# gabegrand/VQA-Counterexamples

Hardware: AMD Instinct MI355X
Metric: VQA-CX triplets/sec (24 candidates each), NeuralCX training step (higher is better)
Workload: dtype f32; 1 GPU; configs[1]: NeuralCX MLP train step (fwd+listwise loss/recall+bwd+Adam), synthetic 2048-d feats, 24 candidates, batch 512 per GPU (weak scaling: global batch 512), H=256, L=1, dropout 0.25, fp32; global_batch=512, per_rank_batch=512, candidates=24, dim_h=256, n_layers=1, parallelism=dp1, feature_table_rows=82783

## Files before the change

### include/neuralcx.h

```cpp
#ifndef NEURALCX_H
#define NEURALCX_H

#include <stddef.h>
#include <stdint.h>

#ifdef __cplusplus
extern "C" {
#endif

#define NCX_OK            0
#define NCX_E_NULL       -1
#define NCX_E_DIMS       -2
#define NCX_E_WORKSPACE  -3
#define NCX_E_FLAGS      -4
#define NCX_E_UNSUPPORTED -5
#define NCX_E_COMM       -6

#define NCX_F_V_MULT   (1u << 0)
#define NCX_F_V_DIST   (1u << 1)
#define NCX_F_V_RANK   (1u << 2)
#define NCX_F_A_EMB    (1u << 3)
#define NCX_F_ALL      (NCX_F_V_MULT | NCX_F_V_DIST | NCX_F_V_RANK | NCX_F_A_EMB)
#define NCX_F_BF16     (1u << 4)
#define NCX_F_REUSE_GT (1u << 5)
#define NCX_F_FUSED_TAIL (1u << 6)
#define NCX_F_X6       (1u << 7)

typedef struct ncx_dims {
    int32_t B;
    int32_t K;
    int32_t dv;
    int32_t dq;
    int32_t dz;
    int32_t da;
    int32_t A;
    int32_t H;
    int32_t L;
    int32_t n_img;
    uint32_t flags;
    int32_t training;
    float   drop_p;
    float   loss_scale;
    uint64_t seed;
} ncx_dims;

typedef struct ncx_inputs {
    const float*   feats;
    const int32_t* img_idx;
    const float*   q_emb;
    const float*   z_orig;
    const float*   z_knns;
    const float*   a_knns;
    const int32_t* answer_aids;
    const float*   a_emb_gt;
    const float*   v_rank;
    const float*   keep_mask;
} ncx_inputs;

typedef struct ncx_params {
    const float* answer_embedding;
    const float* w1;  const float* b1;
    const float* w2;  const float* b2;
    const float* w3;  const float* b3;
    const float* w_out; const float* b_out;
} ncx_params;

typedef struct ncx_grads {
    float* answer_embedding;
    float* w1;  float* b1;
    float* w2;  float* b2;
    float* w3;  float* b3;
    float* w_out; float* b_out;
} ncx_grads;

int64_t ncx_input_size(const ncx_dims* d);

size_t ncx_workspace_bytes(const ncx_dims* d);

int ncx_forward(const ncx_dims* d, const ncx_inputs* in, const ncx_params* p,
                void* workspace, size_t workspace_bytes, float* scores, void* stream);

#define NCX_FWD_ALL     0
#define NCX_FWD_PRELUDE 1
#define NCX_FWD_REST    2
int ncx_forward_phase(const ncx_dims* d, const ncx_inputs* in, const ncx_params* p,
                      void* workspace, size_t workspace_bytes, float* scores, int32_t phase, void* stream);

int ncx_loss_rank(const float* scores, const int32_t* gt, int32_t B, int32_t K, float scale,
                  float* loss_rows, float* loss, float* dscores, int32_t* rank, int32_t* hits,
                  void* stream);

int ncx_backward(const ncx_dims* d, const ncx_inputs* in, const ncx_params* p,
                 void* workspace, size_t workspace_bytes, const float* dscores,
                 const ncx_grads* g, void* stream);

int ncx_backward_phase(const ncx_dims* d, const ncx_inputs* in, const ncx_params* p,
                       void* workspace, size_t workspace_bytes, const float* dscores,
                       const ncx_grads* g, int32_t phase, void* stream);

#define NCX_WS_DGT 1
#define NCX_WS_H1 2
#define NCX_WS_DPRE1 3
#define NCX_WS_DE_PERM 4
int ncx_ws_region(const ncx_dims* d, int32_t which, size_t* offset, size_t* bytes);

int ncx_train_tail(const ncx_dims* d, const ncx_params* p, void* workspace, size_t workspace_bytes, const int32_t* gt,
                   float* scores, float* loss_rows, float* loss, float* dscores, int32_t* rank, int32_t* hits,
                   const ncx_grads* g, void* stream);

#define NCX_COMM_ID_BYTES 128
typedef struct ncx_comm ncx_comm;
int ncx_comm_unique_id(void* id128);
int ncx_comm_create(const void* id128, int32_t nranks, int32_t rank, ncx_comm** out);
int ncx_comm_destroy(ncx_comm* comm);
int ncx_allreduce(ncx_comm* comm, float* buf, size_t n, void* stream);

int ncx_adam_step(float* param, const float* grad, float* exp_avg, float* exp_avg_sq, size_t n,
                  float lr, float beta1, float beta2, float eps, int32_t step, float grad_scale,
                  void* stream);

typedef struct ncx_mutan_params {
    const float* wv;  const float* bv;
    const float* wq;  const float* bq;
    const float* whv; const float* bhv;
    const float* whq; const float* bhq;
    const float* wc;  const float* bc;
    int32_t dhv, dhq, R;
    int32_t act_v, act_q;
} ncx_mutan_params;

size_t ncx_vqa_workspace_bytes(const ncx_dims* d, const ncx_mutan_params* m);

int ncx_vqa_forward(const ncx_dims* d, const float* feats, const int32_t* img_idx, const float* q_emb,
                    const ncx_mutan_params* m, void* workspace, size_t workspace_bytes,
                    float* z_orig, float* z_knns, float* a_knns, float* a_orig, void* stream);

typedef struct ncx_mlb_params {
    const float* wv;  const float* bv;
    const float* wq;  const float* bq;
    const float* wc;  const float* bc;
    int32_t dh;
    int32_t act_v, act_q, act_c;
} ncx_mlb_params;

size_t ncx_mlb_workspace_bytes(const ncx_dims* d, const ncx_mlb_params* m);

int ncx_mlb_forward(const ncx_dims* d, const float* feats, const int32_t* img_idx, const float* q_emb,
                    const ncx_mlb_params* m, void* workspace, size_t workspace_bytes,
                    float* z_orig, float* z_knns, float* a_knns, float* a_orig, void* stream);

typedef struct ncx_mlb_att_dims {
    int32_t B, P, dv, dq, dh_att, G, dh_f, A, n_img;
} ncx_mlb_att_dims;
typedef struct ncx_mlb_att_params {
    const float* wv_att; const float* bv_att;
    const float* wq_att; const float* bq_att;
    const float* wa;     const float* ba;
    const float* wg;     const float* bg;
    const float* wqf;    const float* bqf;
    const float* wc;     const float* bc;
    int32_t act_v_att, act_q_att, act_mm;
    int32_t act_v, act_q, act_c;
} ncx_mlb_att_params;

size_t ncx_mlb_att_workspace_bytes(const ncx_mlb_att_dims* d, const ncx_mlb_att_params* m);

int ncx_mlb_att_forward(const ncx_mlb_att_dims* d, const float* feats, const int32_t* img_idx, const float* q_emb,
                        const ncx_mlb_att_params* m, void* workspace, size_t workspace_bytes,
                        float* logits, float* att, void* stream);
int ncx_mlb_att_forward_flags(const ncx_mlb_att_dims* d, const float* feats, const int32_t* img_idx, const float* q_emb,
                              const ncx_mlb_att_params* m, uint32_t flags, void* workspace, size_t workspace_bytes,
                              float* logits, float* att, void* stream);
int ncx_mlb_att_logits_form(const ncx_mlb_att_dims* d, uint32_t flags);

size_t ncx_knn_status_offset(int32_t n);
size_t ncx_knn_workspace_bytes(int32_t n, int32_t block_rows);
int ncx_knn(const float* table, int32_t n, const float* queries, int32_t nq, int32_t dv, int32_t k,
            int32_t norms_ready, void* workspace, size_t workspace_bytes, int64_t* out_idx, float* out_dist,
            void* stream);

size_t ncx_cosine_gram_workspace_bytes(int32_t A, int32_t da);
int ncx_cosine_gram(const float* emb, int32_t A, int32_t da, void* ws, size_t ws_bytes, float* gram, void* stream);
int ncx_semantic_scores(const float* a_knns, const int32_t* aid, int32_t B, int32_t K, int32_t A, const float* gram,
                        float lam, float* scores, float* raw, int32_t* bad_id_flag, void* stream);

int ncx_similarity_scores(const float* feats, const int32_t* img_idx, int32_t n_img, int32_t dv,
                          const float* z_orig, const float* z_knns, int32_t dz,
                          const float* a_knns, const int32_t* aid, int32_t A,
                          int32_t B, int32_t K,
                          float* scores , float* parts ,
                          int32_t* bad_id_flag, void* stream);

size_t ncx_gru_packed_bytes(int32_t dim_emb, int32_t dim_q);
int ncx_gru_pack(const float* w_ih, const float* w_hh, const float* b_ih, const float* b_hh, int32_t dim_emb, int32_t dim_q,
                 float* packed, void* stream);
size_t ncx_gru_workspace_bytes(int32_t B, int32_t T, int32_t dim_emb, int32_t dim_q);
int ncx_gru_encode(const int32_t* wids, int32_t B, int32_t T, const float* E, int32_t V1, int32_t dim_emb, int32_t dim_q,
                   const float* packed, void* workspace, size_t workspace_bytes, float* q_out, int32_t* bad_id_flag, void* stream);
int ncx_gru_encode_flags(const int32_t* wids, int32_t B, int32_t T, const float* E, int32_t V1, int32_t dim_emb, int32_t dim_q,
                         const float* packed, uint32_t flags, void* workspace, size_t workspace_bytes, float* q_out, int32_t* bad_id_flag,
                         void* stream);
int ncx_gru_step_form(int32_t B, int32_t T, int32_t dim_emb, int32_t dim_q, uint32_t flags);

size_t ncx_gru_train_workspace_bytes(int32_t B, int32_t T, int32_t dim_emb, int32_t dim_q);
size_t ncx_gru_packed_t_bytes(int32_t dim_emb, int32_t dim_q);
int ncx_gru_pack_t(const float* w_ih, const float* w_hh, int32_t dim_emb, int32_t dim_q, float* packed_t, void* stream);
int ncx_gru_train_forward(const int32_t* wids, int32_t B, int32_t T, const float* E, int32_t V1, int32_t dim_emb, int32_t dim_q,
                          const float* packed, void* workspace, size_t workspace_bytes, float* q_out, int32_t* bad_id_flag, void* stream);
int ncx_gru_train_forward_flags(const int32_t* wids, int32_t B, int32_t T, const float* E, int32_t V1, int32_t dim_emb, int32_t dim_q,
                                const float* packed, uint32_t flags, void* workspace, size_t workspace_bytes, float* q_out,
                                int32_t* bad_id_flag, void* stream);
int ncx_gru_train_backward(const int32_t* wids, int32_t B, int32_t T, const float* E, int32_t V1, int32_t dim_emb, int32_t dim_q,
                           const float* packed_t, void* workspace, size_t workspace_bytes, const float* dq_out,
                           float* dW_ih, float* dW_hh, float* db_ih, float* db_hh, float* dE , void* stream);

size_t ncx_lstm2_packed_bytes(int32_t emb, int32_t H);
int ncx_lstm2_pack(const float* w_ih0, const float* w_hh0, const float* b_ih0, const float* b_hh0, const float* w_ih1, const float* w_hh1,
                   const float* b_ih1, const float* b_hh1, int32_t emb, int32_t H, float* packed, void* stream);
size_t ncx_lstm2_workspace_bytes(int32_t B, int32_t T, int32_t emb, int32_t H);
int ncx_lstm2_encode(const int32_t* wids, int32_t B, int32_t T, const float* E, int32_t V1, int32_t emb, int32_t H, const float* packed,
                     void* workspace, size_t workspace_bytes, float* q_out, int32_t* bad_id_flag, void* stream);

size_t ncx_lstm2_train_workspace_bytes(int32_t B, int32_t T, int32_t emb, int32_t H);
size_t ncx_lstm2_packed_t_bytes(int32_t emb, int32_t H);
int ncx_lstm2_pack_t(const float* w_ih0, const float* w_hh0, const float* w_ih1, const float* w_hh1, int32_t emb, int32_t H, float* packed_t,
                     void* stream);
int ncx_lstm2_train_forward(const int32_t* wids, int32_t B, int32_t T, const float* E, int32_t V1, int32_t emb, int32_t H, const float* packed,
                            void* workspace, size_t workspace_bytes, float* q_out, int32_t* bad_id_flag, void* stream);
int ncx_lstm2_train_backward(const int32_t* wids, int32_t B, int32_t T, const float* E, int32_t V1, int32_t emb, int32_t H, const float* packed_t,
                             void* workspace, size_t workspace_bytes, const float* dq_out, float* dW_ih0, float* dW_hh0, float* db_ih0,
                             float* db_hh0, float* dW_ih1, float* dW_hh1, float* db_ih1, float* db_hh1, float* dE , void* stream);

typedef struct ncx_scorer_dims {
    int32_t B, K, dv, dq, dz, A, n_img;
} ncx_scorer_dims;

typedef struct ncx_pairlin_params {
    const float* answer_embedding;
    const float* w;  const float* b;
    const float* w_out; const float* b_out;
} ncx_pairlin_params;
typedef struct ncx_pairlin_grads {
    float* answer_embedding; float* w; float* b; float* w_out; float* b_out;
} ncx_pairlin_grads;

size_t ncx_pairlin_workspace_bytes(const ncx_scorer_dims* d);
int ncx_pairlin_forward(const ncx_scorer_dims* d, const ncx_inputs* in, const ncx_pairlin_params* p, void* workspace,
                        size_t workspace_bytes, float* scores, int32_t* bad_id_flag, void* stream);
int ncx_pairlin_backward(const ncx_scorer_dims* d, const ncx_inputs* in, const ncx_pairlin_params* p, void* workspace,
                         size_t workspace_bytes, const float* dscores, const ncx_pairlin_grads* g, void* stream);
size_t ncx_linctx_workspace_bytes(const ncx_scorer_dims* d);
int ncx_linctx_forward(const ncx_scorer_dims* d, const float* z_knns, const float* w, const float* b, void* workspace,
                       size_t workspace_bytes, float* scores, void* stream);
int ncx_linctx_backward(const ncx_scorer_dims* d, const float* z_knns, const float* dscores, void* workspace,
                        size_t workspace_bytes, float* gw, float* gb, void* stream);

typedef struct ncx_contrastive_dims {
    int32_t B, P, dv, dz, n_img;
} ncx_contrastive_dims;
size_t ncx_contrastive_workspace_bytes(const ncx_contrastive_dims* d);
int ncx_contrastive_forward(const ncx_contrastive_dims* d, const ncx_inputs* in, const float* w, const float* b, void* workspace,
                            size_t workspace_bytes, float* h, int32_t* bad_id_flag, void* stream);
int ncx_contrastive_distances(const ncx_contrastive_dims* d, const float* h, void* workspace, size_t workspace_bytes, float* dist,
                              void* stream);
int ncx_contrastive_loss(const ncx_contrastive_dims* d, void* workspace, size_t workspace_bytes, float margin, float scale,
                         float* losses4, float* dist, void* stream);
int ncx_contrastive_backward(const ncx_contrastive_dims* d, const ncx_inputs* in, void* workspace, size_t workspace_bytes,
                             const float* dh, float* gw, float* gb, void* stream);

typedef struct ncx_vqa_train_dims {
    int32_t B, dv, dq, dz, A, n_img;
    float   p_v, p_q, p_c;
    int32_t dropout_mode;
    int32_t want_dq;
    int32_t pad_;
    uint64_t seed;
} ncx_vqa_train_dims;
typedef struct ncx_mutan_grads {
    float* wv;  float* bv;  float* wq;  float* bq;  float* whv; float* bhv; float* whq; float* bhq; float* wc;  float* bc;
} ncx_mutan_grads;
size_t ncx_vqa_train_workspace_bytes(const ncx_vqa_train_dims* d, const ncx_mutan_params* m);
int ncx_vqa_train_forward(const ncx_vqa_train_dims* d, const float* feats, const int32_t* img_idx, const float* q_emb,
                          const ncx_mutan_params* m, const float* masks, void* workspace, size_t workspace_bytes,
                          float* logits, float* z, void* stream);
int ncx_ce_loss(const float* logits, const int32_t* target, int32_t B, int32_t A, float scale, float* loss, float* dlogits,
                int32_t* hits_top1, int32_t* hits_top5, int32_t* bad_flag, float* rows, void* stream);
int ncx_vqa_train_backward(const ncx_vqa_train_dims* d, const ncx_mutan_params* m, const float* masks, void* workspace,
                           size_t workspace_bytes, const float* dlogits, const ncx_mutan_grads* g, float* dq_emb, void* stream);
#define NCX_VT_WS_VD 1
#define NCX_VT_WS_QD 2
#define NCX_VT_WS_ZC 3
int ncx_vqa_train_ws_region(const ncx_vqa_train_dims* d, const ncx_mutan_params* m, int32_t which, size_t* offset, size_t* bytes);

typedef struct ncx_mlb_grads {
    float* wv;  float* bv;  float* wq;  float* bq;  float* wc;  float* bc;
} ncx_mlb_grads;
size_t ncx_mlb_train_workspace_bytes(const ncx_vqa_train_dims* d, const ncx_mlb_params* m);
int ncx_mlb_train_forward(const ncx_vqa_train_dims* d, const float* feats, const int32_t* img_idx, const float* q_emb,
                          const ncx_mlb_params* m, const float* masks, void* workspace, size_t workspace_bytes,
                          float* logits, float* z, void* stream);
int ncx_mlb_train_backward(const ncx_vqa_train_dims* d, const ncx_mlb_params* m, const float* masks, void* workspace,
                           size_t workspace_bytes, const float* dlogits, const ncx_mlb_grads* g, float* dq_emb, void* stream);
int ncx_mlb_train_ws_region(const ncx_vqa_train_dims* d, const ncx_mlb_params* m, int32_t which, size_t* offset, size_t* bytes);

typedef struct ncx_mlb_att_train {
    float    p_att_v, p_att_q, p_att_mm, p_v, p_q, p_c;
    int32_t  dropout_mode;
    int32_t  want_dq;
    uint64_t seed;
} ncx_mlb_att_train;
typedef struct ncx_mlb_att_grads {
    float* wv_att; float* bv_att; float* wq_att; float* bq_att; float* wa; float* ba;
    float* wg;     float* bg;     float* wqf;    float* bqf;    float* wc; float* bc;
} ncx_mlb_att_grads;
size_t ncx_mlb_att_train_workspace_bytes(const ncx_mlb_att_dims* d, const ncx_mlb_att_train* t, const ncx_mlb_att_params* m);
int ncx_mlb_att_train_forward(const ncx_mlb_att_dims* d, const ncx_mlb_att_train* t, const float* feats, const int32_t* img_idx,
                              const float* q_emb, const ncx_mlb_att_params* m, const float* masks, void* workspace,
                              size_t workspace_bytes, float* logits, float* att, void* stream);
int ncx_mlb_att_train_forward_flags(const ncx_mlb_att_dims* d, const ncx_mlb_att_train* t, const float* feats, const int32_t* img_idx,
                                    const float* q_emb, const ncx_mlb_att_params* m, const float* masks, uint32_t flags, void* workspace,
                                    size_t workspace_bytes, float* logits, float* att, void* stream);
int ncx_mlb_att_train_backward(const ncx_mlb_att_dims* d, const ncx_mlb_att_train* t, const float* feats, const int32_t* img_idx,
                               const float* q_emb, const ncx_mlb_att_params* m, const float* masks, void* workspace,
                               size_t workspace_bytes, const float* att, const float* dlogits, const ncx_mlb_att_grads* g,
                               float* dq_emb, void* stream);
int ncx_mlb_att_train_backward_flags(const ncx_mlb_att_dims* d, const ncx_mlb_att_train* t, const float* feats, const int32_t* img_idx,
                                     const float* q_emb, const ncx_mlb_att_params* m, const float* masks, uint32_t flags, void* workspace,
                                     size_t workspace_bytes, const float* att, const float* dlogits, const ncx_mlb_att_grads* g,
                                     float* dq_emb, void* stream);
int ncx_mlb_att_dwv_form(const ncx_mlb_att_dims* d, uint32_t flags);
#define NCX_AT_WS_XV     1
#define NCX_AT_WS_VATT   2
#define NCX_AT_WS_T      3
#define NCX_AT_WS_VD     4
#define NCX_AT_WS_DWV    5
int ncx_mlb_att_train_ws_region(const ncx_mlb_att_dims* d, const ncx_mlb_att_train* t, const ncx_mlb_att_params* m, int32_t which,
                                size_t* offset, size_t* bytes);

#define NCX_GEMM_GT 0
#define NCX_GEMM_SH 1
#define NCX_GEMM_MAIN 2
#define NCX_GEMM_FWD_L 3
#define NCX_GEMM_DW1C 4
#define NCX_GEMM_DW1S 5
#define NCX_GEMM_DE 6
#define NCX_GEMM_DW1AK 7
#define NCX_GEMM_DAGT 8
#define NCX_GEMM_DWL 9
#define NCX_GEMM_DXL 10
#define NCX_QUERY_DW1_ROUTE 32
int ncx_profile_begin(uint32_t gemm_mask , int32_t max_launches);
int ncx_profile_end(float* ms, int32_t* ids, int32_t cap);
int ncx_profile_stamps(unsigned long long* stamps, int64_t words);
int ncx_plan_query(const ncx_dims* d, int32_t gemm_id, int32_t* out6);
int ncx_wgmap_check(int32_t tiles_m, int32_t tiles_n, int32_t S);

const char* ncx_version(void);

#ifdef __cplusplus
}
#endif
#endif
```

### vqa-counterexamples_amd/csrc/ncx_backward.hip

```cpp
#include "ncx_driver.h"
#include "ncx_wave.h"
#include "ncx_dwred.h"
#include "ncx_bf16.h"

namespace ncx {
__global__ __launch_bounds__(256) void k_dpre_last(const float* __restrict__ gs, const float* __restrict__ w_out,
                                                   const float* __restrict__ h, float* __restrict__ dpre,
                                                   long long total, int H, float scale) {
    long long i = ((long long)blockIdx.x * 256 + threadIdx.x) * 4;
    if (i >= total) return;
    const int r = (int)(i / H), n = (int)(i - (long long)r * H);
    if (n + 3 < H && i + 3 < total) {
        const f32x4 hv = *(const f32x4u*)(h + i);
        const f32x4 wv = *(const f32x4u*)(w_out + n);
        const float g = gs[r];
        f32x4 o;
#pragma unroll
        for (int j = 0; j < 4; ++j) o[j] = hv[j] > 0.f ? g * wv[j] * scale : 0.f;
        *(f32x4u*)(dpre + i) = o;
    } else {
        for (int j = 0; j < 4 && i + j < total; ++j) {
            const int rr = (int)((i + j) / H), nn = (int)((i + j) - (long long)rr * H);
            dpre[i + j] = h[i + j] > 0.f ? gs[rr] * w_out[nn] * scale : 0.f;
        }
// ... 230 lines not shown
                const float gk = __shfl(dsc, k, 64);
                f32x4 dp;
#pragma unroll
                for (int q = 0; q < 4; ++q) { dp[q] = hv[k][q] > 0.f ? gk * w[q] * gate_scale : 0.f; aw[q] = __builtin_fmaf(gk, hv[k][q], aw[q]); ds[q] += dp[q]; }
                put4(dpre + (r0 + k) * H, dp);
            }
        }
        if (dsh) { put4(dsh + (long long)b * H, ds); ab1 += ds; }
    }
    put4(partial_w + (long long)wv * H, aw);
    if (dsh) put4(partial_b1 + (long long)wv * H, ab1);
    sb = wave_sum(sb);
    if (lane == 0) partial_b[wv] = sb;
}

__global__ __launch_bounds__(256) void k_rowgroup_sum(const float* __restrict__ dpre, int B, int K, int H,
                                                      float* __restrict__ dsh) {
    const long long i = (long long)blockIdx.x * 256 + threadIdx.x;
    if (i >= (long long)B * H) return;
    const int b = (int)(i / H), n = (int)(i - (long long)b * H);
    const float* p = dpre + (long long)b * K * H + n;
    float s = 0.f;
    for (int k = 0; k < K; ++k) s += p[(long long)k * H];
    dsh[i] = s;
}

__global__ __launch_bounds__(256) void k_scatter_dsh_by_answer(const float* __restrict__ dsh, const int* __restrict__ aid,
                                                               int B, int H, int A, float* __restrict__ dggt) {
    __shared__ unsigned bits[NCX_SCATTER_MAX_B / 32];
    const int b = blockIdx.x;
    const int id = aid[b];
    int earlier = 0;
    for (int j = threadIdx.x; j < b; j += 256) earlier |= aid[j] == id;
    if (__syncthreads_or(earlier)) return;
    const int nw = (B + 31) / 32;
    for (int w = threadIdx.x; w < nw; w += 256) bits[w] = 0u;
    __syncthreads();
    for (int j = b + threadIdx.x; j < B; j += 256)
        if (aid[j] == id) atomicOr(&bits[j >> 5], 1u << (j & 31));
    __syncthreads();
    for (int n = threadIdx.x; n < H; n += 256) {
        float s = 0.f;
        for (int w = b >> 5; w < nw; ++w) {
            unsigned m = bits[w];
            while (m) {
                const int j = (w << 5) + __ffs(m) - 1;
                m &= m - 1;
                s += dsh[(long long)j * H + n];
            }
        }
        dggt[(long long)n * A + id] = s;
    }
}

struct EmbPrepArgs {
    const float* dsh; const int* aid; float* dggtT;
    const float* src[3]; float* dst[3]; long long lds_[3]; int cols[3], ldd[3], dcols[3], tile0[4];
    int B, H, A, Hp4;
    int* perm;
};
__global__ __launch_bounds__(256) void k_emb_prep(const EmbPrepArgs a, const FixupArgs fix, const Tn8ReduceArgs red) {
    __shared__ unsigned bits[NCX_SCATTER_MAX_B / 32 > 32 * 33 ? NCX_SCATTER_MAX_B / 32 : 32 * 33];
    const int bx = (int)blockIdx.x - (a.perm ? 1 : 0);
    if (bx < 0) {
        __shared__ int scan[256];
        static_assert(NCX_PERM_MAX_A / 32 <= (int)(sizeof(bits) / sizeof(bits[0])), "one bit per answer");
        const int A = a.A, nw = (A + 31) / 32, per = (nw + 255) / 256, tid = threadIdx.x;
        for (int w = tid; w < nw; w += 256) bits[w] = 0u;
        __syncthreads();
        for (int j = tid; j < a.B; j += 256) {
            const int id = a.aid[j];
            if ((unsigned)id < (unsigned)A) atomicOr(&bits[id >> 5], 1u << (id & 31));
        }
        __syncthreads();
        const int w0 = min(tid * per, nw), w1 = min(w0 + per, nw);
        int cnt = 0;
        for (int w = w0; w < w1; ++w) cnt += __popc(bits[w]);
        scan[tid] = cnt;
        __syncthreads();
        for (int off = 1; off < 256; off <<= 1) {
            const int v = tid >= off ? scan[tid - off] : 0;
            __syncthreads();
            scan[tid] += v;
            __syncthreads();
        }
        const int n_present = scan[255];
        int pos = scan[tid] - cnt;
        for (int w = w0; w < w1; ++w) {
            const unsigned m = bits[w];
            for (int bit = 0; bit < 32; ++bit) {
                const int id = 32 * w + bit;
                if (id >= A) break;
                if ((m >> bit) & 1u) a.perm[pos++] = id;
                else a.perm[n_present + (id - pos)] = id;
            }
        }
        if (tid == 0) a.perm[A] = n_present;
        return;
    }
    if (bx >= a.B + a.tile0[3]) {
        const int id = bx - (a.B + a.tile0[3]);
        const int nfix = fix.valid ? fix.grid_x * 4 : 0;
        if (id < nfix) split_fixup_body<64, 64>(fix, id / 4, id % 4);
        else tn8_reduce_body(red, id - nfix);
        return;
    }
    if (bx < a.B) {
        const int b = bx, B = a.B;
        const int id = a.aid[b];
        int earlier = 0;
        for (int j = threadIdx.x; j < b; j += 256) earlier |= a.aid[j] == id;
        if (__syncthreads_or(earlier)) return;
        const int nw = (B + 31) / 32;
        for (int w = threadIdx.x; w < nw; w += 256) bits[w] = 0u;
        __syncthreads();
        for (int j = b + threadIdx.x; j < B; j += 256)
            if (a.aid[j] == id) atomicOr(&bits[j >> 5], 1u << (j & 31));
        __syncthreads();
        for (int n = threadIdx.x; n < a.H; n += 256) {
            float s = 0.f;
            for (int w = b >> 5; w < nw; ++w) {
                unsigned m = bits[w];
                while (m) { const int j = (w << 5) + __ffs(m) - 1; m &= m - 1; s += a.dsh[(long long)j * a.H + n]; }
            }
            a.dggtT[(long long)id * a.Hp4 + n] = s;
        }
        return;
    }
    float* tile = (float*)bits;
    int t = bx - a.B, e = 0;
    while (e < 2 && t >= a.tile0[e + 1]) ++e;
    t -= a.tile0[e];
    const int tiles_h = (a.dcols[e] + 31) / 32;
    const int th = t % tiles_h, tc = t / tiles_h;
    const int x = threadIdx.x & 31, y = threadIdx.x >> 5;
#pragma unroll
    for (int i = 0; i < 4; ++i) {
        const int h = th * 32 + y + 8 * i, c = tc * 32 + x;
        tile[(y + 8 * i) * 33 + x] = (h < a.H && c < a.cols[e]) ? a.src[e][(long long)h * a.lds_[e] + c] : 0.f;
    }
    __syncthreads();
#pragma unroll
    for (int i = 0; i < 4; ++i) {
        const int c = tc * 32 + y + 8 * i, h = th * 32 + x;
        if (c < a.cols[e] && h < a.dcols[e]) a.dst[e][(long long)c * a.ldd[e] + h] = tile[x * 33 + y + 8 * i];
    }
}

__global__ __launch_bounds__(256) void k_zero_cols(float* __restrict__ p, int rows, long long ld, int cols) {
    const long long i = (long long)blockIdx.x * 256 + threadIdx.x;
    if (i >= (long long)rows * cols) return;
    const int r = (int)(i / cols), c = (int)(i - (long long)r * cols);
    p[(long long)r * ld + c] = 0.f;
}
}

using namespace ncx;
extern "C" {
int ncx_train_tail(const ncx_dims* dp, const ncx_params* p, void* workspace, size_t workspace_bytes, const int32_t* gt,
                   float* scores, float* loss_rows, float* loss, float* dscores, int32_t* rank, int32_t* hits,
                   const ncx_grads* g, void* stream_) {
    int rc = check_dims(dp);
    if (rc != NCX_OK) return rc;
    if (!p || !workspace || !gt || !scores || !loss_rows || !rank || !g) return NCX_E_NULL;
    if (!p->w_out || !p->b_out || !g->w_out || !g->b_out || !g->b1) return NCX_E_NULL;
    const ncx_dims& d = *dp;
    if (!(d.flags & NCX_F_FUSED_TAIL)) return NCX_E_FLAGS;
    if (d.K > 32 || d.H > 256) return NCX_E_DIMS;
    const StepRoutes r = routes(d);
    const WsLayout w = ws_layout(d, r);
    if (workspace_bytes < w.total || ((uintptr_t)workspace & 255)) return NCX_E_WORKSPACE;
    hipStream_t s = (hipStream_t)stream_;
    char* ws = (char*)workspace;
    const int H = d.H;
    const bool aemb = d.flags & NCX_F_A_EMB;
    const bool emb_nt = r.emb_nt;
    const int Hp4 = pad_to(H, 4);
    float* dagtT = (float*)(ws + w.dgtT) + (size_t)d.A * Hp4;
    float* dagt = (float*)(ws + w.dagt);
    float* partial = (float*)(ws + w.partial);
    float* part_w = partial;
    float* part_b1 = partial + (size_t)NCX_PRELUDE_WAVES * H;
    float* part_b = partial + (size_t)NCX_PRELUDE_WAVES * H * 2;
    const float dscale = (d.training && d.drop_p > 0.f) ? 1.f / (1.f - d.drop_p) : 1.f;
    const float scale = d.loss_scale > 0.f ? d.loss_scale : 1.f / (float)d.B;
    const int nblk = (int)cdiv(d.B < NCX_PRELUDE_WAVES ? d.B : NCX_PRELUDE_WAVES, 4);
    const bool fuse_l1 = d.L == 1;
    const float* hL = (const float*)(ws + w.h[d.L - 1]);
    float* dpre = (float*)(ws + w.dpre[0]);
    float* dsh = fuse_l1 ? (float*)(ws + w.dsh) : (float*)nullptr;
    float* zb = emb_nt ? dagtT : aemb ? dagt : (float*)nullptr;
    const long long zn = emb_nt ? (long long)d.A * Hp4 : (long long)H * d.A;
#define NCX_TAIL_LAUNCH(KB, FULL) hipLaunchKernelGGL((k_train_tail<KB, FULL>), dim3(nblk * 4), dim3(64), 0, s, hL, p->w_out, p->b_out, gt, d.B, d.K, H, scale, dscale, \
                                               scores, loss_rows, dscores, rank, dpre, dsh, part_w, part_b1, part_b, zb, zn, zchunk)
    const int zchunk = (int)((cdiv(zn, (long long)nblk * 4) + 3) / 4 * 4);
    if (H == 256 && d.K == 24) NCX_TAIL_LAUNCH(24, true);
    else if (d.K <= 8) NCX_TAIL_LAUNCH(8, false); else if (d.K <= 16) NCX_TAIL_LAUNCH(16, false); else if (d.K <= 24) NCX_TAIL_LAUNCH(24, false); else NCX_TAIL_LAUNCH(32, false);
#undef NCX_TAIL_LAUNCH
    NCX_HIP_TRY(hipGetLastError());
    hipLaunchKernelGGL(k_bwd_prelude_finish, dim3((unsigned)cdiv(H, 8), 3), dim3(256), 0, s, (const float*)part_w, (const float*)part_b1,
                       (const float*)part_b, nblk * 4, H, g->w_out, fuse_l1 ? g->b1 : (float*)nullptr, g->b_out,
                       (const float*)loss_rows, (const int*)rank, d.B, loss, hits);
    NCX_HIP_TRY(hipGetLastError());
    return NCX_OK;
}

static int backward_impl(const ncx_dims* dp, const ncx_inputs* in, const ncx_params* p, void* workspace,
                         size_t workspace_bytes, const float* dscores, const ncx_grads* g, void* stream_, int phase) {
    int rc = check_dims(dp);
    if (rc != NCX_OK) return rc;
    if (!in || !p || !workspace || !g || (!dscores && !(dp->flags & NCX_F_FUSED_TAIL))) return NCX_E_NULL;
    const ncx_dims& d = *dp;
    const bool aemb = d.flags & NCX_F_A_EMB;
    if (!g->answer_embedding || !g->w1 || !g->b1 || !g->w_out || !g->b_out) return NCX_E_NULL;
    if (d.L >= 2 && (!g->w2 || !g->b2)) return NCX_E_NULL;
    if (d.L >= 3 && (!g->w3 || !g->b3)) return NCX_E_NULL;
    const StepRoutes r = routes(d);
    const WsLayout w = ws_layout(d, r);
    if (workspace_bytes < w.total || ((uintptr_t)workspace & 255)) return NCX_E_WORKSPACE;
    hipStream_t s = (hipStream_t)stream_;
    char* ws = (char*)workspace;
    const int M = d.B * d.K, H = d.H;
    const SegOffsets o = seg_offsets(d);
    const long long din = o.din;
    const int* idx_k = (const int*)(ws + w.idx_k); const int* idx_o = (const int*)(ws + w.idx_o);
    const int* idx_ob = (const int*)(ws + w.idx_ob);
    const float* mx = (const float*)(ws + w.mx); const float* inv = (const float*)(ws + w.inv);
    const float* misc = (const float*)(ws + w.misc);
    float* dsh = (float*)(ws + w.dsh); float* dgt = (float*)(ws + w.dgt); float* dagt = (float*)(ws + w.dagt);
    const bool emb_nt = r.emb_nt;
    const int Hp4 = pad_to(H, 4), Hp32 = pad_to(H, 32);
    float* dgtT = (float*)(ws + w.dgtT); float* dagtT = dgtT + (size_t)d.A * Hp4;
    float* w1akT = (float*)(ws + w.w1aT); float* w1agtT = w1akT + (size_t)d.da * Hp32;
    float* partial = (float*)(ws + w.partial); float* slab = (float*)(ws + w.slab);
    GemmUse u[U_COUNT];
    list_uses(d, r, u);
    const float dscale = (d.training && d.drop_p > 0.f) ? 1.f / (1.f - d.drop_p) : 1.f;

    auto colsum = [&](const float* x, const float* wgt, int rows, int cols, float* out) -> int {
        const int ch = rows < NCX_COLSUM_CHUNKS * 8 ? (int)cdiv(rows, 8) : NCX_COLSUM_CHUNKS;
        hipLaunchKernelGGL(k_colsum_partial, dim3((unsigned)cdiv(cols, 256), ch), dim3(256), 0, s, x, wgt, rows, cols, partial);
        hipLaunchKernelGGL(k_colsum_finish, dim3((unsigned)cdiv(cols, 8)), dim3(256), 0, s, (const float*)partial, ch, cols, out);
        return (int)hipGetLastError();
    };

    const float* hL = (const float*)(ws + w.h[d.L - 1]);
    float* dpre = (float*)(ws + w.dpre[0]);
    const bool only_de = phase == 4;
    const bool skip_de = phase == 3 || phase == 5;
    const bool do1 = phase != 2 && !only_de, do2 = phase != 1 && phase != 5 && !only_de;
    const bool de_skip = r.de_skip && (phase == 0 || phase == 1);
    int* const de_perm = (int*)(ws + w.de_perm);
    if (!do1) {
        dpre = (float*)(ws + w.dpre[(d.L - 1) & 1]);
    } else if (d.flags & NCX_F_FUSED_TAIL) {
    } else {
        const int nblk = (int)cdiv(d.B < NCX_PRELUDE_WAVES ? d.B : NCX_PRELUDE_WAVES, 4);
        float* part_w = partial;
        float* part_b1 = partial + (size_t)NCX_PRELUDE_WAVES * H;
        float* part_b = partial + (size_t)NCX_PRELUDE_WAVES * H * 2;
        const bool fuse_l1 = d.L == 1;
        hipLaunchKernelGGL(k_bwd_prelude, dim3(nblk), dim3(256), 0, s, dscores, p->w_out, hL, dpre, fuse_l1 ? dsh : (float*)nullptr,
                           d.B, d.K, H, dscale, part_w, part_b1, part_b,
                           emb_nt ? dagtT : aemb ? dagt : (float*)nullptr, emb_nt ? (long long)d.A * Hp4 : (long long)H * d.A);
        NCX_HIP_TRY(hipGetLastError());
        hipLaunchKernelGGL(k_bwd_prelude_finish, dim3((unsigned)cdiv(H, 8), fuse_l1 ? 2 : 1), dim3(256), 0, s, (const float*)part_w,
                           (const float*)part_b1, (const float*)part_b, nblk * 4, H, g->w_out, fuse_l1 ? g->b1 : (float*)nullptr, g->b_out);
        NCX_HIP_TRY(hipGetLastError());
    }
    int cur = 0;
    for (int l = d.L; l >= 2 && do1; --l) {
        const float* wl = l == 2 ? p->w2 : p->w3;
        float* gw = l == 2 ? g->w2 : g->w3;
        float* gb = l == 2 ? g->b2 : g->b3;
        const float* hprev = (const float*)(ws + w.h[l - 2]);
        rc = colsum(dpre, nullptr, M, H, gb); if (rc) return rc;
        {
            GemmArgs a{}; a.mode = MODE_GROUP; a.nseg = 1; a.M = H;
            a.a[0] = x_plain(dpre, H, M, H); a.b[0] = x_plain(hprev, H, M, H); a.klen[0] = M;
            a.out[0] = gw; a.ldo[0] = H; a.n_cols[0] = H;
            rc = run_gemm(U_DWL, a, FORM_TN, u[U_DWL].plan, slab, w.slab_bytes, nullptr, s); if (rc) return rc;
        }
        {
            float* dnext = (float*)(ws + w.dpre[cur ^ 1]);
            GemmArgs a{}; a.mode = MODE_CHAIN; a.nseg = 1; a.M = M;
            a.a[0] = x_plain(dpre, H, M, H); a.b[0] = x_plain(wl, H, H, H); a.klen[0] = H;
            a.out[0] = dnext; a.ldo[0] = H; a.n_cols[0] = H;
            a.epi.gate = hprev; a.epi.ld_gate = H; a.epi.gate_scale = dscale;
            rc = run_gemm(U_DXL, a, FORM_NN, u[U_DXL].plan, slab, w.slab_bytes, nullptr, s); if (rc) return rc;
            dpre = dnext; cur ^= 1;
        }
    }
    if (do1 && d.L >= 2) {
        hipLaunchKernelGGL(k_rowgroup_sum, dim3((unsigned)cdiv((long long)d.B * H, 256)), dim3(256), 0, s, (const float*)dpre, d.B, d.K, H, dsh);
        NCX_HIP_TRY(hipGetLastError());
        rc = colsum(dsh, nullptr, d.B, H, g->b1); if (rc) return rc;
    }
    bool km_deferred = false, km_reduced = false;
    auto run_km = [&](bool finish = true) -> int {
        return profiled(U_DW1C, s, [&] { return dw_km(d, dpre, in->feats, idx_k, idx_o, (float*)(ws + w.km_slab), g->w1 + o.v_other, g->w1 + o.v_mult, din, s, finish); });
    };
    {
        GemmArgs a{}; a.mode = MODE_GROUP; a.M = H;
        int n = 0;
        auto add_c = [&](const XDesc& x, float* out, long long ldo) {
            a.a[n] = x_plain(dpre, H, M, H); a.b[n] = x; a.klen[n] = M; a.out[n] = out; a.ldo[n] = ldo; a.n_cols[n] = x.cols;
            a.split[n] = dw1c_seg_split(x.cols, u[U_DW1C].plan.split, u[U_DW1C].ksteps); ++n; };
        auto add_s = [&](const XDesc& x, float* out) {
            a.a[n] = x_plain(dsh, H, d.B, H); a.b[n] = x; a.klen[n] = d.B; a.out[n] = out; a.ldo[n] = din; a.n_cols[n] = x.cols;
            a.split[n] = u[U_DW1S].plan.split; ++n; };
        const bool bf16 = d.flags & NCX_F_BF16;
        const bool want_dgt = aemb && do1 && !bf16, want_rest = do2;
        if (bf16 && do1) {
            rc = profiled(U_DW1C, s, [&] { return bf16_dw1c(d, dpre, (u16*)(ws + w.dpre_bf), (const u16*)(ws + w.xc), (float*)(ws + w.bf_slab), g->w1, dgt, s); }); if (rc) return rc;
        }
        const bool km = r.km;
        const bool tn8 = r.tn8;
        km_deferred = want_rest && do1 && do2 && km_defers_to_side_stream(d, r);
        const bool km_merge = want_rest && km && !km_deferred && !hook_env("NCX_NO_MERGE_FIX");
        if (want_rest && km && !km_deferred) {
            rc = run_km(!km_merge); if (rc) return rc;
        }
        if (want_rest && !bf16 && !km) {
            add_c(x_gather(in->feats, d.dv, idx_k, M, d.dv), g->w1 + o.v_other, din);
            if (d.flags & NCX_F_V_MULT) add_c(x_gather_mul(in->feats, d.dv, idx_k, idx_o, M, d.dv), g->w1 + o.v_mult, din);
        }
        if (tn8 && (want_dgt || want_rest)) {
            Tn8Prob tp[TN8_MAX_PROB]; int np = 0, n_al = 0;
            auto prob = [&](const float* A_, int rows, const float* X, long long ldx, const float* lse, int gsel, int N, float* out, long long ldo, int n_valid) {
                tp[np] = Tn8Prob{};
                Tn8Prob& q = tp[np++]; q.A = A_; q.rows = rows; q.X = X; q.ldx = ldx; q.lse = lse; q.gsel = gsel; q.N = N; q.out = out; q.ldo = ldo; q.n_valid = n_valid; };
            if (aemb) {
                prob(dpre, M, in->a_knns, d.A, mx, 0, d.A, dgt, d.A, d.A); n_al = 1;
                if (emb_nt) {
                    tp[0].outT = dgtT; tp[0].outT2 = (float*)(ws + w.dgtT2); tp[0].ldT = Hp4; tp[0].padT2 = pad_to(d.A, 32) - d.A;
                }
            }
            else prob(dpre, M, in->a_knns, d.da, nullptr, 0, d.da, g->w1 + o.a_other, din, d.da);
            prob(dpre, M, in->z_knns, d.dz, nullptr, 0, d.dz, g->w1 + o.z_other, din, d.dz);
            prob(dpre, M, misc, w.ldm, nullptr, 0, w.ldm, g->w1 + o.v_dist, din, d.K + 1);
            prob(dsh, d.B, in->feats, d.dv, nullptr, 1, d.dv, g->w1 + o.v_orig, din, d.dv);
            prob(dsh, d.B, in->q_emb, d.dq, nullptr, 0, d.dq, g->w1 + o.q_emb, din, d.dq);
            prob(dsh, d.B, in->z_orig, d.dz, nullptr, 0, d.dz, g->w1 + o.z_orig, din, d.dz);
            if (aemb) prob(dsh, d.B, p->answer_embedding, d.da, nullptr, 2, d.da, g->w1 + o.a_gt, din, d.da);
            else      prob(dsh, d.B, in->a_emb_gt, d.da, nullptr, 0, d.da, g->w1 + o.a_gt, din, d.da);
            const bool with_km = want_rest && km && !km_deferred && km_merge;
            Tn8ReduceArgs red{};
            rc = prof_open(U_DW1C, s); if (rc) return rc;
            rc = dw_tn8_products(d, tp, np, n_al, want_dgt, want_rest, idx_ob, aemb ? in->answer_aids : nullptr, slab, w.slab_bytes, &red, s); if (rc) return rc;
            bool kvec = true;
            KmReduceArgs kr{};
            if (with_km) { kr = dw_km_reduce_args(d, (const float*)(ws + w.km_slab), g->w1 + o.v_other, g->w1 + o.v_mult, din, &kvec); km_reduced = true; }
            rc = dw_reduce_km_tn8(with_km ? &kr : nullptr, kvec, &red, s); if (rc) return rc;
            rc = prof_close(U_DW1C, s); if (rc) return rc;
        }
        if (want_rest && !bf16 && !tn8) {
            if (!aemb) add_c(x_plain(in->a_knns, d.da, M, d.da), g->w1 + o.a_other, din);
        }
        if (want_dgt && !tn8) add_c(x_softmax(in->a_knns, d.A, mx, inv, M, d.A), dgt, d.A);
        if (want_rest && !bf16 && !tn8) {
            add_c(x_plain(in->z_knns, d.dz, M, d.dz), g->w1 + o.z_other, din);
            add_c(x_plain(misc, w.ldm, M, d.K + 1), g->w1 + o.v_dist, din);
        }
        if (want_rest && bf16 && r.tn8_shared) {
            Tn8Prob tp[4]; int np = 0;
            auto prob = [&](const float* X, long long ldx, int gsel, int N, float* out) {
                tp[np] = Tn8Prob{};
                Tn8Prob& q = tp[np++]; q.A = dsh; q.rows = d.B; q.X = X; q.ldx = ldx; q.gsel = gsel; q.N = N; q.out = out; q.ldo = din; q.n_valid = N; };
            prob(in->feats, d.dv, 1, d.dv, g->w1 + o.v_orig);
            prob(in->q_emb, d.dq, 0, d.dq, g->w1 + o.q_emb);
            prob(in->z_orig, d.dz, 0, d.dz, g->w1 + o.z_orig);
            if (aemb) prob(p->answer_embedding, d.da, 2, d.da, g->w1 + o.a_gt);
            else      prob(in->a_emb_gt, d.da, 0, d.da, g->w1 + o.a_gt);
            rc = dw_tn8(d, tp, np, 0, false, true, idx_ob, aemb ? in->answer_aids : nullptr, slab, w.slab_bytes, s); if (rc) return rc;
        } else
        if (want_rest && !tn8) {
            add_s(x_gather(in->feats, d.dv, idx_ob, d.B, d.dv), g->w1 + o.v_orig);
            add_s(x_plain(in->q_emb, d.dq, d.B, d.dq), g->w1 + o.q_emb);
            add_s(x_plain(in->z_orig, d.dz, d.B, d.dz), g->w1 + o.z_orig);
            add_s(aemb ? x_gather(p->answer_embedding, d.da, in->answer_aids, d.B, d.da) : x_plain(in->a_emb_gt, d.da, d.B, d.da),
                  g->w1 + o.a_gt);
        }
        a.nseg = n;
        FixupArgs fix_tn{};
        if (km_merge) a.defer_fix = &fix_tn;
        if (n > 0) { rc = run_gemm(U_DW1C, a, FORM_TN, u[U_DW1C].plan, slab, w.slab_bytes, nullptr, s); if (rc) return rc; }
        if (km_merge && !km_reduced) {
            rc = profiled(U_DW1C, s, [&] { return dw_km_finish(d, (const float*)(ws + w.km_slab), g->w1 + o.v_other, g->w1 + o.v_mult, din, &fix_tn, u[U_DW1C].plan.cfg, s); }); if (rc) return rc;
        }
        if (!(d.flags & NCX_F_V_MULT) && do2) {
            hipLaunchKernelGGL(k_zero_cols, dim3((unsigned)cdiv((long long)H * d.dv, 256)), dim3(256), 0, s, g->w1 + o.v_mult, H, din, d.dv);
            NCX_HIP_TRY(hipGetLastError());
        }
    }
    if (aemb) {
        SideStream* ss = km_deferred ? side_stream() : nullptr;
        hipStream_t se = ss ? ss->s : s;
        FixupArgs fix_ak{};
        Tn8ReduceArgs red_ak{};
        const bool tn8_ak = r.dw1ak_on_tn8(ss != nullptr);
        if (ss) { rc = side_fork(ss, s); if (rc) return rc; }
        const bool bf16e = d.flags & NCX_F_BF16;
        const Bf16Emb bm = bf16e ? bf16_emb_layout(d, ws + w.bf_emb) : Bf16Emb{};
        if (do2 && bf16e) {
            rc = profiled(U_DW1AK, se, [&] { return bf16_dw1ak(d, bm, dgt, g->w1, se); }); if (rc) return rc;
        } else if (do2 && tn8_ak) {
            Tn8Prob q{};
            q.A = (const float*)(ws + w.dgtT2); q.rows = pad_to(d.A, 32); q.rows_valid = d.A; q.X = p->answer_embedding; q.ldx = d.da; q.N = d.da;
            q.out = g->w1 + o.a_other; q.ldo = din; q.n_valid = d.da;
            rc = prof_open(U_DW1AK, se); if (rc) return rc;
            rc = dw_tn8_products(d, &q, 1, 0, false, true, nullptr, nullptr, slab, w.slab_bytes, &red_ak, se); if (rc) return rc;
            if (!(do1 && emb_nt)) { rc = dw_reduce_km_tn8(nullptr, true, &red_ak, se); if (rc) return rc; red_ak.n_tiles_total = 0; }
            rc = prof_close(U_DW1AK, se); if (rc) return rc;
        } else if (do2) {
            GemmArgs a{}; a.mode = MODE_CHAIN; a.nseg = 1; a.M = H;
            a.a[0] = x_plain(dgt, d.A, H, d.A); a.b[0] = x_plain(p->answer_embedding, d.da, d.A, d.da); a.klen[0] = d.A;
            a.out[0] = g->w1 + o.a_other; a.ldo[0] = din; a.n_cols[0] = d.da;
            if (do1 && emb_nt && u[U_DW1AK].plan.cfg == CFG_64x64 && !hook_env("NCX_NO_MERGE_FIX")) a.defer_fix = &fix_ak;
            rc = run_gemm(U_DW1AK, a, FORM_NN, u[U_DW1AK].plan, ss ? (float*)(ws + w.slab2) : slab,
                          ss ? w.slab2_bytes : w.slab_bytes, nullptr, se); if (rc) return rc;
        }
        if (do1 && emb_nt) {
            EmbPrepArgs ea{};
            ea.dsh = dsh; ea.aid = in->answer_aids; ea.dggtT = dagtT; ea.B = d.B; ea.H = H; ea.A = d.A; ea.Hp4 = Hp4;
            const float* srcs[3] = {dgt, p->w1 + o.a_other, p->w1 + o.a_gt};
            float* dsts[3] = {dgtT, w1akT, w1agtT};
            const long long ldss[3] = {d.A, din, din};
            const int colss[3] = {tn8_ak ? 0 : d.A, d.da, d.da}, ldds[3] = {Hp4, Hp32, Hp32};
            int tiles = 0;
            for (int e = 0; e < 3; ++e) {
                ea.src[e] = srcs[e]; ea.dst[e] = dsts[e]; ea.lds_[e] = ldss[e]; ea.cols[e] = colss[e]; ea.ldd[e] = ldds[e]; ea.dcols[e] = ldds[e];
                ea.tile0[e] = tiles; tiles += ((ldds[e] + 31) / 32) * ((colss[e] + 31) / 32);
            }
            ea.tile0[3] = tiles;
            ea.perm = de_skip ? de_perm : (int*)nullptr;
            hipLaunchKernelGGL(k_emb_prep, dim3((de_skip ? 1 : 0) + d.B + tiles + (fix_ak.valid ? fix_ak.grid_x * 4 : 0) + red_ak.n_tiles_total * 8), dim3(256), 0, se, ea, fix_ak, red_ak);
            fix_ak.valid = 0; red_ak.n_tiles_total = 0;
            NCX_HIP_TRY(hipGetLastError());
        } else if (do1) {
            hipLaunchKernelGGL(k_scatter_dsh_by_answer, dim3(d.B), dim3(256), 0, se, (const float*)dsh, in->answer_aids, d.B, H, d.A, dagt);
            NCX_HIP_TRY(hipGetLastError());
        }
        if (fix_ak.valid) { rc = run_fixup2(fix_ak, FixupArgs{}, CFG_64x64, se); if (rc) return rc; }
        if (((do1 && !skip_de) || only_de) && bf16e) {
            rc = profiled(U_DE, se, [&] { return bf16_de(d, bm, dgt, g->answer_embedding, se); }); if (rc) return rc;
        } else if (((do1 && !skip_de) || only_de) && emb_nt) {
            MainArgs a{}; a.M = d.A; a.N = d.da; a.nseg = 2;
            a.seg[0].kind = MK_PLAIN; a.seg[0].a = dgtT;  a.seg[0].lda = Hp4; a.seg[0].klen = Hp4; a.seg[0].b = w1akT;  a.seg[0].ldb = Hp32;
            a.seg[1].kind = MK_PLAIN; a.seg[1].a = dagtT; a.seg[1].lda = Hp4; a.seg[1].klen = Hp4; a.seg[1].b = w1agtT; a.seg[1].ldb = Hp32;
            a.out = g->answer_embedding; a.ldo = d.da;
            a.split = 1;
            if (de_skip) {
                a.seg[0].kind = MK_GATHER; a.seg[0].idx = de_perm;
                a.seg[1].kind = MK_GATHER; a.seg[1].idx = de_perm;
            }
            rc = profiled(U_DE, se, [&] { return de_skip ? main_forward_rowmap(a, se) : main_forward(a, se); }); if (rc) return rc;
        } else if ((do1 && !skip_de) || only_de) {
            GemmArgs a{}; a.mode = MODE_CHAIN; a.nseg = 2; a.M = d.A;
            a.a[0] = x_plain(dgt, d.A, H, d.A);  a.b[0] = x_plain(p->w1 + o.a_other, din, H, d.da); a.klen[0] = H;
            a.a[1] = x_plain(dagt, d.A, H, d.A); a.b[1] = x_plain(p->w1 + o.a_gt, din, H, d.da);    a.klen[1] = H;
            a.out[0] = g->answer_embedding; a.ldo[0] = d.da; a.n_cols[0] = d.da;
            rc = run_gemm(U_DE, a, FORM_TN, u[U_DE].plan, ss ? (float*)(ws + w.slab2) : slab, ss ? w.slab2_bytes : w.slab_bytes, nullptr, se); if (rc) return rc;
        }
        if (km_deferred) { rc = run_km(); if (rc) return rc; }
        if (ss) { rc = side_join(ss, s); if (rc) return rc; }
    } else if (do1) {
        NCX_HIP_TRY(hipMemsetAsync(g->answer_embedding, 0, (size_t)d.A * d.da * 4, s));
    }
    return NCX_OK;
}

int ncx_backward(const ncx_dims* dp, const ncx_inputs* in, const ncx_params* p, void* workspace,
                 size_t workspace_bytes, const float* dscores, const ncx_grads* g, void* stream_) {
    return backward_impl(dp, in, p, workspace, workspace_bytes, dscores, g, stream_, 0);
}

int ncx_backward_phase(const ncx_dims* dp, const ncx_inputs* in, const ncx_params* p, void* workspace,
                       size_t workspace_bytes, const float* dscores, const ncx_grads* g, int32_t phase, void* stream_) {
    if (phase < 0 || phase > 5) return NCX_E_FLAGS;
    return backward_impl(dp, in, p, workspace, workspace_bytes, dscores, g, stream_, phase);
}

int ncx_ws_region(const ncx_dims* dp, int32_t which, size_t* offset, size_t* bytes) {
    if (check_dims(dp) != NCX_OK) return NCX_E_DIMS;
    if (!offset || !bytes) return NCX_E_NULL;
    if (which != NCX_WS_DGT && which != NCX_WS_H1 && which != NCX_WS_DPRE1 && which != NCX_WS_DE_PERM) return NCX_E_FLAGS;
    const StepRoutes r = routes(*dp);
    const WsLayout w = ws_layout(*dp, r);
    if (which == NCX_WS_DE_PERM) {
        *offset = w.de_perm; *bytes = r.de_skip ? ((size_t)dp->A + 1) * 4 : 0;
        return NCX_OK;
    }
    if (which == NCX_WS_H1 || which == NCX_WS_DPRE1) {
        *offset = which == NCX_WS_H1 ? w.h[0] : w.dpre[(dp->L - 1) & 1];
        *bytes = (size_t)dp->B * dp->K * dp->H * 4;
        return NCX_OK;
    }
    if (!r.emb_nt) { *offset = w.dgt; *bytes = (dp->flags & NCX_F_A_EMB) ? (size_t)2 * dp->H * dp->A * 4 : 0; }
    else { *offset = w.dgtT; *bytes = (size_t)2 * dp->A * pad_to(dp->H, 4) * 4; }
    return NCX_OK;
}
}
```

### vqa-counterexamples_amd/csrc/ncx_diag.hip

```cpp
#include "ncx_driver.h"
#include <stdlib.h>

using namespace ncx;
extern "C" {
int ncx_profile_begin(uint32_t gemm_mask, int32_t max_launches) {
    if (g_prof.on || gemm_mask == 0 || (gemm_mask >> U_COUNT) != 0 || max_launches < 1 || max_launches > 65536) return NCX_E_DIMS;
    g_prof.ev = (hipEvent_t*)malloc(sizeof(hipEvent_t) * 2 * (size_t)max_launches);
    g_prof.ids = (int*)malloc(sizeof(int) * (size_t)max_launches);
    if (!g_prof.ev || !g_prof.ids) return NCX_E_NULL;
    for (int i = 0; i < 2 * max_launches; ++i) NCX_HIP_TRY(hipEventCreate(&g_prof.ev[i]));
    g_prof.mask = gemm_mask; g_prof.n = 0; g_prof.cap = max_launches; g_prof.on = true;
    return NCX_OK;
}

int ncx_profile_end(float* ms, int32_t* ids, int32_t cap) {
    if (!g_prof.on) return NCX_E_FLAGS;
    int n = 0;
    for (int i = 0; i < g_prof.n; ++i) {
        if (hipEventSynchronize(g_prof.ev[2 * i + 1]) != hipSuccess) break;
        float t = 0.f;
        if (hipEventElapsedTime(&t, g_prof.ev[2 * i], g_prof.ev[2 * i + 1]) != hipSuccess) break;
        if (n < cap) { if (ms) ms[n] = t; if (ids) ids[n] = g_prof.ids[i]; }
        ++n;
    }
    for (int i = 0; i < 2 * g_prof.cap; ++i) (void)hipEventDestroy(g_prof.ev[i]);
    free(g_prof.ev); free(g_prof.ids);
    g_prof.ev = nullptr; g_prof.ids = nullptr; g_prof.on = false; g_prof.mask = 0; g_prof.n = 0; g_prof.cap = 0;
    return n < cap ? n : cap;
}

int ncx_profile_stamps(unsigned long long* stamps, int64_t words) {
    if ((stamps == nullptr) != (words == 0) || words < 0) return NCX_E_DIMS;
    int dev = 0;
    NCX_HIP_TRY(hipGetDevice(&dev));
    if (dev < 0 || dev >= 16) return NCX_E_DIMS;
    if (!stamps) { g_stamps[dev].ptr.store(nullptr, std::memory_order_release); g_stamps[dev].words.store(0, std::memory_order_release); }
    else { g_stamps[dev].ptr.store(nullptr, std::memory_order_release); g_stamps[dev].words.store(words, std::memory_order_release);
           g_stamps[dev].ptr.store(stamps, std::memory_order_release); }
    return NCX_OK;
}

int ncx_wgmap_check(int32_t tiles_m, int32_t tiles_n, int32_t S) {
    if (tiles_m < 1 || tiles_n < 1 || S < 1 || (long long)tiles_m * tiles_n * S > (1 << 24)) return NCX_E_DIMS;
    const WgMap w{tiles_m, tiles_n, S};
    const int total = tiles_m * tiles_n * S, count = w.count();
    if (count < total) return 1;
    unsigned char* seen = (unsigned char*)calloc((size_t)total, 1);
    if (!seen) return NCX_E_NULL;
    int bad = 0, nvalid = 0;
    for (int lw = 0; lw < count && !bad; ++lw) {
        int tm = -1, tn = -1, z = -1;
        if (!w.decode(lw, tm, tn, z)) continue;
        ++nvalid;
        if (tm < 0 || tm >= tiles_m || tn < 0 || tn >= tiles_n || z < 0 || z >= S) { bad = 2; break; }
        if (w.encode(tm, tn, z) != lw) { bad = 3; break; }
        unsigned char& f = seen[((size_t)z * tiles_m + tm) * tiles_n + tn];
        if (f) { bad = 4; break; }
        f = 1;
    }
    if (!bad && nvalid != total) bad = 5;
    free(seen);
    return bad;
}

int ncx_plan_query(const ncx_dims* d, int32_t gemm_id, int32_t* out6) {
    if (check_dims(d) != NCX_OK || !out6) return NCX_E_DIMS;
    if (gemm_id == NCX_QUERY_DW1_ROUTE) {
        const bool bf16 = d->flags & NCX_F_BF16;
        const StepRoutes r = routes(*d);
        out6[0] = r.km_form;
        out6[1] = (bf16 ? r.tn8_shared : r.tn8) ? (r.tn8_x6 ? 2 : 1) : 0;
        int grid = 0;
        out6[2] = dw_tn8_pieces(*d, bf16 ? TN8_LIST_SHARED : TN8_LIST_MAIN, &grid);
        out6[3] = grid;
        out6[4] = r.dw1ak_on_tn8(km_defers_to_side_stream(*d, r)) ? 1 : 0;
        out6[5] = TN8_MAX_SEG;
        return NCX_OK;
    }
    if (gemm_id < 0 || gemm_id >= U_COUNT) return NCX_E_DIMS;
    GemmUse u[U_COUNT];
    list_uses(*d, routes(*d), u);
    out6[0] = u[gemm_id].form; out6[1] = (int32_t)u[gemm_id].M; out6[2] = (int32_t)u[gemm_id].N;
    out6[3] = (int32_t)u[gemm_id].ksteps; out6[4] = u[gemm_id].plan.cfg; out6[5] = u[gemm_id].plan.split;
    const bool fast = (gemm_id == U_MAIN && main_fwd_dims_ok(*d)) || (gemm_id == U_FWD_L && hidden_fwd_dims_ok(*d) && !(d->flags & NCX_F_BF16));
    if (fast) {
        const long long M = (long long)d->B * d->K, T = u[gemm_id].ksteps;
        const int sp = main_split(M, d->H, T);
        const bool vfold = gemm_id == U_MAIN && (d->flags & NCX_F_V_MULT) && (d->K == 24 || (d->K == 48 && main_fold_rows(M, d->H) >= 96)) && d->dv % 32 == 0 && d->dv >= 64 && sp == 1;
        const long long tiles96 = ((M + 95) / 96) * ((d->H + 127) / 128);
        out6[4] = vfold ? (main_fold_rows(M, d->H) == 192 ? 8 : (main_fold_rows(M, d->H) == 96 || d->K == 48) ? 7 : 6) : (sp == 1 && tiles96 * 10 >= (long long)num_cus() * 9) ? CFG_96x128 : 5;
        out6[5] = sp;
    }
    return NCX_OK;
}
}
```

### vqa-counterexamples_amd/csrc/ncx_driver.h

```cpp
#pragma once
#include "ncx_plan.h"
#include <atomic>

#pragma GCC visibility push(hidden)
namespace ncx {
struct SideStream { hipStream_t s; hipEvent_t fork, join; int state, mode; };
SideStream* side_stream();
int side_fork(SideStream* ss, hipStream_t main);
int side_join(SideStream* ss, hipStream_t main);
bool km_defers_to_side_stream(const ncx_dims& d, const StepRoutes& r);

struct ProfState { bool on; unsigned mask; int n, cap; hipEvent_t* ev; int* ids; };
extern ProfState g_prof;
struct StampSlot { std::atomic<unsigned long long*> ptr; std::atomic<long long> words; };
extern StampSlot g_stamps[16];
unsigned long long* stamps_for_current_device(long long need_words);
int prof_open(int use_id, hipStream_t s);
int prof_close(int use_id, hipStream_t s);
template <class F> static inline int profiled(int use_id, hipStream_t s, F&& launch) {
    int rc = prof_open(use_id, s); if (rc) return rc;
    rc = launch(); if (rc) return rc;
    return prof_close(use_id, s);
}
int run_gemm(int use_id, GemmArgs& a, int form, const GemmPlan& pl, float* slab, size_t slab_bytes, const float* reduce_bias, hipStream_t s);
void set_dropout(EpiArgs& e, const ncx_dims& d, const ncx_inputs& in, int layer, long long M);
}
#pragma GCC visibility pop
```

### vqa-counterexamples_amd/csrc/ncx_internal.h

```cpp
#pragma once
#include "ncx_common.h"
#include "ncx_gemm.h"

namespace ncx {

enum TileCfg : int { CFG_64x64 = 0, CFG_128x128 = 1, CFG_96x128 = 2, CFG_96x64 = 3, CFG_128x64 = 4 };
enum GemmForm : int { FORM_NT = 0, FORM_TN = 1, FORM_NN = 2 };

int run_gemm_nt(GemmArgs& a, int cfg, hipStream_t s);
int run_fixup2(const FixupArgs& a, const FixupArgs& b, int cfg, hipStream_t s);
int run_gemm_nt_fold(GemmArgs& a, hipStream_t s);
int run_gemm_tn(GemmArgs& a, int cfg, hipStream_t s);
int run_gemm_nn(GemmArgs& a, int cfg, hipStream_t s);
int occupancy_nt(int cfg);
int occupancy_tn(int cfg);
int occupancy_nn(int cfg);

struct SegOffsets {
    int v_orig, v_other, v_mult, v_dist, v_rank, q_emb, z_orig, z_other, a_gt, a_other, din;
};
static inline SegOffsets seg_offsets(const ncx_dims& d) {
    SegOffsets o; int c = 0;
    o.v_orig = c;  c += d.dv;
    o.v_other = c; c += d.dv;
    o.v_mult = c;  c += d.dv;
    o.v_dist = c;  c += 1;
    o.v_rank = c;  c += d.K;
    o.q_emb = c;   c += d.dq;
    o.z_orig = c;  c += d.dz;
    o.z_other = c; c += d.dz;
    o.a_gt = c;    c += d.da;
    o.a_other = c; c += d.da;
    o.din = c;
    return o;
}

struct GemmPlan { int cfg; int split; };
GemmPlan plan_gemm(int form, long long M, long long N, long long ksteps, bool allow_96);
int num_cus();
static inline long long cdiv(long long a, long long b) { return (a + b - 1) / b; }
static inline long long ksteps(long long k) { return cdiv(k, GEMM_BK); }
__attribute__((visibility("hidden"))) size_t gemm_slab_bytes(GemmArgs a, const GemmPlan& pl);
__attribute__((visibility("hidden"))) int run_gemm_planned(GemmArgs& a, int form, const GemmPlan& pl, float* slab, size_t slab_bytes,
                                                           const float* reduce_bias, hipStream_t s);
__attribute__((visibility("hidden"))) hipError_t colsum_rows(const float* in, long long ld, int R, int cols, float* out, hipStream_t s);

struct WsLayout {
    size_t idx_k, idx_o, idx_ob;
    size_t mx, inv;
    size_t misc;
    size_t gt;
    size_t sh;
    size_t h[3];
    size_t dpre[2];
    size_t dsh;
    size_t dgt;
    size_t dagt;
    size_t dgtT;
    size_t dgtT2;
    size_t de_perm;
    size_t w1aT;
    size_t partial;
    size_t slab;
    size_t slab_bytes;
    size_t slab2, slab2_bytes;
    size_t xc, wc, dpre_bf, bf_slab;
    size_t bf_emb;
    size_t km_slab;
    size_t mslab, mslab_bytes;
    size_t wpad;
    int ldm;
    int ldgt;
    size_t total;
};
constexpr int NCX_COLSUM_CHUNKS = 256;
constexpr int NCX_PRELUDE_WAVES = 1024;

enum MainKind : int { MK_PLAIN = 0, MK_GATHER = 1, MK_GATHER_MUL = 2, MK_SOFTMAX = 3,
                      MK_VFOLD = 4 };
constexpr int MAIN_MAX_SEG = 5;
struct MainSeg {
    const float* a;
    const int*   idx;
    const int*   idx2;
    const float* lse;
    const float* b;
    const float* b2;
    long long lda, ldb;
    int kind, klen;
};
struct MainArgs {
    MainSeg seg[MAIN_MAX_SEG]; int nseg, M, N, split; float* out; long long ldo; EpiArgs epi;
    float* slab;
    float* dist_out; long long ld_dist;
    unsigned long long* stamps;
    int x6;
    float* t_out; float* t_out0;
};
int main_forward(MainArgs& a, hipStream_t s);
int main_forward_rowmap(MainArgs& a, hipStream_t s);
int main_forward_mlb(MainArgs& a, hipStream_t s);
int main_split(long long M, long long N, long long T);
int main_fold_rows_eff(long long M, long long N, int rowdiv);
int main_fold_rows(long long M, long long N);

constexpr int DW_KM_SPLIT = 8;
bool dw_km_supported(const ncx_dims& d);
enum DwKmForm : int { KM_FORM_NONE = 0, KM_FORM_8 = 1, KM_FORM_X6 = 2, KM_FORM_GENERIC = 3, KM_FORM_GROUPED = 4 };
int dw_km_form(const ncx_dims& d);
size_t dw_km_slab_bytes(const ncx_dims& d);
int dw_km(const ncx_dims& d, const float* dpre, const float* feats, const int* idx_k, const int* idx_o, float* slab,
          float* g_vother, float* g_vmult, long long din, hipStream_t s, bool finish = true);
int dw_km_finish(const ncx_dims& d, const float* slab, float* g_vother, float* g_vmult, long long din, const FixupArgs* fix, int fix_cfg,
                 hipStream_t s);
constexpr int TN8_MAX_PROB = 8;
constexpr int TN8_MAX_SEG = 16;
struct Tn8Prob {
    const float* A;
    const float* X; long long ldx;
    const float* lse;
    int gsel;
    int rows, N;
    float* out; long long ldo; int n_valid;
    int rows_valid;
    float* outT; float* outT2; long long ldT; int padT2;
};
bool dw_tn8_supported(const ncx_dims& d);
bool dw_tn8_shapes_ok(const ncx_dims& d);
bool dw_tn8_shared_ok(const ncx_dims& d);
enum Tn8List : int { TN8_LIST_MAIN = 0, TN8_LIST_SHARED = 1, TN8_LIST_AK = 2 };
int dw_tn8_pieces(const ncx_dims& d, int list, int* grid);
bool dw_tn8_x6(const ncx_dims& d);
size_t dw_tn8_slab_bytes(const ncx_dims& d);
int dw_tn8(const ncx_dims& d, const Tn8Prob* probs, int np, int n_al, bool do_al, bool do_rest, const int* idx_ob, const int* aid,
           float* slab, size_t slab_bytes, hipStream_t s);
bool mutan_fold_supported(const ncx_dims& d, const ncx_mutan_params& m);
int mutan_fold(const ncx_dims& d, const ncx_mutan_params& m, const float* xv, const float* hq, float* z_orig, float* z_knns, hipStream_t s);
__attribute__((visibility("hidden"))) hipError_t pad_rows(const float* src, long long ld_src, int cols, float* dst, int ldd, int rows, hipStream_t s);
WsLayout ws_layout(const ncx_dims& d);
__host__ __device__ static inline int pad_to(int x, int m) { return (x + m - 1) / m * m; }
static inline bool main_fwd_extents_ok(const ncx_dims& d) {
    const long long lim = (1ll << 32) - 65536, M = (long long)d.B * d.K, wa = d.A > d.da ? d.A : d.da;
    return (long long)d.n_img * d.dv * 4 < lim && M * wa * 4 < lim && M * (long long)d.H * 4 < lim && M * (long long)d.dz * 4 < lim && (long long)d.A * wa * 4 < lim &&
           (long long)d.H * (2ll * d.dv + d.dq + 2ll * d.dz + 2ll * d.da + d.K + 2) * 4 < lim;
}
static inline bool main_fwd_dims_ok(const ncx_dims& d) {
    return d.dv % 4 == 0 && d.dz % 4 == 0 && ((d.flags & NCX_F_A_EMB) ? d.A : d.da) % 4 == 0 && !(d.flags & NCX_F_BF16) && main_fwd_extents_ok(d);
}
static inline bool hidden_fwd_dims_ok(const ncx_dims& d) { return d.H % 4 == 0 && main_fwd_extents_ok(d); }
constexpr uint32_t NCX_F_PRIV_DIST_IN_MAIN = 1u << 30;


}
```

### vqa-counterexamples_amd/csrc/ncx_loss_adam.hip

```cpp
#include "ncx_wave.h"

namespace ncx {
__global__ __launch_bounds__(256) void k_loss_rank(const float* __restrict__ scores, const int* __restrict__ gt,
                                                   int B, int K, float scale, float* __restrict__ loss_rows,
                                                   float* __restrict__ dscores, int* __restrict__ rank) {
    const int lane = threadIdx.x & 63;
    const int b = blockIdx.x * 4 + (threadIdx.x >> 6);
    if (b >= B) return;
    const float s = lane < K ? scores[(long long)b * K + lane] : -INFINITY;
    const int g = gt[b];
    const float m = wave_max(s);
    const float e = lane < K ? __expf(s - m) : 0.f;
    const float sum = wave_sum(e);
    const float sg = __shfl(s, g, 64);
    if (dscores && lane < K) dscores[(long long)b * K + lane] = (e / sum - (lane == g ? 1.f : 0.f)) * scale;
    const bool ahead = lane < K && (s > sg || (s == sg && lane < g));
    const unsigned long long bal = __ballot(ahead);
    if (lane == 0) {
        if (loss_rows) loss_rows[b] = (logf(sum) - (sg - m)) * scale;
        if (rank) rank[b] = __popcll(bal);
    }
}

__global__ __launch_bounds__(256) void k_loss_finish(const float* __restrict__ loss_rows, const int* __restrict__ rank,
                                                     int B, float* __restrict__ loss, int* __restrict__ hits) {
    __shared__ float sl[4];
    __shared__ int s1[4], s5[4];
    float acc = 0.f; int h1 = 0, h5 = 0;
    for (int i = threadIdx.x; i < B; i += 256) {
        if (loss_rows) acc += loss_rows[i];
        if (rank) { const int rk = rank[i]; h1 += rk < 1; h5 += rk < 5; }
    }
    acc = wave_sum(acc);
    h1 = (int)wave_sum((float)h1); h5 = (int)wave_sum((float)h5);
    const int w = threadIdx.x >> 6;
    if ((threadIdx.x & 63) == 0) { sl[w] = acc; s1[w] = h1; s5[w] = h5; }
    __syncthreads();
    if (threadIdx.x == 0) {
        if (loss) loss[0] = sl[0] + sl[1] + sl[2] + sl[3];
        if (hits) { hits[0] = s1[0] + s1[1] + s1[2] + s1[3]; hits[1] = s5[0] + s5[1] + s5[2] + s5[3]; }
    }
}

__global__ __launch_bounds__(256) void k_adam(float* __restrict__ p, const float* __restrict__ g, float* __restrict__ m,
                                              float* __restrict__ v, size_t n, float step_size, float b1, float b2,
                                              float eps, float inv_bc2_sqrt, float gscale) {
    size_t i = ((size_t)blockIdx.x * 256 + threadIdx.x) * 4;
    const size_t stride = (size_t)gridDim.x * 256 * 4;
    for (; i < n; i += stride) {
        if (i + 3 < n) {
            f32x4 pv = *(f32x4*)(p + i), gv = *(const f32x4*)(g + i), mv = *(f32x4*)(m + i), vv = *(f32x4*)(v + i);
#pragma unroll
            for (int j = 0; j < 4; ++j) {
                const float gj = gv[j] * gscale;
                mv[j] = mv[j] + (gj - mv[j]) * (1.f - b1);
                vv[j] = vv[j] * b2 + (1.f - b2) * gj * gj;
                const float den = sqrtf(vv[j]) * inv_bc2_sqrt + eps;
                pv[j] = pv[j] - step_size * (mv[j] / den);
            }
            *(f32x4*)(p + i) = pv; *(f32x4*)(m + i) = mv; *(f32x4*)(v + i) = vv;
        } else {
            for (size_t j = i; j < n; ++j) {
                const float gj = g[j] * gscale;
                const float mj = m[j] + (gj - m[j]) * (1.f - b1);
                const float vj = v[j] * b2 + (1.f - b2) * gj * gj;
                m[j] = mj; v[j] = vj;
                p[j] = p[j] - step_size * (mj / (sqrtf(vj) * inv_bc2_sqrt + eps));
            }
        }
    }
}
}

using namespace ncx;
extern "C" {
int ncx_loss_rank(const float* scores, const int32_t* gt, int32_t B, int32_t K, float scale, float* loss_rows,
                  float* loss, float* dscores, int32_t* rank, int32_t* hits, void* stream_) {
    if (!scores || !gt) return NCX_E_NULL;
    if (B < 1 || K < 1 || K > 64) return NCX_E_DIMS;
    if ((loss && !loss_rows) || (hits && !rank)) return NCX_E_NULL;
    hipStream_t s = (hipStream_t)stream_;
    if (scale <= 0.f) scale = 1.f / (float)B;
    hipLaunchKernelGGL(k_loss_rank, dim3((unsigned)cdiv(B, 4)), dim3(256), 0, s, scores, gt, B, K, scale, loss_rows, dscores, rank);
    NCX_HIP_TRY(hipGetLastError());
    if (loss || hits) {
        hipLaunchKernelGGL(k_loss_finish, dim3(1), dim3(256), 0, s, (const float*)loss_rows, (const int*)rank, B, loss, hits);
        NCX_HIP_TRY(hipGetLastError());
    }
    return NCX_OK;
}

int ncx_adam_step(float* param, const float* grad, float* exp_avg, float* exp_avg_sq, size_t n, float lr,
                  float beta1, float beta2, float eps, int32_t step, float grad_scale, void* stream_) {
    if (!param || !grad || !exp_avg || !exp_avg_sq) return NCX_E_NULL;
    if (step < 1 || n == 0) return NCX_E_DIMS;
    if (((uintptr_t)param | (uintptr_t)grad | (uintptr_t)exp_avg | (uintptr_t)exp_avg_sq) & 15) return NCX_E_WORKSPACE;
    const double bc1 = 1.0 - pow((double)beta1, (double)step);
    const double bc2 = 1.0 - pow((double)beta2, (double)step);
    const float step_size = (float)((double)lr / bc1);
    const float inv_bc2_sqrt = (float)(1.0 / sqrt(bc2));
    size_t blocks = (n + 1023) / 1024;
    if (blocks > 4096) blocks = 4096;
    hipLaunchKernelGGL(k_adam, dim3((unsigned)blocks), dim3(256), 0, (hipStream_t)stream_, param, grad, exp_avg, exp_avg_sq, n,
                       step_size, beta1, beta2, eps, inv_bc2_sqrt, grad_scale);
    NCX_HIP_TRY(hipGetLastError());
    return NCX_OK;
}
}
```

### vqa-counterexamples_amd/csrc/ncx_main.h

```cpp
#pragma once
#include "ncx_internal.h"
#include <type_traits>

namespace ncx {

constexpr int MF_BK = 32, MF_P = MF_BK + 4, MF_T = 256;

enum { LK_PLAIN = 0, LK_MUL = 1, LK_SOFTMAX = 2 };
template <int V> struct IntC { static constexpr int value = V; };

constexpr int MF6_P = 80;
template <int BM_, int BN_, int WGM_, int WGN_, int DEPTH_, int OCC_, int T_ = MF_T, bool X6_ = false>
struct MainCfg {
    static constexpr int BM = BM_, BN = BN_, WGM = WGM_, WGN = WGN_, DEPTH = DEPTH_, OCC = OCC_, T = T_;
    static constexpr bool X6 = X6_;
    static constexpr int EPI = 0;
    static constexpr int RP = T / 8;
    static constexpr int BM_LDS = (BM + RP - 1) / RP * RP;
    static constexpr int LDS6 = 2 * 3 * (BM_LDS + BN) * MF6_P;
    static constexpr int LDS_FOLD6 = 2 * (3 * 208 * MF6_P + 8 * 32 * 4 + 128 * MF_P * 4);
    static constexpr int LDS32 = 2 * (BM_LDS + BN) * MF_P * 4;
    static constexpr int LDS = !X6_ ? LDS32 : (LDS_FOLD6 > LDS6 ? (LDS_FOLD6 > LDS32 ? LDS_FOLD6 : LDS32) : (LDS6 > LDS32 ? LDS6 : LDS32));
    static constexpr int LDS_FOLD = BM % 96 == 0 ? 2 * (32 * (T / 64) + 128) * MF_P * 4
                                                 : 2 * (80 + 2 * 64) * MF_P * 4;
};

enum { EPI_STD = 0, EPI_MLB = 1, EPI_ROWMAP = 2 };
template <class CFG> struct WithMlbEpi : CFG { static constexpr int EPI = EPI_MLB; };
template <class CFG> struct WithRowMap : CFG { static constexpr int EPI = EPI_ROWMAP; };

typedef const __attribute__((address_space(1))) float* gfptr;
typedef const __attribute__((address_space(1))) int* giptr;
typedef const __attribute__((address_space(1))) f32x4u* gf4ptr;

template <class CFG, bool DIST, int K0, int K1 = -1, int K2 = -1, int K3 = -1, int K4 = -1>
__global__ __launch_bounds__(CFG::T, CFG::OCC) void k_main_fwd(const MainArgs args) {
    constexpr bool VFOLD = K0 == MK_VFOLD;
    constexpr int DIST_SEG = VFOLD ? 1 : 2;
    static_assert(!DIST || (VFOLD ? K1 == MK_PLAIN : (K1 == MK_GATHER_MUL && K2 == MK_PLAIN)), "DIST: v_o, v_k segment followed by the dist | rank segment");
    static_assert(!VFOLD || (CFG::BM == 48 && CFG::BN == 64 && CFG::WGM == 1 && CFG::WGN == 4 && CFG::DEPTH == 2) ||
                            (CFG::BM == 96 && CFG::BN == 64 && CFG::WGM == 2 && CFG::WGN == 2 && CFG::DEPTH == 2) ||
                            (CFG::BM == 192 && CFG::BN == 64 && CFG::T == 512 && CFG::WGM == 4 && CFG::WGN == 2 && CFG::DEPTH == 2), "fold: 48 x 64, 96 x 64 or (8 waves) 192 x 64 tiles");
    static_assert(!(DIST && CFG::X6), "the X6 form leaves the distance to k_prep");
    constexpr int KS[6] = {K0, K1, K2, K3, K4, -1};
    constexpr int NSEG = K1 < 0 ? 1 : K2 < 0 ? 2 : K3 < 0 ? 3 : K4 < 0 ? 4 : 5;
    constexpr int BM = CFG::BM, BN = CFG::BN, BK = MF_BK, P = MF_P, DEPTH = CFG::DEPTH, BML = CFG::BM_LDS;
    constexpr int WTM = BM / CFG::WGM, WTN = BN / CFG::WGN, WM = WTM / 16, WN = WTN / 16, NSUB = BK / 8, NMF = 2 * WM * WN;
    constexpr int MT = CFG::T, RP = CFG::RP;
    static_assert(CFG::WGM * CFG::WGN == MT / 64 && WTM % 16 == 0 && WTN % 16 == 0 && BN % RP == 0 && NSUB == 4, "tile");
    static_assert(MT == 256 || !VFOLD || BM % 96 == 0, "the 48-row fold is a 256-thread form");
    constexpr int NA = BML / RP, NB = BN / RP;
    extern __shared__ __attribute__((aligned(16))) float mf_smem[];
    float* const lds_a = mf_smem;
    float* const lds_b = mf_smem + 2 * BML * P;
    const int tid = threadIdx.x, lane = tid & 63, wave = tid >> 6, li = lane & 15, lk = lane >> 4;
    const int wm0 = (wave / CFG::WGN) * WTM, wn0 = (wave % CFG::WGN) * WTN;
    const int M = args.M, N = args.N;
    const int tiles_m = (M + BM - 1) / BM, tiles_n = (N + BN - 1) / BN;
    const int S = args.split > 1 ? args.split : 1;
    const int id = blockIdx.x, xcd = id & 7, local = id >> 3;
    const int tn = local % tiles_n, unit = (local / tiles_n) * 8 + xcd;
    if (unit >= tiles_m * S) return;
    const int tm = unit / S, z = unit - tm * S;
    const int m0 = tm * BM, n0 = tn * BN;
    const int quad = tid & 7, trow = tid >> 3;
    unsigned long long* const stamps = args.stamps ? args.stamps + (size_t)blockIdx.x * 16 : nullptr;
    auto stamp = [&](int slot) __attribute__((always_inline)) {
        if (stamps && tid == 0) stamps[slot] = __builtin_readcyclecounter();
    };
    if (stamps && tid == 0) { stamps[14] = __builtin_amdgcn_s_memrealtime(); stamps[13] = __builtin_amdgcn_s_getreg((3 << 11) | (0 << 6) | 20); }
    stamp(0);

    f32x4 acc[WM][WN];
#pragma unroll
    for (int i = 0; i < WM; ++i)
#pragma unroll
        for (int j = 0; j < WN; ++j) acc[i][j] = f32x4{0.f, 0.f, 0.f, 0.f};
    f32x2 afA[WM], bfA[WN], afB[WM], bfB[WN];
#pragma unroll
    for (int i = 0; i < WM; ++i) afB[i] = f32x2{0.f, 0.f};
#pragma unroll
    for (int j = 0; j < WN; ++j) bfB[j] = f32x2{0.f, 0.f};

    auto read_frags = [&](int buf, int s, f32x2 (&af)[WM], f32x2 (&bf)[WN]) __attribute__((always_inline)) {
        const float* a = lds_a + buf * BML * P + (wm0 + li) * P + 8 * s + 2 * lk;
        const float* b = lds_b + buf * BN * P + (wn0 + li) * P + 8 * s + 2 * lk;
#pragma unroll
        for (int i = 0; i < WM; ++i) af[i] = *(const f32x2*)(a + i * 16 * P);
#pragma unroll
        for (int j = 0; j < WN; ++j) bf[j] = *(const f32x2*)(b + j * 16 * P);
    };
    auto mfma = [&](const f32x2 (&af)[WM], const f32x2 (&bf)[WN]) __attribute__((always_inline)) {
#pragma unroll
        for (int e = 0; e < 2; ++e)
#pragma unroll
            for (int i = 0; i < WM; ++i)
#pragma unroll
                for (int j = 0; j < WN; ++j) acc[i][j] = __builtin_amdgcn_mfma_f32_16x16x4f32(af[i][e], bf[j][e], acc[i][j], 0, 0, 0);
    };

    constexpr bool X6 = CFG::X6;
    static_assert(!X6 || (VFOLD && BM == 192 && WM == 3 && WN == 2 && DEPTH == 2), "X6: the 8-wave 192 x 64 fold form only");
    typedef __bf16 mbf16x8 __attribute__((ext_vector_type(8)));
    typedef unsigned int mu32x2 __attribute__((ext_vector_type(2)));
    constexpr int P6 = MF6_P, A6_PL = BML * P6, PL6 = (BML + BN) * P6, BUF6 = 3 * PL6;
    unsigned char* const lds6 = (unsigned char*)mf_smem;
    mbf16x8 xa[2][3], xb[2][X6 ? WN : 1][3];
    auto split_store6 = [&](f32x4 v, unsigned char* base) __attribute__((always_inline)) {
        unsigned p1[4], p2[4], p3[4];
#pragma unroll
        for (int j = 0; j < 4; ++j) {
            const float xj = v[j];
            p1[j] = __builtin_bit_cast(unsigned, xj) & 0xFFFF0000u;
            const float r1 = xj - __builtin_bit_cast(float, p1[j]);
            p2[j] = __builtin_bit_cast(unsigned, r1) & 0xFFFF0000u;
            const float r2 = r1 - __builtin_bit_cast(float, p2[j]);
            p3[j] = __builtin_bit_cast(unsigned, r2);
        }
        const mu32x2 w1 = {__builtin_amdgcn_perm(p1[1], p1[0], 0x07060302u), __builtin_amdgcn_perm(p1[3], p1[2], 0x07060302u)};
        const mu32x2 w2 = {__builtin_amdgcn_perm(p2[1], p2[0], 0x07060302u), __builtin_amdgcn_perm(p2[3], p2[2], 0x07060302u)};
        const mu32x2 w3 = {__builtin_amdgcn_perm(p3[1], p3[0], 0x07060302u), __builtin_amdgcn_perm(p3[3], p3[2], 0x07060302u)};
        *(mu32x2*)(base) = w1; *(mu32x2*)(base + PL6) = w2; *(mu32x2*)(base + 2 * PL6) = w3;
    };
    auto read_a6 = [&](int buf, int i, mbf16x8 (&f)[3]) __attribute__((always_inline)) {
        const unsigned char* a = lds6 + buf * BUF6 + (wm0 + 16 * i + li) * P6 + 16 * lk;
#pragma unroll
        for (int p = 0; p < 3; ++p) f[p] = *(const mbf16x8*)(a + p * PL6);
    };
    auto read_b6 = [&](int buf, mbf16x8 (&f)[X6 ? WN : 1][3]) __attribute__((always_inline)) {
        const unsigned char* b = lds6 + buf * BUF6 + A6_PL + (wn0 + li) * P6 + 16 * lk;
#pragma unroll
        for (int j = 0; j < (X6 ? WN : 1); ++j)
#pragma unroll
            for (int p = 0; p < 3; ++p) f[j][p] = *(const mbf16x8*)(b + j * 16 * P6 + p * PL6);
    };
    auto mfma6 = [&](const mbf16x8 (&a)[3], const mbf16x8 (&b)[X6 ? WN : 1][3], f32x4 (&c)[WN]) __attribute__((always_inline)) {
        if constexpr (X6) {
#pragma unroll
            for (int j = 0; j < WN; ++j) c[j] = __builtin_amdgcn_mfma_f32_16x16x32_bf16(a[0], b[j][2], c[j], 0, 0, 0);
#pragma unroll
            for (int j = 0; j < WN; ++j) c[j] = __builtin_amdgcn_mfma_f32_16x16x32_bf16(a[1], b[j][1], c[j], 0, 0, 0);
#pragma unroll
            for (int j = 0; j < WN; ++j) c[j] = __builtin_amdgcn_mfma_f32_16x16x32_bf16(a[2], b[j][0], c[j], 0, 0, 0);
#pragma unroll
            for (int j = 0; j < WN; ++j) c[j] = __builtin_amdgcn_mfma_f32_16x16x32_bf16(a[0], b[j][1], c[j], 0, 0, 0);
#pragma unroll
            for (int j = 0; j < WN; ++j) c[j] = __builtin_amdgcn_mfma_f32_16x16x32_bf16(a[1], b[j][0], c[j], 0, 0, 0);
#pragma unroll
            for (int j = 0; j < WN; ++j) c[j] = __builtin_amdgcn_mfma_f32_16x16x32_bf16(a[0], b[j][0], c[j], 0, 0, 0);
        }
    };

    int nsteps[MAIN_MAX_SEG], total_steps = 0;
#pragma unroll
    for (int i = 0; i < MAIN_MAX_SEG; ++i) { nsteps[i] = i < NSEG ? (args.seg[i].klen + BK - 1) / BK : 0; total_steps += nsteps[i]; }
    constexpr bool ROWMAP = CFG::EPI == EPI_ROWMAP;
    static_assert(!ROWMAP || (K0 == MK_GATHER && K1 == MK_GATHER && NSEG == 2 && !DIST && !X6), "row map: two gathered segments");
    const int g0 = (int)((long long)total_steps * z / S), g1_all = (int)((long long)total_steps * (z + 1) / S);
    const int g1 = [&]() __attribute__((always_inline)) {
        if constexpr (ROWMAP) return m0 >= ((giptr)args.seg[0].idx)[M] ? min(g1_all, nsteps[0]) : g1_all;
        else return g1_all;
    }();

    f32x4 va[DEPTH][NA], vm[DEPTH][NA], vb[DEPTH][NB];
    typedef unsigned int bu32x4 __attribute__((ext_vector_type(4)));
    __amdgpu_buffer_rsrc_t rsPA = __builtin_amdgcn_make_buffer_rsrc((void*)nullptr, 0, 0, 0x00020000), rsPB = rsPA;
    unsigned roA[NA], roM[NA], roB[NB]; float lse[NA];
    float dacc[NA];
    constexpr int FOLD_DIST_OFF = 2 * (BML + BN) * P > 32 * (MT / 64) * 68 ? 2 * (BML + BN) * P : 32 * (MT / 64) * 68;
#pragma unroll
    for (int i = 0; i < NA; ++i) dacc[i] = 0.f;
    auto setup = [&](auto kind_c, const MainSeg& g) __attribute__((always_inline)) {
        constexpr int KIND = decltype(kind_c)::value;
#pragma unroll
        for (int i = 0; i < NA; ++i) {
            const int r = min(m0 + min(trow + RP * i, BM - 1), M - 1);
            constexpr bool GAT = KIND == MK_GATHER || KIND == MK_GATHER_MUL;
            const unsigned row = GAT ? (unsigned)((giptr)g.idx)[r] : (unsigned)r;
            roA[i] = row * (unsigned)(g.lda * 4);
            roM[i] = KIND == MK_GATHER_MUL ? (unsigned)((giptr)g.idx2)[r] * (unsigned)(g.lda * 4) : roA[i];
            lse[i] = KIND == MK_SOFTMAX ? ((gfptr)g.lse)[r] : 0.f;
        }
#pragma unroll
        for (int i = 0; i < NB; ++i) roB[i] = (unsigned)min(n0 + trow + RP * i, N - 1) * (unsigned)(g.ldb * 4) + 16u * quad;
        rsPA = __builtin_amdgcn_make_buffer_rsrc(const_cast<float*>(g.a), 0, 0xFFFFFFF0u, 0x00020000);
        rsPB = __builtin_amdgcn_make_buffer_rsrc(const_cast<float*>(g.b), 0, 0xFFFFFFF0u, 0x00020000);
    };
    auto issue = [&](auto set_c, auto mul_c, int klen, int nst, int t) __attribute__((always_inline)) {
        constexpr int S = decltype(set_c)::value;
        const int tk4 = min(t, nst - 1) * (BK * 4);
        const unsigned ca4 = (unsigned)min(tk4 + 16 * quad, (klen - 4) * 4);
#pragma unroll
        for (int i = 0; i < NA; ++i) va[S][i] = __builtin_bit_cast(f32x4, (bu32x4)__builtin_amdgcn_raw_buffer_load_b128(rsPA, roA[i] + ca4, 0, 0));
        if (decltype(mul_c)::value) {
#pragma unroll
            for (int i = 0; i < NA; ++i) vm[S][i] = __builtin_bit_cast(f32x4, (bu32x4)__builtin_amdgcn_raw_buffer_load_b128(rsPA, roM[i] + ca4, 0, 0));
        }
#pragma unroll
        for (int i = 0; i < NB; ++i) vb[S][i] = __builtin_bit_cast(f32x4, (bu32x4)__builtin_amdgcn_raw_buffer_load_b128(rsPB, roB[i], tk4, 0));
    };
    typedef IntC<0> S0; typedef IntC<DEPTH - 1> S1;
    typedef std::true_type Tt; typedef std::false_type Ff;

    auto run_seg = [&](auto idx_c, const int t0, const int t1, const bool pf_next) __attribute__((always_inline)) {
        constexpr int I = decltype(idx_c)::value;
        constexpr int KIND = KS[I], NKIND = KS[I + 1];
        constexpr int LKIND = KIND == MK_GATHER_MUL ? LK_MUL : KIND == MK_SOFTMAX ? LK_SOFTMAX : LK_PLAIN;
        typedef std::integral_constant<bool, LKIND == LK_MUL> MULC;
        const MainSeg& sg = args.seg[I];
        const int klen = sg.klen;
        const int nst = (klen + BK - 1) / BK;
        float lse_c[NA];
#pragma unroll
// ... 647 lines not shown
#pragma unroll
        for (int i = 0; i < WM; ++i)
#pragma unroll
            for (int j = 0; j < WN; ++j)
#pragma unroll
                for (int q = 0; q < 4; ++q) {
                    const int rho = wm0 + 16 * i + 4 * lk + q;
                    acc[i][j][q] = fc[(32 * (rho / 24) + rho % 24) * CP + wn0 + 16 * j + li];
                }
        __syncthreads();
      }
    };

    bool started = false;
    int base = 0;
    auto seg_pass = [&](auto idx_c) __attribute__((always_inline)) {
        constexpr int I = decltype(idx_c)::value;
        const int nst = nsteps[I];
        const int lo = min(max(g0 - base, 0), nst), hi = min(max(g1 - base, 0), nst);
        base += nst;
        if (lo < hi) {
            if (!started) {
                const MainSeg& g = args.seg[I];
                setup(IntC<KS[I]>{}, g);
                typedef std::integral_constant<bool, KS[I] == MK_GATHER_MUL> MI;
                issue(S0{}, MI{}, g.klen, nst, lo);
                if (DEPTH == 2) issue(S1{}, MI{}, g.klen, nst, lo + 1);
                started = true;
            }
            run_seg(idx_c, lo, hi, g1 > base);
        }
        stamp(1 + I);
    };
    if constexpr (VFOLD) {
        if constexpr (X6) {
            run_vfold6(args.seg[0], NSEG > 1);
            const mbf16x8 z8 = {0, 0, 0, 0, 0, 0, 0, 0};
#pragma unroll
            for (int q = 0; q < 2; ++q)
#pragma unroll
                for (int p = 0; p < 3; ++p) {
                    xa[q][p] = z8;
#pragma unroll
                    for (int j = 0; j < WN; ++j) xb[q][j][p] = z8;
                }
        }
        else if constexpr (BM % 96 == 0) run_vfold4(args.seg[0], NSEG > 1);
        else run_vfold(args.seg[0], NSEG > 1);
        base = nsteps[0]; started = true;
        stamp(1);
    } else {
        seg_pass(IntC<0>{});
    }
    if constexpr (NSEG > 1) seg_pass(IntC<1>{});
    if constexpr (NSEG > 2) seg_pass(IntC<2>{});
    if constexpr (NSEG > 3) seg_pass(IntC<3>{});
    if constexpr (NSEG > 4) seg_pass(IntC<4>{});
    if constexpr (!X6) mfma(afB, bfB);

    constexpr int SP = BN + 4;
    float* const stage = mf_smem;
    constexpr int QR = BN / 4;
    const EpiArgs& e = args.epi;
    float* const dst = S > 1 ? args.slab + (long long)z * M * N : args.out;
    const long long ldd = S > 1 ? (long long)N : args.ldo;
    const bool plain = S > 1 || !(e.rowadd || e.bias || e.relu || e.dropout || e.gate);
    auto item = [&](int f, int& r, int& n, int& nl) __attribute__((always_inline)) {
        const int rr = f / QR, cq = f - rr * QR;
        r = m0 + rr; n = n0 + 4 * cq;
        nl = min(n, N - 4 >= 0 ? N - 4 : 0);
        return rr * SP + 4 * cq;
    };
    auto win = [&](const float* p, int nl, int sh) __attribute__((always_inline)) {
        const f32x4 w = *(const f32x4u*)(p + nl);
        f32x4 o;
#pragma unroll
        for (int jj = 0; jj < 4; ++jj) { const int sj = jj + sh; o[jj] = sj == 0 ? w[0] : sj == 1 ? w[1] : sj == 2 ? w[2] : sj == 3 ? w[3] : 0.f; }
        return o;
    };
    const bool use_add = !plain && e.rowadd;
    const int rdiv = use_add ? e.rowdiv : 1;
    auto fetch_add = [&](int f) __attribute__((always_inline)) -> f32x4 {
        int r2, n2, nl2; item(f, r2, n2, nl2);
        const int n2c = min(n2, N - 1), nl2c = min(nl2, n2c);
        return win(e.rowadd + (long long)(min(r2, M - 1) / rdiv) * e.ld_rowadd, nl2c, n2c - nl2c);
    };
    constexpr int LAST_F = BM * QR - 1;
    f32x4 add0 = {0.f, 0.f, 0.f, 0.f}, add1 = add0, add2 = add0;
    if (use_add) { add0 = fetch_add(min(tid, LAST_F)); add1 = fetch_add(min(tid + MT, LAST_F)); add2 = fetch_add(min(tid + 2 * MT, LAST_F)); }
    int orow_v = 0;
    if constexpr (ROWMAP) orow_v = ((giptr)args.seg[0].idx)[min(m0 + min(tid, BM - 1), M - 1)];
#pragma unroll
    for (int i = 0; i < WM; ++i)
#pragma unroll
        for (int j = 0; j < WN; ++j)
#pragma unroll
            for (int q = 0; q < 4; ++q) stage[(wm0 + 16 * i + 4 * lk + q) * SP + wn0 + 16 * j + li] = acc[i][j][q];
    int* const orow = (int*)(stage + BM * SP);
    if constexpr (ROWMAP) {
        static_assert(!ROWMAP || (BM <= MT && (BM * SP + BM) * 4 <= CFG::LDS), "row map: one thread per tile row, table behind the staged tile");
        if (tid < BM) orow[tid] = orow_v;
    }
    __syncthreads();
#pragma unroll 1
    for (int f = tid; f < BM * QR; f += MT) {
        int r, n, nl;
        const int so = item(f, r, n, nl);
        const f32x4 addv = add0;
        add0 = add1; add1 = add2;
        if (use_add) add2 = fetch_add(min(f + 3 * MT, LAST_F));
        if (r >= M || n >= N) continue;
        f32x4 v = *(const f32x4*)(stage + so);
        const int sh = n - nl;
        if (!plain) {
            f32x4 add = addv, msk = {1.f, 1.f, 1.f, 1.f}, gte = {1.f, 1.f, 1.f, 1.f};
            if (e.bias) add += win(e.bias, nl, sh);
            if (e.dropout == 2) msk = win(e.keep_mask + (long long)r * e.ld_mask, nl, sh);
            if (e.gate) gte = win(e.gate + (long long)r * e.ld_gate, nl, sh);
#pragma unroll
            for (int jj = 0; jj < 4; ++jj) {
                float x = v[jj] + add[jj];
                if (e.relu == 1) x = x > 0.f ? x : 0.f;
                else if (e.relu == 2) x = tanhf(x);
                if (e.dropout == 1)
                    x = dropout_keep(e.seed_lo, e.seed_hi, e.layer, (unsigned long long)r * (unsigned)N + (unsigned)(n + jj), e.drop_p) ? x * e.drop_scale : 0.f;
                else if (e.dropout == 2)
                    x = msk[jj] != 0.f ? x * e.drop_scale : 0.f;
                if (e.gate) x = gte[jj] > 0.f ? x * e.gate_scale : 0.f;
                v[jj] = x;
            }
        }
        if constexpr (CFG::EPI == EPI_MLB) {
            const int g = e.rowsplit_g, b = r / g, jr = r - b * g;
            const f32x4 xq = win(e.fold_mul + (long long)b * e.ld_fold, nl, sh);
            v *= xq;
            const long long ro = jr == 0 ? (long long)b : (long long)b * (g - 1) + jr - 1;
            float* oz = (jr == 0 ? e.out0 + ro * e.ldo0 : args.out + ro * args.ldo) + n;
            if (n + 3 < N) *(f32x4u*)oz = v;
            else { oz[0] = v[0]; if (n + 1 < N) oz[1] = v[1]; if (n + 2 < N) oz[2] = v[2]; }
            if (args.t_out) {
                float* ot = (jr == 0 ? args.t_out0 : args.t_out) + ro * N + n;
                f32x4 t;
#pragma unroll
                for (int jj = 0; jj < 4; ++jj) t[jj] = tanhf(v[jj]);
                if (n + 3 < N) *(f32x4u*)ot = t;
                else { ot[0] = t[0]; if (n + 1 < N) ot[1] = t[1]; if (n + 2 < N) ot[2] = t[2]; }
            }
            continue;
        }
        float* o = dst + (long long)r * ldd + n;
        if constexpr (ROWMAP) o = dst + (long long)orow[f / QR] * ldd + n;
        if (n + 3 < N) *(f32x4u*)o = v;
        else { o[0] = v[0]; if (n + 1 < N) o[1] = v[1]; if (n + 2 < N) o[2] = v[2]; }
    }
    stamp(8);
    if (stamps && tid == 0) stamps[15] = __builtin_amdgcn_s_memrealtime();
}

__global__ __launch_bounds__(256) void k_main_fixup(const MainArgs a) {
    const int M = a.M, N = a.N, S = a.split;
    const int nq = (N + 3) / 4;
    const long long i = (long long)blockIdx.x * 256 + threadIdx.x;
    if (i >= (long long)M * nq) return;
    const int r = (int)(i / nq), n0 = (int)(i - (long long)r * nq) * 4;
    float v[4] = {0.f, 0.f, 0.f, 0.f};
    const long long mn = (long long)M * N, off = (long long)r * N + n0;
    for (int z = 0; z < S; ++z)
#pragma unroll
        for (int j = 0; j < 4; ++j) if (n0 + j < N) v[j] += a.slab[z * mn + off + j];
    const EpiArgs& e = a.epi;
#pragma unroll
    for (int j = 0; j < 4; ++j) {
        const int n = n0 + j;
        if (n >= N) break;
        a.out[(long long)r * a.ldo + n] = apply_epilogue(e, v[j], r, n, N);
    }
}

static inline bool main_fwd_operand_ok(int klen) { return klen >= 4 && klen % 4 == 0; }

template <int K0, int... REST> struct FirstKind { static constexpr int value = K0; };

template <class CFG, bool DIST, int... KINDS>
static inline int launch_main_fwd_seq(MainArgs& a, hipStream_t s) {
    constexpr int lds = FirstKind<KINDS...>::value == MK_VFOLD ? (CFG::LDS_FOLD > CFG::LDS ? CFG::LDS_FOLD : CFG::LDS) : CFG::LDS;
    static DevMask attr{0};
    NCX_HIP_TRY(set_max_lds_once(attr, (const void*)k_main_fwd<CFG, DIST, KINDS...>, lds));
    const int tiles_m = (a.M + CFG::BM - 1) / CFG::BM, tiles_n = (a.N + CFG::BN - 1) / CFG::BN;
    const int S = a.split > 1 ? a.split : 1;
    const int grid = ((tiles_m * S + 7) / 8) * 8 * tiles_n;
    hipLaunchKernelGGL((k_main_fwd<CFG, DIST, KINDS...>), dim3(grid), dim3(CFG::T), lds, s, a);
    NCX_HIP_TRY(hipGetLastError());
    if (S > 1) {
        const long long nthreads = (long long)a.M * ((a.N + 3) / 4);
        hipLaunchKernelGGL(k_main_fixup, dim3((unsigned)((nthreads + 255) / 256)), dim3(256), 0, s, a);
        NCX_HIP_TRY(hipGetLastError());
    }
    return NCX_OK;
}

template <class CFG>
static inline int launch_main_fwd(MainArgs& a, hipStream_t s) {
    if (a.nseg < 1 || a.nseg > MAIN_MAX_SEG || a.M < 1 || a.N < 1) return NCX_E_DIMS;
    for (int i = 0; i < a.nseg; ++i) if (!main_fwd_operand_ok(a.seg[i].klen)) return NCX_E_DIMS;
    if (a.epi.rowadd && a.epi.rowdiv < 3) return NCX_E_DIMS;
    if (a.split > 1 && !a.slab) return NCX_E_WORKSPACE;
    auto is = [&](std::initializer_list<int> ks) { if ((int)ks.size() != a.nseg) return false; int i = 0; for (int k : ks) if (a.seg[i++].kind != k) return false; return true; };
    constexpr int G = MK_GATHER, X = MK_GATHER_MUL, P = MK_PLAIN, S = MK_SOFTMAX;
    constexpr int V = MK_VFOLD;
    if constexpr (CFG::EPI == EPI_ROWMAP) {
        const EpiArgs& e = a.epi;
        if (!is({G, G}) || a.split > 1 || a.dist_out || !a.out || !a.seg[0].idx || a.seg[0].idx != a.seg[1].idx ||
            e.rowadd || e.bias || e.relu || e.dropout || e.gate)
            return NCX_E_FLAGS;
        return launch_main_fwd_seq<CFG, false, G, G>(a, s);
    } else
    if constexpr (CFG::EPI == EPI_MLB) {
        if (!is({G}) || a.split > 1 || a.dist_out || a.N < 4 || !a.epi.bias || !a.epi.fold_mul || a.epi.rowsplit_g < 2 || !a.epi.out0 ||
            !a.out || (a.t_out && !a.t_out0))
            return NCX_E_FLAGS;
        return launch_main_fwd_seq<CFG, false, G>(a, s);
    } else {
    if (a.seg[0].kind == V) {
        if constexpr (CFG::BM == 48 && CFG::BN == 64 && CFG::WGM == 1 && CFG::DEPTH == 2) {
            if (a.split > 1 || a.seg[0].klen % MF_BK || a.seg[0].klen < 2 * MF_BK || !a.epi.rowadd || a.epi.rowdiv != 24) return NCX_E_FLAGS;
            if (a.dist_out) {
                if (is({V, P, P, S})) return launch_main_fwd_seq<CFG, true, V, P, P, S>(a, s);
                if (is({V, P, P, P})) return launch_main_fwd_seq<CFG, true, V, P, P, P>(a, s);
            } else {
                if (is({V, P, P, S})) return launch_main_fwd_seq<CFG, false, V, P, P, S>(a, s);
                if (is({V, P, P, P})) return launch_main_fwd_seq<CFG, false, V, P, P, P>(a, s);
            }
        }
        if constexpr (CFG::BM % 96 == 0 && CFG::BN == 64 && CFG::WGM * CFG::WGN == CFG::T / 64 && CFG::DEPTH == 2) {
            if (a.split > 1 || a.seg[0].klen % MF_BK || a.seg[0].klen < 2 * MF_BK || !a.epi.rowadd || (a.epi.rowdiv != 24 && a.epi.rowdiv != 48))
                return NCX_E_FLAGS;
            if (a.dist_out) {
                if constexpr (CFG::X6) return NCX_E_FLAGS;
                else {
                    if (a.epi.rowdiv != 24) return NCX_E_FLAGS;
                    if (is({V, P, P, S})) return launch_main_fwd_seq<CFG, true, V, P, P, S>(a, s);
                    if (is({V, P, P, P})) return launch_main_fwd_seq<CFG, true, V, P, P, P>(a, s);
                    return NCX_E_FLAGS;
                }
            }
            if (is({V, P, P, S})) return launch_main_fwd_seq<CFG, false, V, P, P, S>(a, s);
            if (is({V, P, P, P})) return launch_main_fwd_seq<CFG, false, V, P, P, P>(a, s);
        }
        return NCX_E_FLAGS;
    }
    if constexpr (CFG::X6) return NCX_E_FLAGS;
    else {
    if (a.dist_out) {
        if (a.split > 1 || a.nseg < 3 || a.seg[1].klen % MF_BK) return NCX_E_FLAGS;
        if (is({G, X, P, P, S})) return launch_main_fwd_seq<CFG, true, G, X, P, P, S>(a, s);
        if (is({G, X, P, P, P})) return launch_main_fwd_seq<CFG, true, G, X, P, P, P>(a, s);
        return NCX_E_FLAGS;
    }
    if (is({G, X, P, P, S})) return launch_main_fwd_seq<CFG, false, G, X, P, P, S>(a, s);
    if (is({P}))             return launch_main_fwd_seq<CFG, false, P>(a, s);
    if (is({G}))             return launch_main_fwd_seq<CFG, false, G>(a, s);
    if (is({G, P, P, S}))    return launch_main_fwd_seq<CFG, false, G, P, P, S>(a, s);
    if (is({G, X, P, P, P})) return launch_main_fwd_seq<CFG, false, G, X, P, P, P>(a, s);
    if (is({G, P, P, P}))    return launch_main_fwd_seq<CFG, false, G, P, P, P>(a, s);
    if (is({P, P}))          return launch_main_fwd_seq<CFG, false, P, P>(a, s);
    return NCX_E_FLAGS;
    }
    }
}

}
```

### vqa-counterexamples_amd/csrc/ncx_main.hip

```cpp
#include "ncx_main.h"

namespace ncx {

typedef MainCfg<48, 128, 1, 4, 2, 2> MainCfg0;
typedef MainCfg<96, 64, 2, 2, 1, 2> MainCfg1;
typedef MainCfg<96, 128, 2, 2, 2, 1> MainCfg2;
typedef MainCfg<160, 128, 2, 2, 2, 1> MainCfgW;
typedef MainCfg<64, 64, 2, 2, 2, 3> MainCfg3;
typedef MainCfg<48, 64, 1, 4, 2, 2> MainCfgFold;
typedef MainCfg<96, 64, 2, 2, 2, 2> MainCfgFold4;
typedef MainCfg<192, 64, 4, 2, 2, 2, 512, true> MainCfgFold8X6;
typedef MainCfg<192, 64, 4, 2, 2, 2, 512> MainCfgFold8;

template <class C> using AsIs = C;
template <template <class> class W>
static int main_forward_chain(MainArgs& a, hipStream_t s) {
    long long T = 0;
    for (int i = 0; i < a.nseg; ++i) T += (a.seg[i].klen + MF_BK - 1) / MF_BK;
    if (a.split <= 1 && T <= 32 && (long long)((a.M + 63) / 64) * ((a.N + 63) / 64) >= 2 * num_cus() && !hook_env("NCX_MAIN_CFG"))
        return launch_main_fwd<W<MainCfg3>>(a, s);
    const long long tiles96 = (long long)((a.M + 95) / 96) * ((a.N + 127) / 128);
    constexpr bool wide_ok = W<MainCfgW>::EPI != EPI_ROWMAP;
    if constexpr (wide_ok)
    if (a.split <= 1 && a.nseg == 1 && a.seg[0].kind == MK_GATHER && !hook_env("NCX_MAIN_CFG")) {
        const long long cus = num_cus(), tiles160 = (long long)((a.M + 159) / 160) * ((a.N + 127) / 128);
        const double e96 = (double)tiles96 / (double)(((tiles96 + cus - 1) / cus) * cus), e160 = (double)tiles160 / (double)(((tiles160 + cus - 1) / cus) * cus);
        if (tiles160 * 10 >= cus * 7 && e160 > e96 + 0.1) return launch_main_fwd<W<MainCfgW>>(a, s);
    }
    int cfg = (a.split <= 1 && tiles96 * 10 >= (long long)num_cus() * 9) ? 2 : 0;
    if (const char* e = hook_env("NCX_MAIN_CFG")) cfg = atoi(e);
    if (cfg == 3) {
        if constexpr (wide_ok) return launch_main_fwd<W<MainCfgW>>(a, s);
        else return NCX_E_FLAGS;
    }
    if (cfg == 1) return launch_main_fwd<W<MainCfg1>>(a, s);
    if (cfg == 2) return launch_main_fwd<W<MainCfg2>>(a, s);
    return launch_main_fwd<W<MainCfg0>>(a, s);
}

int main_forward(MainArgs& a, hipStream_t s) {
    if (a.nseg > 0 && a.seg[0].kind == MK_VFOLD) {
        const int rows = main_fold_rows_eff(a.M, a.N, a.epi.rowdiv);
        if (rows == 192 && a.x6 && a.epi.rowdiv == 24) return launch_main_fwd<MainCfgFold8X6>(a, s);
        return rows == 192 ? launch_main_fwd<MainCfgFold8>(a, s) : rows == 96 ? launch_main_fwd<MainCfgFold4>(a, s) : launch_main_fwd<MainCfgFold>(a, s);
    }
    return main_forward_chain<AsIs>(a, s);
}

int main_forward_rowmap(MainArgs& a, hipStream_t s) {
    if (a.nseg != 2 || a.seg[0].kind != MK_GATHER) return NCX_E_FLAGS;
    return main_forward_chain<WithRowMap>(a, s);
}

int main_forward_mlb(MainArgs& a, hipStream_t s) {
    const long long tiles96 = (long long)((a.M + 95) / 96) * ((a.N + 127) / 128);
    if (tiles96 * 10 >= (long long)num_cus() * 9) return launch_main_fwd<WithMlbEpi<MainCfg2>>(a, s);
    return launch_main_fwd<WithMlbEpi<MainCfg0>>(a, s);
}

int main_fold_rows_eff(long long M, long long N, int rowdiv) {
    int rows = main_fold_rows(M, N);
    if (rowdiv == 48 && rows == 48) rows = 96;
    if (const char* f4 = hook_env("NCX_FOLD4")) rows = atoi(f4) != 0 ? 96 : (rowdiv == 48 ? 96 : 48);
    if (const char* f8 = hook_env("NCX_FOLD8")) rows = atoi(f8) != 0 ? 192 : (rows == 192 ? 96 : rows);
    return rows;
}

int main_fold_rows(long long M, long long N) {
    const long long cus = num_cus();
    const long long wg96 = ((M + 95) / 96) * ((N + 63) / 64), wg192 = ((M + 191) / 192) * ((N + 63) / 64);
    if (wg96 * 4 < cus * 2 * 3) return 48;
    const double e8 = (double)wg192 / (double)(((wg192 + cus - 1) / cus) * cus), e4 = (double)wg96 / (double)(((wg96 + 2 * cus - 1) / (2 * cus)) * 2 * cus);
    return e8 + 0.03 >= e4 ? 192 : 96;
}

int main_split(long long M, long long N, long long T) {
    const long long tiles = ((M + 47) / 48) * ((N + 127) / 128), cus = num_cus();
    if (tiles >= cus) return 1;
    long long S = 2 * cus / tiles;
    if (S > T / 8) S = T / 8;
    if (const char* e = hook_env("NCX_MAIN_SPLIT")) S = atoll(e);
    return (int)(S < 1 ? 1 : S);
}

}
```

### vqa-counterexamples_amd/neuralcx/_lib.py

```python
import ctypes as C
import os

_HERE = os.path.dirname(os.path.abspath(__file__))
LIB_PATH = os.environ.get("NCX_LIB") or os.path.join(os.path.dirname(_HERE), "lib", "libneuralcx_hip.so")

NCX_F_V_MULT, NCX_F_V_DIST, NCX_F_V_RANK, NCX_F_A_EMB = 1, 2, 4, 8
NCX_F_ALL = 15
NCX_F_REUSE_GT = 32
NCX_F_FUSED_TAIL = 64
NCX_F_X6 = 128
NCX_F_BF16 = 16

EXPORTS = ("ncx_input_size", "ncx_workspace_bytes", "ncx_forward", "ncx_forward_phase", "ncx_loss_rank", "ncx_backward", "ncx_backward_phase",
           "ncx_adam_step", "ncx_version", "ncx_profile_begin", "ncx_profile_end", "ncx_plan_query",
           "ncx_vqa_workspace_bytes", "ncx_vqa_forward", "ncx_mlb_workspace_bytes", "ncx_mlb_forward", "ncx_mlb_att_workspace_bytes", "ncx_mlb_att_forward", "ncx_mlb_att_forward_flags", "ncx_mlb_att_logits_form", "ncx_knn_workspace_bytes", "ncx_knn_status_offset", "ncx_knn", "ncx_cosine_gram_workspace_bytes", "ncx_cosine_gram", "ncx_semantic_scores",
           "ncx_similarity_scores",
           "ncx_gru_packed_bytes", "ncx_gru_pack", "ncx_gru_workspace_bytes", "ncx_gru_encode", "ncx_gru_encode_flags", "ncx_gru_step_form",
           "ncx_gru_train_workspace_bytes", "ncx_gru_packed_t_bytes", "ncx_gru_pack_t", "ncx_gru_train_forward", "ncx_gru_train_forward_flags", "ncx_gru_train_backward",
           "ncx_lstm2_packed_bytes", "ncx_lstm2_pack", "ncx_lstm2_workspace_bytes", "ncx_lstm2_encode",
           "ncx_lstm2_train_workspace_bytes", "ncx_lstm2_packed_t_bytes", "ncx_lstm2_pack_t", "ncx_lstm2_train_forward", "ncx_lstm2_train_backward",
           "ncx_ws_region", "ncx_wgmap_check",
           "ncx_comm_unique_id", "ncx_comm_create", "ncx_comm_destroy", "ncx_allreduce", "ncx_train_tail", "ncx_profile_stamps",
           "ncx_pairlin_workspace_bytes", "ncx_pairlin_forward", "ncx_pairlin_backward",
           "ncx_linctx_workspace_bytes", "ncx_linctx_forward", "ncx_linctx_backward",
           "ncx_contrastive_workspace_bytes", "ncx_contrastive_forward", "ncx_contrastive_distances", "ncx_contrastive_loss",
           "ncx_contrastive_backward",
           "ncx_vqa_train_workspace_bytes", "ncx_vqa_train_forward", "ncx_ce_loss", "ncx_vqa_train_backward", "ncx_vqa_train_ws_region",
           "ncx_mlb_train_workspace_bytes", "ncx_mlb_train_forward", "ncx_mlb_train_backward", "ncx_mlb_train_ws_region",
           "ncx_mlb_att_train_workspace_bytes", "ncx_mlb_att_train_forward", "ncx_mlb_att_train_forward_flags", "ncx_mlb_att_train_backward", "ncx_mlb_att_train_ws_region",
           "ncx_mlb_att_train_backward_flags", "ncx_mlb_att_dwv_form")


class NcxDims(C.Structure):
    _fields_ = [("B", C.c_int32), ("K", C.c_int32), ("dv", C.c_int32), ("dq", C.c_int32),
                ("dz", C.c_int32), ("da", C.c_int32), ("A", C.c_int32), ("H", C.c_int32),
                ("L", C.c_int32), ("n_img", C.c_int32), ("flags", C.c_uint32),
                ("training", C.c_int32), ("drop_p", C.c_float), ("loss_scale", C.c_float),
                ("seed", C.c_uint64)]


class NcxInputs(C.Structure):
    _fields_ = [(n, C.c_void_p) for n in ("feats", "img_idx", "q_emb", "z_orig", "z_knns", "a_knns",
                                           "answer_aids", "a_emb_gt", "v_rank", "keep_mask")]


_PNAMES = ("answer_embedding", "w1", "b1", "w2", "b2", "w3", "b3", "w_out", "b_out")


class NcxParams(C.Structure):
    _fields_ = [(n, C.c_void_p) for n in _PNAMES]


class NcxGrads(C.Structure):
    _fields_ = [(n, C.c_void_p) for n in _PNAMES]


class NcxMutanParams(C.Structure):
    _fields_ = [(n, C.c_void_p) for n in ("wv", "bv", "wq", "bq", "whv", "bhv", "whq", "bhq", "wc", "bc")] + \
               [(n, C.c_int32) for n in ("dhv", "dhq", "R", "act_v", "act_q")]


class NcxMutanGrads(C.Structure):
    _fields_ = [(n, C.c_void_p) for n in ("wv", "bv", "wq", "bq", "whv", "bhv", "whq", "bhq", "wc", "bc")]


class NcxVqaTrainDims(C.Structure):
    _fields_ = [(n, C.c_int32) for n in ("B", "dv", "dq", "dz", "A", "n_img")] + [(n, C.c_float) for n in ("p_v", "p_q", "p_c")] + \
               [("dropout_mode", C.c_int32), ("want_dq", C.c_int32), ("pad_", C.c_int32), ("seed", C.c_uint64)]


class NcxMlbParams(C.Structure):
    _fields_ = [(n, C.c_void_p) for n in ("wv", "bv", "wq", "bq", "wc", "bc")] + \
               [(n, C.c_int32) for n in ("dh", "act_v", "act_q", "act_c")]


class NcxMlbAttDims(C.Structure):
    _fields_ = [(n, C.c_int32) for n in ("B", "P", "dv", "dq", "dh_att", "G", "dh_f", "A", "n_img")]


class NcxMlbAttParams(C.Structure):
    _fields_ = [(n, C.c_void_p) for n in ("wv_att", "bv_att", "wq_att", "bq_att", "wa", "ba", "wg", "bg", "wqf", "bqf", "wc", "bc")] + \
               [(n, C.c_int32) for n in ("act_v_att", "act_q_att", "act_mm", "act_v", "act_q", "act_c")]


class NcxMlbAttTrain(C.Structure):
    _fields_ = [(n, C.c_float) for n in ("p_att_v", "p_att_q", "p_att_mm", "p_v", "p_q", "p_c")] + \
               [("dropout_mode", C.c_int32), ("want_dq", C.c_int32), ("seed", C.c_uint64)]


class NcxMlbAttGrads(C.Structure):
    _fields_ = [(n, C.c_void_p) for n in ("wv_att", "bv_att", "wq_att", "bq_att", "wa", "ba", "wg", "bg", "wqf", "bqf", "wc", "bc")]


class NcxMlbGrads(C.Structure):
    _fields_ = [(n, C.c_void_p) for n in ("wv", "bv", "wq", "bq", "wc", "bc")]


class NcxScorerDims(C.Structure):
    _fields_ = [(n, C.c_int32) for n in ("B", "K", "dv", "dq", "dz", "A", "n_img")]


class NcxContrastiveDims(C.Structure):
    _fields_ = [(n, C.c_int32) for n in ("B", "P", "dv", "dz", "n_img")]


_PL_NAMES = ("answer_embedding", "w", "b", "w_out", "b_out")


class NcxPairlinParams(C.Structure):
    _fields_ = [(n, C.c_void_p) for n in _PL_NAMES]


class NcxPairlinGrads(C.Structure):
    _fields_ = [(n, C.c_void_p) for n in _PL_NAMES]


class NcxError(RuntimeError):
    pass


_ERR = {-1: "NCX_E_NULL (required pointer is NULL)", -2: "NCX_E_DIMS (dimension out of range)",
        -3: "NCX_E_WORKSPACE (workspace too small or misaligned)", -4: "NCX_E_FLAGS (inconsistent lesion inputs)",
        -5: "NCX_E_UNSUPPORTED (RCCL could not be loaded)", -6: "NCX_E_COMM (RCCL reported an error)"}

_lib = None


def lib():
    global _lib
    if _lib is not None:
        return _lib
    if not os.path.exists(LIB_PATH):
        raise NcxError("HIP library not built: %s is missing. Run `python -c 'import __graft_entry__ as g; "
                       "g.build()'` or `make -C vqa-counterexamples_amd`." % LIB_PATH)
    import torch
    L = C.CDLL(LIB_PATH)
    L.ncx_version.restype = C.c_char_p
    L.ncx_input_size.restype = C.c_int64
    L.ncx_input_size.argtypes = [C.POINTER(NcxDims)]
    L.ncx_workspace_bytes.restype = C.c_size_t
    L.ncx_workspace_bytes.argtypes = [C.POINTER(NcxDims)]
    L.ncx_forward.restype = C.c_int
    L.ncx_forward.argtypes = [C.POINTER(NcxDims), C.POINTER(NcxInputs), C.POINTER(NcxParams), C.c_void_p,
                              C.c_size_t, C.c_void_p, C.c_void_p]
    L.ncx_forward_phase.restype = C.c_int
    L.ncx_forward_phase.argtypes = [C.POINTER(NcxDims), C.POINTER(NcxInputs), C.POINTER(NcxParams), C.c_void_p,
                                    C.c_size_t, C.c_void_p, C.c_int32, C.c_void_p]
    L.ncx_loss_rank.restype = C.c_int
    L.ncx_loss_rank.argtypes = [C.c_void_p, C.c_void_p, C.c_int32, C.c_int32, C.c_float, C.c_void_p,
                                C.c_void_p, C.c_void_p, C.c_void_p, C.c_void_p, C.c_void_p]
    L.ncx_backward.restype = C.c_int
    L.ncx_backward.argtypes = [C.POINTER(NcxDims), C.POINTER(NcxInputs), C.POINTER(NcxParams), C.c_void_p,
                               C.c_size_t, C.c_void_p, C.POINTER(NcxGrads), C.c_void_p]
    L.ncx_backward_phase.restype = C.c_int
    L.ncx_backward_phase.argtypes = [C.POINTER(NcxDims), C.POINTER(NcxInputs), C.POINTER(NcxParams), C.c_void_p,
                                     C.c_size_t, C.c_void_p, C.POINTER(NcxGrads), C.c_int32, C.c_void_p]
    L.ncx_adam_step.restype = C.c_int
    L.ncx_adam_step.argtypes = [C.c_void_p, C.c_void_p, C.c_void_p, C.c_void_p, C.c_size_t, C.c_float,
                                C.c_float, C.c_float, C.c_float, C.c_int32, C.c_float, C.c_void_p]
    L.ncx_vqa_workspace_bytes.restype = C.c_size_t
    L.ncx_vqa_workspace_bytes.argtypes = [C.POINTER(NcxDims), C.POINTER(NcxMutanParams)]
    L.ncx_vqa_forward.restype = C.c_int
    L.ncx_vqa_forward.argtypes = [C.POINTER(NcxDims), C.c_void_p, C.c_void_p, C.c_void_p, C.POINTER(NcxMutanParams), C.c_void_p,
                                  C.c_size_t, C.c_void_p, C.c_void_p, C.c_void_p, C.c_void_p, C.c_void_p]
    L.ncx_mlb_workspace_bytes.restype = C.c_size_t
    L.ncx_mlb_workspace_bytes.argtypes = [C.POINTER(NcxDims), C.POINTER(NcxMlbParams)]
    L.ncx_mlb_forward.restype = C.c_int
    L.ncx_mlb_forward.argtypes = [C.POINTER(NcxDims), C.c_void_p, C.c_void_p, C.c_void_p, C.POINTER(NcxMlbParams), C.c_void_p,
                                  C.c_size_t, C.c_void_p, C.c_void_p, C.c_void_p, C.c_void_p, C.c_void_p]
    L.ncx_mlb_att_workspace_bytes.restype = C.c_size_t
    L.ncx_mlb_att_workspace_bytes.argtypes = [C.POINTER(NcxMlbAttDims), C.POINTER(NcxMlbAttParams)]
    L.ncx_mlb_att_forward.restype = C.c_int
    L.ncx_mlb_att_forward.argtypes = [C.POINTER(NcxMlbAttDims), C.c_void_p, C.c_void_p, C.c_void_p, C.POINTER(NcxMlbAttParams), C.c_void_p,
                                      C.c_size_t, C.c_void_p, C.c_void_p, C.c_void_p]
    L.ncx_mlb_att_forward_flags.restype = C.c_int
    L.ncx_mlb_att_forward_flags.argtypes = [C.POINTER(NcxMlbAttDims), C.c_void_p, C.c_void_p, C.c_void_p, C.POINTER(NcxMlbAttParams), C.c_uint32,
                                            C.c_void_p, C.c_size_t, C.c_void_p, C.c_void_p, C.c_void_p]
    L.ncx_mlb_att_logits_form.restype = C.c_int
    L.ncx_mlb_att_logits_form.argtypes = [C.POINTER(NcxMlbAttDims), C.c_uint32]
    L.ncx_knn_workspace_bytes.restype = C.c_size_t
    L.ncx_knn_workspace_bytes.argtypes = [C.c_int32, C.c_int32]
    L.ncx_knn_status_offset.restype = C.c_size_t
    L.ncx_knn_status_offset.argtypes = [C.c_int32]
    L.ncx_knn.restype = C.c_int
    L.ncx_knn.argtypes = [C.c_void_p, C.c_int32, C.c_void_p, C.c_int32, C.c_int32, C.c_int32, C.c_int32, C.c_void_p,
                          C.c_size_t, C.c_void_p, C.c_void_p, C.c_void_p]
    L.ncx_cosine_gram_workspace_bytes.restype = C.c_size_t
    L.ncx_cosine_gram_workspace_bytes.argtypes = [C.c_int32, C.c_int32]
    L.ncx_cosine_gram.restype = C.c_int
    L.ncx_cosine_gram.argtypes = [C.c_void_p, C.c_int32, C.c_int32, C.c_void_p, C.c_size_t, C.c_void_p, C.c_void_p]
    L.ncx_semantic_scores.restype = C.c_int
    L.ncx_semantic_scores.argtypes = [C.c_void_p, C.c_void_p, C.c_int32, C.c_int32, C.c_int32, C.c_void_p, C.c_float,
                                      C.c_void_p, C.c_void_p, C.c_void_p, C.c_void_p]
    L.ncx_similarity_scores.restype = C.c_int
    L.ncx_similarity_scores.argtypes = [C.c_void_p, C.c_void_p, C.c_int32, C.c_int32, C.c_void_p, C.c_void_p, C.c_int32, C.c_void_p,
                                        C.c_void_p, C.c_int32, C.c_int32, C.c_int32, C.c_void_p, C.c_void_p, C.c_void_p, C.c_void_p]
    L.ncx_gru_packed_bytes.restype = C.c_size_t
    L.ncx_gru_packed_bytes.argtypes = [C.c_int32, C.c_int32]
    L.ncx_gru_pack.restype = C.c_int
    L.ncx_gru_pack.argtypes = [C.c_void_p, C.c_void_p, C.c_void_p, C.c_void_p, C.c_int32, C.c_int32, C.c_void_p, C.c_void_p]
    L.ncx_gru_workspace_bytes.restype = C.c_size_t
    L.ncx_gru_workspace_bytes.argtypes = [C.c_int32, C.c_int32, C.c_int32, C.c_int32]
    L.ncx_gru_encode.restype = C.c_int
    L.ncx_gru_encode.argtypes = [C.c_void_p, C.c_int32, C.c_int32, C.c_void_p, C.c_int32, C.c_int32, C.c_int32, C.c_void_p, C.c_void_p,
                                 C.c_size_t, C.c_void_p, C.c_void_p, C.c_void_p]
    L.ncx_gru_encode_flags.restype = C.c_int
    L.ncx_gru_encode_flags.argtypes = L.ncx_gru_encode.argtypes[:8] + [C.c_uint32] + L.ncx_gru_encode.argtypes[8:]
    L.ncx_gru_step_form.restype = C.c_int
    L.ncx_gru_step_form.argtypes = [C.c_int32, C.c_int32, C.c_int32, C.c_int32, C.c_uint32]
    L.ncx_gru_train_workspace_bytes.restype = C.c_size_t
    L.ncx_gru_train_workspace_bytes.argtypes = [C.c_int32, C.c_int32, C.c_int32, C.c_int32]
    L.ncx_gru_packed_t_bytes.restype = C.c_size_t
    L.ncx_gru_packed_t_bytes.argtypes = [C.c_int32, C.c_int32]
    L.ncx_gru_pack_t.restype = C.c_int
    L.ncx_gru_pack_t.argtypes = [C.c_void_p, C.c_void_p, C.c_int32, C.c_int32, C.c_void_p, C.c_void_p]
    L.ncx_gru_train_forward.restype = C.c_int
    L.ncx_gru_train_forward.argtypes = L.ncx_gru_encode.argtypes
    L.ncx_gru_train_forward_flags.restype = C.c_int
    L.ncx_gru_train_forward_flags.argtypes = L.ncx_gru_encode_flags.argtypes
    L.ncx_gru_train_backward.restype = C.c_int
    L.ncx_gru_train_backward.argtypes = [C.c_void_p, C.c_int32, C.c_int32, C.c_void_p, C.c_int32, C.c_int32, C.c_int32, C.c_void_p, C.c_void_p,
                                         C.c_size_t] + [C.c_void_p] * 7
    L.ncx_lstm2_packed_bytes.restype = C.c_size_t
    L.ncx_lstm2_packed_bytes.argtypes = [C.c_int32, C.c_int32]
    L.ncx_lstm2_pack.restype = C.c_int
    L.ncx_lstm2_pack.argtypes = [C.c_void_p] * 8 + [C.c_int32, C.c_int32, C.c_void_p, C.c_void_p]
    L.ncx_lstm2_workspace_bytes.restype = C.c_size_t
    L.ncx_lstm2_workspace_bytes.argtypes = [C.c_int32, C.c_int32, C.c_int32, C.c_int32]
    L.ncx_lstm2_encode.restype = C.c_int
    L.ncx_lstm2_encode.argtypes = L.ncx_gru_encode.argtypes
    L.ncx_lstm2_train_workspace_bytes.restype = C.c_size_t
    L.ncx_lstm2_train_workspace_bytes.argtypes = [C.c_int32, C.c_int32, C.c_int32, C.c_int32]
    L.ncx_lstm2_packed_t_bytes.restype = C.c_size_t
    L.ncx_lstm2_packed_t_bytes.argtypes = [C.c_int32, C.c_int32]
    L.ncx_lstm2_pack_t.restype = C.c_int
    L.ncx_lstm2_pack_t.argtypes = [C.c_void_p] * 4 + [C.c_int32, C.c_int32, C.c_void_p, C.c_void_p]
    L.ncx_lstm2_train_forward.restype = C.c_int
    L.ncx_lstm2_train_forward.argtypes = L.ncx_gru_encode.argtypes
    L.ncx_lstm2_train_backward.restype = C.c_int
    L.ncx_lstm2_train_backward.argtypes = [C.c_void_p, C.c_int32, C.c_int32, C.c_void_p, C.c_int32, C.c_int32, C.c_int32, C.c_void_p, C.c_void_p,
                                           C.c_size_t] + [C.c_void_p] * 11
    L.ncx_ws_region.restype = C.c_int
    L.ncx_ws_region.argtypes = [C.POINTER(NcxDims), C.c_int32, C.POINTER(C.c_size_t), C.POINTER(C.c_size_t)]
    L.ncx_profile_begin.restype = C.c_int
    L.ncx_profile_begin.argtypes = [C.c_uint32, C.c_int32]
    L.ncx_profile_end.restype = C.c_int
    L.ncx_profile_end.argtypes = [C.POINTER(C.c_float), C.POINTER(C.c_int32), C.c_int32]
    L.ncx_profile_stamps.restype = C.c_int
    L.ncx_profile_stamps.argtypes = [C.c_void_p, C.c_int64]
    L.ncx_train_tail.restype = C.c_int
    L.ncx_train_tail.argtypes = [C.POINTER(NcxDims), C.POINTER(NcxParams), C.c_void_p, C.c_size_t] + [C.c_void_p] * 7 + [C.POINTER(NcxGrads), C.c_void_p]
    L.ncx_comm_unique_id.restype = C.c_int; L.ncx_comm_unique_id.argtypes = [C.c_void_p]
    L.ncx_comm_create.restype = C.c_int; L.ncx_comm_create.argtypes = [C.c_void_p, C.c_int32, C.c_int32, C.POINTER(C.c_void_p)]
    L.ncx_comm_destroy.restype = C.c_int; L.ncx_comm_destroy.argtypes = [C.c_void_p]
    L.ncx_allreduce.restype = C.c_int; L.ncx_allreduce.argtypes = [C.c_void_p, C.c_void_p, C.c_size_t, C.c_void_p]
    L.ncx_plan_query.restype = C.c_int
    L.ncx_plan_query.argtypes = [C.POINTER(NcxDims), C.c_int32, C.POINTER(C.c_int32)]
    P_SD = C.POINTER(NcxScorerDims)
    L.ncx_pairlin_workspace_bytes.restype = C.c_size_t
    L.ncx_pairlin_workspace_bytes.argtypes = [P_SD]
    L.ncx_pairlin_forward.restype = C.c_int
    L.ncx_pairlin_forward.argtypes = [P_SD, C.POINTER(NcxInputs), C.POINTER(NcxPairlinParams), C.c_void_p, C.c_size_t,
                                      C.c_void_p, C.c_void_p, C.c_void_p]
    L.ncx_pairlin_backward.restype = C.c_int
    L.ncx_pairlin_backward.argtypes = [P_SD, C.POINTER(NcxInputs), C.POINTER(NcxPairlinParams), C.c_void_p, C.c_size_t,
                                       C.c_void_p, C.POINTER(NcxPairlinGrads), C.c_void_p]
    L.ncx_linctx_workspace_bytes.restype = C.c_size_t
    L.ncx_linctx_workspace_bytes.argtypes = [P_SD]
    L.ncx_linctx_forward.restype = C.c_int
    L.ncx_linctx_forward.argtypes = [P_SD, C.c_void_p, C.c_void_p, C.c_void_p, C.c_void_p, C.c_size_t, C.c_void_p, C.c_void_p]
    L.ncx_linctx_backward.restype = C.c_int
    L.ncx_linctx_backward.argtypes = [P_SD, C.c_void_p, C.c_void_p, C.c_void_p, C.c_size_t, C.c_void_p, C.c_void_p, C.c_void_p]
    P_CD = C.POINTER(NcxContrastiveDims)
    L.ncx_contrastive_workspace_bytes.restype = C.c_size_t
    L.ncx_contrastive_workspace_bytes.argtypes = [P_CD]
    L.ncx_contrastive_forward.restype = C.c_int
    L.ncx_contrastive_forward.argtypes = [P_CD, C.POINTER(NcxInputs), C.c_void_p, C.c_void_p, C.c_void_p, C.c_size_t, C.c_void_p,
                                          C.c_void_p, C.c_void_p]
    L.ncx_contrastive_distances.restype = C.c_int
    L.ncx_contrastive_distances.argtypes = [P_CD, C.c_void_p, C.c_void_p, C.c_size_t, C.c_void_p, C.c_void_p]
    L.ncx_contrastive_loss.restype = C.c_int
    L.ncx_contrastive_loss.argtypes = [P_CD, C.c_void_p, C.c_size_t, C.c_float, C.c_float, C.c_void_p, C.c_void_p, C.c_void_p]
    L.ncx_contrastive_backward.restype = C.c_int
    L.ncx_contrastive_backward.argtypes = [P_CD, C.POINTER(NcxInputs), C.c_void_p, C.c_size_t, C.c_void_p, C.c_void_p, C.c_void_p,
                                           C.c_void_p]
    P_VT, P_MP = C.POINTER(NcxVqaTrainDims), C.POINTER(NcxMutanParams)
    L.ncx_vqa_train_workspace_bytes.restype = C.c_size_t
    L.ncx_vqa_train_workspace_bytes.argtypes = [P_VT, P_MP]
    L.ncx_vqa_train_forward.restype = C.c_int
    L.ncx_vqa_train_forward.argtypes = [P_VT, C.c_void_p, C.c_void_p, C.c_void_p, P_MP, C.c_void_p, C.c_void_p, C.c_size_t, C.c_void_p,
                                        C.c_void_p, C.c_void_p]
    L.ncx_ce_loss.restype = C.c_int
    L.ncx_ce_loss.argtypes = [C.c_void_p, C.c_void_p, C.c_int32, C.c_int32, C.c_float] + [C.c_void_p] * 7
    L.ncx_vqa_train_backward.restype = C.c_int
    L.ncx_vqa_train_backward.argtypes = [P_VT, P_MP, C.c_void_p, C.c_void_p, C.c_size_t, C.c_void_p, C.POINTER(NcxMutanGrads), C.c_void_p,
                                         C.c_void_p]
    L.ncx_vqa_train_ws_region.restype = C.c_int
    L.ncx_vqa_train_ws_region.argtypes = [P_VT, P_MP, C.c_int32, C.POINTER(C.c_size_t), C.POINTER(C.c_size_t)]
    P_LP = C.POINTER(NcxMlbParams)
    L.ncx_mlb_train_workspace_bytes.restype = C.c_size_t
    L.ncx_mlb_train_workspace_bytes.argtypes = [P_VT, P_LP]
    L.ncx_mlb_train_forward.restype = C.c_int
    L.ncx_mlb_train_forward.argtypes = [P_VT, C.c_void_p, C.c_void_p, C.c_void_p, P_LP, C.c_void_p, C.c_void_p, C.c_size_t, C.c_void_p,
                                        C.c_void_p, C.c_void_p]
    L.ncx_mlb_train_backward.restype = C.c_int
    L.ncx_mlb_train_backward.argtypes = [P_VT, P_LP, C.c_void_p, C.c_void_p, C.c_size_t, C.c_void_p, C.POINTER(NcxMlbGrads), C.c_void_p,
                                         C.c_void_p]
    L.ncx_mlb_train_ws_region.restype = C.c_int
    L.ncx_mlb_train_ws_region.argtypes = [P_VT, P_LP, C.c_int32, C.POINTER(C.c_size_t), C.POINTER(C.c_size_t)]
    P_AD, P_AT, P_AP = C.POINTER(NcxMlbAttDims), C.POINTER(NcxMlbAttTrain), C.POINTER(NcxMlbAttParams)
    L.ncx_mlb_att_train_workspace_bytes.restype = C.c_size_t
    L.ncx_mlb_att_train_workspace_bytes.argtypes = [P_AD, P_AT, P_AP]
    L.ncx_mlb_att_train_forward.restype = C.c_int
    L.ncx_mlb_att_train_forward.argtypes = [P_AD, P_AT, C.c_void_p, C.c_void_p, C.c_void_p, P_AP, C.c_void_p, C.c_void_p, C.c_size_t,
                                            C.c_void_p, C.c_void_p, C.c_void_p]
    L.ncx_mlb_att_train_forward_flags.restype = C.c_int
    L.ncx_mlb_att_train_forward_flags.argtypes = [P_AD, P_AT, C.c_void_p, C.c_void_p, C.c_void_p, P_AP, C.c_void_p, C.c_uint32, C.c_void_p,
                                                  C.c_size_t, C.c_void_p, C.c_void_p, C.c_void_p]
    L.ncx_mlb_att_train_backward.restype = C.c_int
    L.ncx_mlb_att_train_backward.argtypes = [P_AD, P_AT, C.c_void_p, C.c_void_p, C.c_void_p, P_AP, C.c_void_p, C.c_void_p, C.c_size_t,
                                             C.c_void_p, C.c_void_p, C.POINTER(NcxMlbAttGrads), C.c_void_p, C.c_void_p]
    L.ncx_mlb_att_train_backward_flags.restype = C.c_int
    L.ncx_mlb_att_train_backward_flags.argtypes = [P_AD, P_AT, C.c_void_p, C.c_void_p, C.c_void_p, P_AP, C.c_void_p, C.c_uint32, C.c_void_p,
                                                   C.c_size_t, C.c_void_p, C.c_void_p, C.POINTER(NcxMlbAttGrads), C.c_void_p, C.c_void_p]
    L.ncx_mlb_att_dwv_form.restype = C.c_int
    L.ncx_mlb_att_dwv_form.argtypes = [P_AD, C.c_uint32]
    L.ncx_mlb_att_train_ws_region.restype = C.c_int
    L.ncx_mlb_att_train_ws_region.argtypes = [P_AD, P_AT, P_AP, C.c_int32, C.POINTER(C.c_size_t), C.POINTER(C.c_size_t)]
    _lib = L
    return L


def check(rc, what):
    if rc == 0:
        return
    if rc < 0:
        raise NcxError("%s failed: %s" % (what, _ERR.get(rc, rc)))
    raise NcxError("%s failed: hipError_t %d" % (what, rc))


def version():
    return lib().ncx_version().decode()


GEMM_IDS = dict(GT=0, SH=1, MAIN=2, FWD_L=3, DW1C=4, DW1S=5, DE=6, DW1AK=7, DAGT=8, DWL=9, DXL=10)


def profile_begin(names, max_launches=4096):
    mask = 0
    for n in names:
        mask |= 1 << GEMM_IDS[n]
    check(lib().ncx_profile_begin(mask, max_launches), "ncx_profile_begin")


def profile_end(cap=4096):
    ms = (C.c_float * cap)()
    ids = (C.c_int32 * cap)()
    n = lib().ncx_profile_end(ms, ids, cap)
    if n < 0:
        check(n, "ncx_profile_end")
    inv = {v: k for k, v in GEMM_IDS.items()}
    out = {}
    for i in range(n):
        out.setdefault(inv[ids[i]], []).append(float(ms[i]))
    return out


def profile_stamps(buf=None):
    if buf is None:
        check(lib().ncx_profile_stamps(None, 0), "ncx_profile_stamps")
    else:
        check(lib().ncx_profile_stamps(C.c_void_p(buf.data_ptr()), buf.numel()), "ncx_profile_stamps")


NCX_QUERY_DW1_ROUTE = 32
DW1_FOLD_FORMS = ("none", "k_dw_km8", "k_dw_km_x6", "k_dw_km", "grouped")
DW1_TN_FORMS = ("grouped", "k_dw_tn8", "k_dw_tn8_x6")


def plan_query(d, name):
    out = (C.c_int32 * 6)()
    if name == "DW1_ROUTE":
        check(lib().ncx_plan_query(C.byref(d), NCX_QUERY_DW1_ROUTE, out), "ncx_plan_query")
        return dict(fold=DW1_FOLD_FORMS[out[0]], tn=DW1_TN_FORMS[out[1]], tn_pieces=out[2], tn_grid=out[3],
                    a_other_on_tn=bool(out[4]), tn_max_pieces=out[5])
    check(lib().ncx_plan_query(C.byref(d), GEMM_IDS[name], out), "ncx_plan_query")
    return dict(form=("NT", "TN", "NN")[out[0]], M=out[1], N=out[2], ksteps=out[3],
                tile=("64x64", "128x128", "96x128", "96x64", "128x64", "48x128", "48x64 (per-triplet fold of the two v segments)",
                      "96x64 (per-triplet fold of the two v segments, four triplets per workgroup)",
                      "192x64 (per-triplet fold of the two v segments, eight triplets per 8-wave workgroup, one workgroup per CU)")[out[4]], ksplit=out[5])


def comm_unique_id() -> bytes:
    buf = C.create_string_buffer(128)
    check(lib().ncx_comm_unique_id(buf), "ncx_comm_unique_id")
    return buf.raw


def comm_create(unique_id: bytes, nranks: int, rank: int) -> C.c_void_p:
    if len(unique_id) != 128:
        raise ValueError("unique id must be the 128 bytes ncx_comm_unique_id produced on rank 0")
    comm = C.c_void_p()
    check(lib().ncx_comm_create(C.create_string_buffer(unique_id, 128), int(nranks), int(rank), C.byref(comm)), "ncx_comm_create")
    return comm


def allreduce(comm: C.c_void_p, t, stream_ptr=None) -> None:
    import torch
    if t.dtype != torch.float32 or not t.is_contiguous() or not t.is_cuda:
        raise TypeError("ncx_allreduce takes a contiguous fp32 device tensor")
    sp = torch.cuda.current_stream(t.device).cuda_stream if stream_ptr is None else stream_ptr
    check(lib().ncx_allreduce(comm, C.c_void_p(t.data_ptr()), t.numel(), C.c_void_p(sp)), "ncx_allreduce")


def comm_destroy(comm: C.c_void_p) -> None:
    check(lib().ncx_comm_destroy(comm), "ncx_comm_destroy")
```

### vqa-counterexamples_amd/neuralcx/engine.py

```python
import math
from typing import Dict, Optional

import torch

from . import dp, ops
from ._lib import NCX_F_ALL, NCX_F_A_EMB, NCX_F_BF16, NCX_F_FUSED_TAIL, NCX_F_REUSE_GT, NCX_F_X6

STATE_NAMES = ("answer_embedding.weight", "linear_1.weight", "linear_1.bias", "linear_2.weight", "linear_2.bias",
               "linear_3.weight", "linear_3.bias", "out.weight", "out.bias")


def param_shapes(K, dv, dq, dz, da, A, H, L):
    din = 3 * dv + 2 * da + 2 * dz + dq + K + 1
    s = {"answer_embedding.weight": (A, da), "linear_1.weight": (H, din), "linear_1.bias": (H,)}
    if L >= 2: s["linear_2.weight"] = (H, H); s["linear_2.bias"] = (H,)
    if L >= 3: s["linear_3.weight"] = (H, H); s["linear_3.bias"] = (H,)
    s["out.weight"] = (1, H); s["out.bias"] = (1,)
    return s


class FlatParams:

    def __init__(self, shapes: Dict[str, tuple], device):
        self.shapes = shapes
# ... 15 lines not shown
    def fields(self):
        return {ops.STATE_TO_FIELD[n]: v for n, v in self.views.items()}


class NeuralCXEngine:
    def __init__(self, K=24, dv=2048, dq=2400, dz=360, da=2400, A=2000, H=256, L=1, drop_p=0.25, lr=1e-4,
                 device="cuda:0", spec: Optional[dict] = None, world_size=1, process_group=None, bf16: bool = False, x6: bool = False):
        self.cfg = dict(K=K, dv=dv, dq=dq, dz=dz, da=da, A=A, H=H, L=L)
        self.drop_p, self.lr = drop_p, lr
        self.device = torch.device(device)
        self.flags = ops.flags_from_spec(spec) if spec is not None else NCX_F_ALL
        if bf16:
            if self.flags != NCX_F_ALL:
                raise ValueError("the bf16 variant supports the full model_spec only (no lesions)")
            self.flags |= NCX_F_BF16
        if x6:
            self.flags |= NCX_F_X6
        self.params = FlatParams(param_shapes(**self.cfg), self.device)
        self.grads = self.params.like()
        self.exp_avg = torch.zeros_like(self.params.flat)
        self.exp_avg_sq = torch.zeros_like(self.params.flat)
        self.step_count = 0
        self.world_size, self.pg = world_size, process_group
        self.fused_tail = True
        self._ws = None
        self._ws_key = None
        self.seed = 42
        self.rank = 0
        self._weights_version = 0
        self._gt_key = None
        self.comm_profile = False
        self.comm_events = []
        self.pipeline = True
        self._pending = None

    def init_parameters(self, seed=42, emb=None):
        self.flush()
        g = torch.Generator(device="cpu").manual_seed(seed)
        for n, v in self.params.views.items():
            if n == "answer_embedding.weight":
                t = torch.randn(v.shape, generator=g) if emb is None else torch.as_tensor(emb, dtype=torch.float32)
            else:
                fan_in = v.shape[1] if v.dim() == 2 else self.params.shapes[n.replace("bias", "weight")][1]
                b = 1.0 / math.sqrt(fan_in)
                t = (torch.rand(v.shape, generator=g) * 2 - 1) * b
            v.copy_(t)
        self._weights_version += 1

    def load_state(self, state: Dict[str, torch.Tensor]):
        self.flush()
        for n, v in self.params.views.items():
            v.copy_(state[n].to(self.device))
        self._weights_version += 1

    def state_dict(self):
        self.flush()
        return {n: v.detach().clone() for n, v in self.params.views.items()}

    def optimizer_state(self):
        self.flush()
        return {"exp_avg": self.exp_avg.detach().cpu(), "exp_avg_sq": self.exp_avg_sq.detach().cpu(), "step": self.step_count,
                "numel": self.params.numel}

    def load_optimizer_state(self, st):
        self.flush()
        if st["numel"] != self.params.numel:
            raise ValueError("optimizer state of another model (%d vs %d parameters)" % (st["numel"], self.params.numel))
        self.exp_avg.copy_(st["exp_avg"].to(self.device)); self.exp_avg_sq.copy_(st["exp_avg_sq"].to(self.device))
        self.step_count = int(st["step"])

    def _dims(self, batch: ops.Batch, training: bool, loss_scale: float):
        c = self.cfg
        d = ops.make_dims(batch, H=c["H"], L=c["L"], da=c["da"], A=c["A"], flags=self.flags, training=training,
                          drop_p=self.drop_p if training else 0.0, loss_scale=loss_scale,
                          seed=(self.seed << 32) ^ (self.rank << 24) ^ self.step_count)
        need = ops.workspace_bytes(d) + 256
        if self._ws is None or self._ws.numel() < need:
            self._ws = torch.empty(need, dtype=torch.uint8, device=self.device)
        return d

    def flush(self):
        if self._pending is None:
            return
        h2, step, ev = self._pending
        self._pending = None
        n_emb = self.params.offsets["linear_1.weight"]
        if ev: ev[2].record()
        h2.wait()
        if ev: ev[3].record(); self.comm_events.append(ev)
        ops.adam_step(self.params.flat[n_emb:], self.grads.flat[n_emb:], self.exp_avg[n_emb:], self.exp_avg_sq[n_emb:], step, lr=self.lr)

    def forward(self, batch: ops.Batch, training=False):
        self.flush()
        d = self._dims(batch, training, 0.0)
        key = (self._weights_version, self._ws.data_ptr(), d.B, d.K, d.H, d.A)
        if not training and (self.flags & NCX_F_A_EMB) and self._gt_key == key:
            d.flags |= NCX_F_REUSE_GT
        scores = ops.forward(d, batch, self.params.fields(), self._ws)
        self._gt_key = key
        return scores, d

    def eval_step(self, batch: ops.Batch, gt: torch.Tensor):
        scores, _ = self.forward(batch, training=False)
        r = ops.ranking_loss(scores, gt, want_grad=False)
        r["scores"] = scores
        return r

    def train_step(self, batch: ops.Batch, gt: torch.Tensor, global_batch: Optional[int] = None, active: bool = True):
        B = batch.img_idx.shape[0]
        gb = global_batch if global_batch is not None else B * self.world_size
        self.step_count += 1
        self._weights_version += 1
        d = self._dims(batch, True, 1.0 / gb)
        fused = active and self.fused_tail and ops.fused_tail_ok(d)
        if fused:
            d.flags |= NCX_F_FUSED_TAIL
        if self._pending is not None:
            ops.forward(d, batch, self.params.fields(), self._ws, phase=ops.FWD_PRELUDE)
            self.flush()
            scores = ops.forward(d, batch, self.params.fields(), self._ws, phase=ops.FWD_REST)
        else:
            scores = ops.forward(d, batch, self.params.fields(), self._ws)
        if fused:
            r = ops.train_tail(d, self.params.fields(), self._ws, scores, gt, self.grads.fields())
        else:
            r = ops.ranking_loss(scores, gt, scale=1.0 / gb)
        if not active:
            for k in ("dscores", "loss", "loss_rows", "hits"):
                r[k].zero_()
        if self.world_size > 1:
            n_emb = self.params.offsets["linear_1.weight"]
            f = self.params.fields()
            if self.flags & NCX_F_A_EMB:
                ops.backward(d, batch, f, self._ws, r["dscores"], self.grads.fields(), phase=5)
                h1 = torch.distributed.all_reduce(ops.ws_dgt_view(d, self._ws), group=self.pg, async_op=True)
                ops.backward(d, batch, f, self._ws, r["dscores"], self.grads.fields(), phase=2)
                h2 = torch.distributed.all_reduce(self.grads.flat[n_emb:], group=self.pg, async_op=True)
                ev = [torch.cuda.Event(enable_timing=True) for _ in range(4)] if self.comm_profile else None
                if ev: ev[0].record()
                h1.wait()
                if ev: ev[1].record()
                ops.backward(d, batch, f, self._ws, r["dscores"], self.grads.fields(), phase=4)
                ops.adam_step(self.params.flat[:n_emb], self.grads.flat[:n_emb], self.exp_avg[:n_emb], self.exp_avg_sq[:n_emb],
                              self.step_count, lr=self.lr)
                self._pending = (h2, self.step_count, ev)
                if not self.pipeline:
                    self.flush()
                r["scores"] = scores
                return r
            else:
                ops.backward(d, batch, f, self._ws, r["dscores"], self.grads.fields())
                torch.distributed.all_reduce(self.grads.flat[n_emb:], group=self.pg)
        else:
            ops.backward(d, batch, self.params.fields(), self._ws, r["dscores"], self.grads.fields())
        ops.adam_step(self.params.flat, self.grads.flat, self.exp_avg, self.exp_avg_sq, self.step_count, lr=self.lr)
        r["scores"] = scores
        return r


    def make_batch_from_vqa(self, feats, img_idx, q_emb, answer_aids, mutan_weights):
        _, z_o, a_k, z_k = ops.vqa_forward(feats, img_idx, q_emb, mutan_weights, want_a_orig=False)
        return ops.Batch(feats, img_idx, q_emb, z_o, z_k, a_k, answer_aids)
```

### vqa-counterexamples_amd/neuralcx/ops.py

```python
import ctypes as C
from dataclasses import dataclass
from typing import Dict, Optional

import torch

import os

from . import _lib
from ._lib import (NCX_F_A_EMB, NCX_F_ALL, NCX_F_V_DIST, NCX_F_V_MULT, NCX_F_V_RANK, NcxDims, NcxGrads,
                   NcxInputs, NcxMlbParams, NcxMutanParams, NcxParams)

PARAM_FIELDS = ("answer_embedding", "w1", "b1", "w2", "b2", "w3", "b3", "w_out", "b_out")
STATE_TO_FIELD = {"answer_embedding.weight": "answer_embedding", "linear_1.weight": "w1", "linear_1.bias": "b1",
                  "linear_2.weight": "w2", "linear_2.bias": "b2", "linear_3.weight": "w3", "linear_3.bias": "b3",
                  "out.weight": "w_out", "out.bias": "b_out"}


def flags_from_spec(spec: Optional[dict]) -> int:
    if spec is None:
        return NCX_F_ALL
    f = 0
    if spec.get("v_mult", True): f |= NCX_F_V_MULT
    if spec.get("v_dist", True): f |= NCX_F_V_DIST
    if spec.get("v_rank", True): f |= NCX_F_V_RANK
# ... 42 lines not shown
        s.feats = _ptr(self.feats, torch.float32, "feats")
        s.img_idx = _ptr(self.img_idx, torch.int32, "img_idx")
        s.q_emb = _ptr(self.q_emb, torch.float32, "q_emb")
        s.z_orig = _ptr(self.z_orig, torch.float32, "z_orig")
        s.z_knns = _ptr(self.z_knns, torch.float32, "z_knns")
        s.a_knns = _ptr(self.a_knns, torch.float32, "a_knns")
        s.answer_aids = _ptr(self.answer_aids, torch.int32, "answer_aids")
        s.a_emb_gt = _ptr(self.a_emb_gt, torch.float32, "a_emb_gt")
        s.v_rank = _ptr(self.v_rank, torch.float32, "v_rank")
        s.keep_mask = _ptr(self.keep_mask, torch.float32, "keep_mask")
        return s


EXTRA_FLAGS = _lib.NCX_F_X6 if os.environ.get("NCX_X6", "0") not in ("", "0") else 0


def make_dims(batch: Batch, H: int, L: int, da: int, A: int, flags: int = NCX_F_ALL, training: bool = False,
              drop_p: float = 0.0, loss_scale: float = 0.0, seed: int = 0) -> NcxDims:
    B, K1 = batch.img_idx.shape
    d = NcxDims()
    d.B, d.K = B, K1 - 1
    d.dv, d.dq, d.dz = batch.feats.shape[1], batch.q_emb.shape[1], batch.z_orig.shape[1]
    d.da, d.A, d.H, d.L = da, A, H, L
    d.n_img = batch.feats.shape[0]
    d.flags, d.training, d.drop_p, d.loss_scale, d.seed = flags | EXTRA_FLAGS, int(training), float(drop_p), float(loss_scale), int(seed) & (2 ** 64 - 1)
    K = d.K
    assert batch.z_knns.shape == (B, K, d.dz), batch.z_knns.shape
    assert batch.q_emb.shape[0] == B and batch.z_orig.shape == (B, d.dz)
    if flags & NCX_F_A_EMB:
        assert batch.a_knns.shape == (B, K, A), (batch.a_knns.shape, (B, K, A))
        assert batch.answer_aids is not None and batch.answer_aids.shape == (B,)
    else:
        assert batch.a_knns.shape == (B, K, da) and batch.a_emb_gt is not None and batch.a_emb_gt.shape == (B, da)
    if not (flags & NCX_F_V_RANK):
        assert batch.v_rank is not None and batch.v_rank.shape == (B, K, K)
    if batch.keep_mask is not None:
        assert batch.keep_mask.shape == (L, B * K, H)
    return d


def _params_struct(params: Dict[str, torch.Tensor], cls):
    s = cls()
    for f in PARAM_FIELDS:
        setattr(s, f, _ptr(params.get(f), torch.float32, f))
    return s


def workspace_bytes(d: NcxDims) -> int:
    n = _lib.lib().ncx_workspace_bytes(C.byref(d))
    if n == 0:
        raise _lib.NcxError("ncx_workspace_bytes: invalid dims")
    return n


def alloc_workspace(d: NcxDims, device) -> torch.Tensor:
    return torch.empty(workspace_bytes(d) + 256, dtype=torch.uint8, device=device)


def _ws_ptr(ws: torch.Tensor):
    base = ws.data_ptr()
    aligned = (base + 255) // 256 * 256
    return C.c_void_p(aligned), ws.numel() - (aligned - base)


def fused_tail_ok(d: NcxDims) -> bool:
    return d.K <= 32 and d.H <= 256


def train_tail(d: NcxDims, params: Dict[str, torch.Tensor], ws: torch.Tensor, scores: torch.Tensor, gt: torch.Tensor,
               grads: Dict[str, torch.Tensor], want_dscores: bool = False):
    dev = scores.device
    loss_rows = torch.empty(d.B, dtype=torch.float32, device=dev)
    loss = torch.empty(1, dtype=torch.float32, device=dev)
    dscores = torch.empty_like(scores) if want_dscores else None
    rank = torch.empty(d.B, dtype=torch.int32, device=dev)
    hits = torch.empty(2, dtype=torch.int32, device=dev)
    p, n = _ws_ptr(ws)
    ps, gs = _params_struct(params, NcxParams), _params_struct(grads, NcxGrads)
    _lib.check(_lib.lib().ncx_train_tail(C.byref(d), C.byref(ps), p, n, _ptr(gt, torch.int32, "gt"), C.c_void_p(scores.data_ptr()),
                                         C.c_void_p(loss_rows.data_ptr()), C.c_void_p(loss.data_ptr()),
                                         _ptr(dscores, torch.float32, "dscores"), C.c_void_p(rank.data_ptr()),
                                         C.c_void_p(hits.data_ptr()), C.byref(gs), _stream()), "ncx_train_tail")
    return dict(loss=loss, loss_rows=loss_rows, dscores=dscores, rank=rank, hits=hits)


FWD_ALL, FWD_PRELUDE, FWD_REST = 0, 1, 2


def forward(d: NcxDims, batch: Batch, params: Dict[str, torch.Tensor], ws: torch.Tensor, phase: int = FWD_ALL) -> Optional[torch.Tensor]:
    p, n = _ws_ptr(ws)
    ins, ps = batch.c_struct(), _params_struct(params, NcxParams)
    if phase == FWD_PRELUDE:
        _lib.check(_lib.lib().ncx_forward_phase(C.byref(d), C.byref(ins), C.byref(ps), p, n, None, FWD_PRELUDE, _stream()), "ncx_forward_phase")
        return None
    scores = torch.empty(d.B, d.K, dtype=torch.float32, device=batch.feats.device)
    if phase == FWD_ALL:
        _lib.check(_lib.lib().ncx_forward(C.byref(d), C.byref(ins), C.byref(ps), p, n,
                                          C.c_void_p(scores.data_ptr()), _stream()), "ncx_forward")
    else:
        _lib.check(_lib.lib().ncx_forward_phase(C.byref(d), C.byref(ins), C.byref(ps), p, n,
                                                C.c_void_p(scores.data_ptr()), int(phase), _stream()), "ncx_forward_phase")
    return scores


def backward(d: NcxDims, batch: Batch, params: Dict[str, torch.Tensor], ws: torch.Tensor, dscores: torch.Tensor,
             grads: Dict[str, torch.Tensor], phase: int = 0) -> None:
    p, n = _ws_ptr(ws)
    ins, ps, gs = batch.c_struct(), _params_struct(params, NcxParams), _params_struct(grads, NcxGrads)
    if phase == 0:
        _lib.check(_lib.lib().ncx_backward(C.byref(d), C.byref(ins), C.byref(ps), p, n,
                                           _ptr(dscores, torch.float32, "dscores"), C.byref(gs), _stream()), "ncx_backward")
    else:
        _lib.check(_lib.lib().ncx_backward_phase(C.byref(d), C.byref(ins), C.byref(ps), p, n,
                                                 _ptr(dscores, torch.float32, "dscores"), C.byref(gs), int(phase), _stream()),
                   "ncx_backward_phase")


def ws_dgt_view(d: NcxDims, ws: torch.Tensor) -> torch.Tensor:
    off, nbytes = C.c_size_t(0), C.c_size_t(0)
    _lib.check(_lib.lib().ncx_ws_region(C.byref(d), 1, C.byref(off), C.byref(nbytes)), "ncx_ws_region")
    base = (ws.data_ptr() + 255) // 256 * 256 - ws.data_ptr()
    return ws[base + off.value: base + off.value + nbytes.value].view(torch.float32)


def ws_de_perm_view(d: NcxDims, ws: torch.Tensor) -> torch.Tensor:
    off, nbytes = C.c_size_t(0), C.c_size_t(0)
    _lib.check(_lib.lib().ncx_ws_region(C.byref(d), 4, C.byref(off), C.byref(nbytes)), "ncx_ws_region")
    base = (ws.data_ptr() + 255) // 256 * 256 - ws.data_ptr()
    return ws[base + off.value: base + off.value + nbytes.value].view(torch.int32)


def ranking_loss(scores: torch.Tensor, gt: torch.Tensor, scale: float = 0.0, want_grad: bool = True):
    B, K = scores.shape
    dev = scores.device
    loss_rows = torch.empty(B, dtype=torch.float32, device=dev)
    loss = torch.empty(1, dtype=torch.float32, device=dev)
    dscores = torch.empty_like(scores) if want_grad else None
    rank = torch.empty(B, dtype=torch.int32, device=dev)
    hits = torch.empty(2, dtype=torch.int32, device=dev)
    _lib.check(_lib.lib().ncx_loss_rank(_ptr(scores, torch.float32, "scores"), _ptr(gt, torch.int32, "gt"), B, K,
                                        float(scale), C.c_void_p(loss_rows.data_ptr()), C.c_void_p(loss.data_ptr()),
                                        _ptr(dscores, torch.float32, "dscores"), C.c_void_p(rank.data_ptr()),
                                        C.c_void_p(hits.data_ptr()), _stream()), "ncx_loss_rank")
    return dict(loss=loss, loss_rows=loss_rows, dscores=dscores, rank=rank, hits=hits)


def adam_step(param, grad, exp_avg, exp_avg_sq, step, lr=1e-4, betas=(0.9, 0.999), eps=1e-8, grad_scale=1.0):
    n = param.numel()
    assert grad.numel() == n and exp_avg.numel() == n and exp_avg_sq.numel() == n
    _lib.check(_lib.lib().ncx_adam_step(_ptr(param, torch.float32, "param"), _ptr(grad, torch.float32, "grad"),
                                        _ptr(exp_avg, torch.float32, "exp_avg"), _ptr(exp_avg_sq, torch.float32, "exp_avg_sq"),
                                        n, lr, betas[0], betas[1], eps, int(step), float(grad_scale), _stream()),
               "ncx_adam_step")


class MutanWeights:

    def __init__(self, vqa_model):
        f, opt = vqa_model.fusion, vqa_model.opt["fusion"]
        for k in ("activation_hv", "activation_hq", "activation_mm"):
            if k in opt:
                raise _lib.NcxError("ncx_vqa_forward supports the options/cx/*.yaml MUTAN (no %s)" % k)
        if "activation" in vqa_model.opt.get("classif", {}):
            raise _lib.NcxError("ncx_vqa_forward: classif.activation is not supported")
        act = {None: 0, "tanh": 2}
        if opt.get("activation_v") not in act or opt.get("activation_q") not in act:
            raise _lib.NcxError("ncx_vqa_forward supports activation_v/q in {none, tanh}")
        c = lambda t: t.detach().float().contiguous()
        self.t = dict(wv=c(f.linear_v.weight), bv=c(f.linear_v.bias), wq=c(f.linear_q.weight), bq=c(f.linear_q.bias),
                      whv=c(torch.cat([l.weight for l in f.list_linear_hv])), bhv=c(torch.cat([l.bias for l in f.list_linear_hv])),
                      whq=c(torch.cat([l.weight for l in f.list_linear_hq])), bhq=c(torch.cat([l.bias for l in f.list_linear_hq])),
                      wc=c(vqa_model.linear_classif.weight), bc=c(vqa_model.linear_classif.bias))
        self.dhv, self.dhq, self.R, self.dz = opt["dim_hv"], opt["dim_hq"], opt["R"], opt["dim_mm"]
        self.A = self.t["wc"].shape[0]
        self.act_v, self.act_q = act[opt.get("activation_v")], act[opt.get("activation_q")]

    @classmethod
    def from_tensors(cls, t: Dict[str, torch.Tensor], R: int, act_v: int = 2, act_q: int = 2):
        self = cls.__new__(cls)
        self.t = dict(t)
        self.dhv, self.dhq, self.R = t["wv"].shape[0], t["wq"].shape[0], int(R)
        self.A, self.dz = t["wc"].shape
        self.act_v, self.act_q = int(act_v), int(act_q)
        return self

    def c_struct(self):
        m = NcxMutanParams()
        for k, v in self.t.items():
            setattr(m, k, _ptr(v, torch.float32, k))
        m.dhv, m.dhq, m.R, m.act_v, m.act_q = self.dhv, self.dhq, self.R, self.act_v, self.act_q
        return m


class MlbWeights:
    WS_BYTES, FORWARD = "ncx_mlb_workspace_bytes", "ncx_mlb_forward"

    def __init__(self, vqa_model):
        f, opt = vqa_model.fusion, vqa_model.opt["fusion"]
        for k in ("dim_v", "dim_q", "dim_h"):
            if k not in opt:
                raise _lib.NcxError("ncx_mlb_forward needs fusion.%s (a block that passes an input through is not supported)" % k)
        act = {None: 0, "tanh": 2}
        acts = (opt.get("activation_v"), opt.get("activation_q"), vqa_model.opt.get("classif", {}).get("activation"))
        for name, a in zip(("fusion.activation_v", "fusion.activation_q", "classif.activation"), acts):
            if a not in act:
                raise _lib.NcxError("ncx_mlb_forward supports %s in {none, tanh}, got %r" % (name, a))
        c = lambda t: t.detach().float().contiguous()
        self.t = dict(wv=c(f.linear_v.weight), bv=c(f.linear_v.bias), wq=c(f.linear_q.weight), bq=c(f.linear_q.bias),
                      wc=c(vqa_model.linear_classif.weight), bc=c(vqa_model.linear_classif.bias))
        self.dz = opt["dim_h"]
        self.A = self.t["wc"].shape[0]
        self.act_v, self.act_q, self.act_c = (act[a] for a in acts)

    @classmethod
    def from_tensors(cls, t: Dict[str, torch.Tensor], act_v: int = 2, act_q: int = 2, act_c: int = 2):
        self = cls.__new__(cls)
        self.t = dict(t)
        self.A, self.dz = t["wc"].shape
        self.act_v, self.act_q, self.act_c = int(act_v), int(act_q), int(act_c)
        return self

    def c_struct(self):
        m = NcxMlbParams()
        for k, v in self.t.items():
            setattr(m, k, _ptr(v, torch.float32, k))
        m.dh, m.act_v, m.act_q, m.act_c = self.dz, self.act_v, self.act_q, self.act_c
        return m


def vqa_weights(vqa_model):
    from vqa.models.fusion import MLBFusion
    return MlbWeights(vqa_model) if isinstance(vqa_model.fusion, MLBFusion) else MutanWeights(vqa_model)


def vqa_forward(feats: torch.Tensor, img_idx: torch.Tensor, q_emb: torch.Tensor, mw, want_a_orig=False, ws=None):
    B, K1 = img_idx.shape
    d = NcxDims()
    d.B, d.K, d.dv, d.dq, d.dz, d.da, d.A, d.H, d.L = B, K1 - 1, feats.shape[1], q_emb.shape[1], mw.dz, 4, mw.A, 4, 1
    d.n_img = feats.shape[0]
    m = mw.c_struct()
    ws_name, fwd_name = getattr(mw, "WS_BYTES", "ncx_vqa_workspace_bytes"), getattr(mw, "FORWARD", "ncx_vqa_forward")
    need = getattr(_lib.lib(), ws_name)(C.byref(d), C.byref(m))
    if need == 0:
        raise _lib.NcxError("%s: invalid dims" % ws_name)
    if ws is None or ws.numel() < need + 256:
        ws = torch.empty(need + 256, dtype=torch.uint8, device=feats.device)
    dev = feats.device
    z_o = torch.empty(B, mw.dz, device=dev); z_k = torch.empty(B, K1 - 1, mw.dz, device=dev)
    a_k = torch.empty(B, K1 - 1, mw.A, device=dev)
    a_o = torch.empty(B, mw.A, device=dev) if want_a_orig else None
    p, n = _ws_ptr(ws)
    _lib.check(getattr(_lib.lib(), fwd_name)(C.byref(d), _ptr(feats, torch.float32, "feats"), _ptr(img_idx, torch.int32, "img_idx"),
                                             _ptr(q_emb, torch.float32, "q_emb"), C.byref(m), p, n, C.c_void_p(z_o.data_ptr()),
                                             C.c_void_p(z_k.data_ptr()), C.c_void_p(a_k.data_ptr()),
                                             C.c_void_p(a_o.data_ptr()) if a_o is not None else None, _stream()), fwd_name)
    return a_o, z_o, a_k, z_k


MLB_ATT_FIELDS = ("wv_att", "bv_att", "wq_att", "bq_att", "wa", "ba", "wg", "bg", "wqf", "bqf", "wc", "bc")
MLB_ATT_ACTS = ("act_v_att", "act_q_att", "act_mm", "act_v", "act_q", "act_c")


def mlb_att_acts(opt) -> Optional[Dict[str, int]]:
    att, fus, cla = opt["attention"], opt["fusion"], opt.get("classif", {})
    names = (att.get("activation_v"), att.get("activation_q"), att.get("activation_mm"), fus.get("activation_v"), fus.get("activation_q"),
             cla.get("activation"))
    code = {None: 0, "tanh": 2}
    if any(a not in code for a in names):
        return None
    return {k: code[a] for k, a in zip(MLB_ATT_ACTS, names)}


class MlbAttWeights:

    def __init__(self, model):
        acts = mlb_att_acts(model.opt)
        if acts is None:
            raise _lib.NcxError("ncx_mlb_att_forward supports activations in {none, tanh}")
        c = lambda t: t.detach().float().contiguous()
        lin = list(model.list_linear_v_fusion)
        self.t = dict(wv_att=c(model.conv_v_att.weight.flatten(1)), bv_att=c(model.conv_v_att.bias),
                      wq_att=c(model.linear_q_att.weight), bq_att=c(model.linear_q_att.bias),
                      wa=c(model.conv_att.weight.flatten(1)), ba=c(model.conv_att.bias),
                      wg=c(torch.stack([l.weight for l in lin])), bg=c(torch.stack([l.bias for l in lin])),
                      wqf=c(model.linear_q_fusion.weight), bqf=c(model.linear_q_fusion.bias),
                      wc=c(model.linear_classif.weight), bc=c(model.linear_classif.bias))
        self.acts = acts
        self._set_dims()

    @classmethod
    def from_tensors(cls, t: Dict[str, torch.Tensor], **acts):
        self = cls.__new__(cls)
        self.t = dict(t)
        self.acts = {k: int(acts.get(k, 2)) for k in MLB_ATT_ACTS}
        self._set_dims()
        return self

    def _set_dims(self):
        t = self.t
        self.dh_att, self.dv = t["wv_att"].shape
        self.dq = t["wq_att"].shape[1]
        self.G, self.dh_f = t["wg"].shape[:2]
        self.A = t["wc"].shape[0]
        want = dict(wv_att=(self.dh_att, self.dv), bv_att=(self.dh_att,), wq_att=(self.dh_att, self.dq), bq_att=(self.dh_att,),
                    wa=(self.G, self.dh_att), ba=(self.G,), wg=(self.G, self.dh_f, self.dv), bg=(self.G, self.dh_f),
                    wqf=(self.G * self.dh_f, self.dq), bqf=(self.G * self.dh_f,), wc=(self.A, self.G * self.dh_f), bc=(self.A,))
# ... 1063 lines not shown
```

Before: 656,900 triplets/s.

## Fuse Adam update into the final backward answer-embedding GEMM kernel

Adds ncx_backward_adam, which runs the optimizer inside the last backward GEMM launch (the answer-embedding gradient pass). The GEMM epilogue applies Adam to the embedding parameters, and extra 'passenger' workgroups in the same grid update the remaining MLP parameters. This removes the separate Adam kernel launch and a re-read of the embedding gradient, and lets the small parameter update overlap with the GEMM tiles. If the fused route is not eligible, it falls back to the standalone Adam kernel. The Adam arithmetic is also rewritten with explicit FMAs, which may change rounding slightly.

After: 664,800 triplets/s, median of 6. +1.2%, better.

```diff
diff --git a/include/neuralcx.h b/include/neuralcx.h
--- a/include/neuralcx.h
+++ b/include/neuralcx.h
@@ -118,6 +118,16 @@
 int ncx_adam_step(float* param, const float* grad, float* exp_avg, float* exp_avg_sq, size_t n,
                   float lr, float beta1, float beta2, float eps, int32_t step, float grad_scale,
                   void* stream);
+
+typedef struct ncx_adam_state {
+    float* param; const float* grad; float* exp_avg; float* exp_avg_sq;
+    size_t n, n_emb;
+    int32_t step;
+    float lr, beta1, beta2, eps, grad_scale;
+} ncx_adam_state;
+int ncx_backward_adam(const ncx_dims* d, const ncx_inputs* in, const ncx_params* p,
+                      void* workspace, size_t workspace_bytes, const float* dscores,
+                      const ncx_grads* g, const ncx_adam_state* opt, void* stream);
 
 typedef struct ncx_mutan_params {
     const float* wv;  const float* bv;
@@ -349,6 +359,7 @@
 #define NCX_GEMM_DWL 9
 #define NCX_GEMM_DXL 10
 #define NCX_QUERY_DW1_ROUTE 32
+#define NCX_QUERY_FUSED_ADAM 33
 int ncx_profile_begin(uint32_t gemm_mask , int32_t max_launches);
 int ncx_profile_end(float* ms, int32_t* ids, int32_t cap);
 int ncx_profile_stamps(unsigned long long* stamps, int64_t words);
diff --git a/vqa-counterexamples_amd/csrc/ncx_adam.h b/vqa-counterexamples_amd/csrc/ncx_adam.h
--- /dev/null
+++ b/vqa-counterexamples_amd/csrc/ncx_adam.h
@@ -0,0 +1,78 @@
+#pragma once
+#include "ncx_gemm.h"
+#include <math.h>
+
+namespace ncx {
+
+struct AdamScalars { float step_size, b1, b2, eps, inv_bc2_sqrt, gscale; };
+
+static inline AdamScalars adam_scalars(float lr, float beta1, float beta2, float eps, int step, float grad_scale) {
+    const double bc1 = 1.0 - pow((double)beta1, (double)step);
+    const double bc2 = 1.0 - pow((double)beta2, (double)step);
+    AdamScalars s;
+    s.step_size = (float)((double)lr / bc1);
+    s.inv_bc2_sqrt = (float)(1.0 / sqrt(bc2));
+    s.b1 = beta1; s.b2 = beta2; s.eps = eps; s.gscale = grad_scale;
+    return s;
+}
+
+template <bool VFMA = true>
+__device__ __forceinline__ void adam_update(float& p, const float g, float& m, float& v, const float step_size, const float b1, const float b2,
+                                            const float eps, const float inv_bc2_sqrt, const float gscale) {
+#pragma clang fp contract(off)
+    const float gj = g * gscale;
+    const float d = __builtin_fmaf(g, gscale, -m);
+    m = __builtin_fmaf(1.f - b1, d, m);
+    const float u = gj * ((1.f - b2) * gj);
+    if (VFMA) v = __builtin_fmaf(b2, v, u);
+    else v = b2 * v + u;
+    const float den = __builtin_fmaf(inv_bc2_sqrt, sqrtf(v), eps);
+    p = __builtin_fmaf(-step_size, m / den, p);
+}
+
+__device__ __forceinline__ void adam_quad(float* __restrict__ p, const float* __restrict__ g, float* __restrict__ m, float* __restrict__ v,
+                                          const size_t i, const AdamScalars& s) {
+    f32x4 pv = *(f32x4*)(p + i), mv = *(f32x4*)(m + i), vv = *(f32x4*)(v + i);
+    const f32x4 gv = *(const f32x4*)(g + i);
+#pragma unroll
+    for (int j = 0; j < 4; ++j) {
+        float pj = pv[j], mj = mv[j], vj = vv[j];
+        adam_update(pj, gv[j], mj, vj, s.step_size, s.b1, s.b2, s.eps, s.inv_bc2_sqrt, s.gscale);
+        pv[j] = pj; mv[j] = mj; vv[j] = vj;
+    }
+    *(f32x4*)(p + i) = pv; *(f32x4*)(m + i) = mv; *(f32x4*)(v + i) = vv;
+}
+
+__device__ __forceinline__ void adam_tail(float* __restrict__ p, const float* __restrict__ g, float* __restrict__ m, float* __restrict__ v,
+                                          const size_t i, const size_t n, const AdamScalars& s) {
+    const size_t paired = i + ((n - i) & ~(size_t)1);
+    for (size_t j = i; j < n; ++j) {
+        float pj = p[j], mj = m[j], vj = v[j];
+        if (j < paired) adam_update<true>(pj, g[j], mj, vj, s.step_size, s.b1, s.b2, s.eps, s.inv_bc2_sqrt, s.gscale);
+        else adam_update<false>(pj, g[j], mj, vj, s.step_size, s.b1, s.b2, s.eps, s.inv_bc2_sqrt, s.gscale);
+        m[j] = mj; v[j] = vj; p[j] = pj;
+    }
+}
+
+struct AdamFuse {
+    float* p; float* m; float* v;
+    float* tp; const float* tg; float* tm; float* tv;
+    unsigned long long tn;
+    int n_pass, pass_at;
+    AdamScalars s;
+};
+
+__device__ __forceinline__ void adam_passenger(const AdamFuse& a, const int w, const int tid, const int nthreads) {
+    const size_t n = a.tn, quads = (n + 3) / 4, per = (quads + a.n_pass - 1) / a.n_pass;
+    const size_t q0 = (size_t)w * per, q1 = q0 + per < quads ? q0 + per : quads;
+    for (size_t q = q0 + tid; q < q1; q += nthreads) {
+        const size_t i = q * 4;
+        if (i + 3 < n) adam_quad(a.tp, a.tg, a.tm, a.tv, i, a.s);
+        else adam_tail(a.tp, a.tg, a.tm, a.tv, i, n, a.s);
+    }
+}
+
+__attribute__((visibility("hidden"))) int adam_launch(float* param, const float* grad, float* exp_avg, float* exp_avg_sq, size_t n,
+                                                      const AdamScalars& s, hipStream_t stream);
+
+}
diff --git a/vqa-counterexamples_amd/csrc/ncx_backward.hip b/vqa-counterexamples_amd/csrc/ncx_backward.hip
--- a/vqa-counterexamples_amd/csrc/ncx_backward.hip
+++ b/vqa-counterexamples_amd/csrc/ncx_backward.hip
@@ -406,6 +406,14 @@
     if (i >= (long long)rows * cols) return;
     const int r = (int)(i / cols), c = (int)(i - (long long)r * cols);
     p[(long long)r * ld + c] = 0.f;
+}
+}
+
+namespace ncx {
+bool fused_adam_route(const ncx_dims& d, const StepRoutes& r) {
+    if (!(d.flags & NCX_F_A_EMB) || (d.flags & NCX_F_BF16) || !r.emb_nt) return false;
+    if (km_defers_to_side_stream(d, r) || hook_env("NCX_NO_FUSED_ADAM")) return false;
+    return main_short_form(d.A, d.da, 2 * cdiv(pad_to(d.H, 4), GEMM_BK), 1);
 }
 }
 
@@ -460,7 +468,8 @@
 }
 
 static int backward_impl(const ncx_dims* dp, const ncx_inputs* in, const ncx_params* p, void* workspace,
-                         size_t workspace_bytes, const float* dscores, const ncx_grads* g, void* stream_, int phase) {
+                         size_t workspace_bytes, const float* dscores, const ncx_grads* g, void* stream_, int phase,
+                         const AdamFuse* adam = nullptr, bool* adam_done = nullptr) {
     int rc = check_dims(dp);
     if (rc != NCX_OK) return rc;
     if (!in || !p || !workspace || !g || (!dscores && !(dp->flags & NCX_F_FUSED_TAIL))) return NCX_E_NULL;
@@ -708,7 +717,13 @@
                 a.seg[0].kind = MK_GATHER; a.seg[0].idx = de_perm;
                 a.seg[1].kind = MK_GATHER; a.seg[1].idx = de_perm;
             }
+            if (adam && phase == 0 && !ss) {
+                a.adam = *adam;
+                rc = profiled(U_DE, se, [&] { return main_forward_adam(a, de_skip, se); }); if (rc) return rc;
+                if (adam_done) *adam_done = true;
+            } else {
             rc = profiled(U_DE, se, [&] { return de_skip ? main_forward_rowmap(a, se) : main_forward(a, se); }); if (rc) return rc;
+            }
         } else if ((do1 && !skip_de) || only_de) {
             GemmArgs a{}; a.mode = MODE_CHAIN; a.nseg = 2; a.M = d.A;
             a.a[0] = x_plain(dgt, d.A, H, d.A);  a.b[0] = x_plain(p->w1 + o.a_other, din, H, d.da); a.klen[0] = H;
@@ -727,6 +742,42 @@
 int ncx_backward(const ncx_dims* dp, const ncx_inputs* in, const ncx_params* p, void* workspace,
                  size_t workspace_bytes, const float* dscores, const ncx_grads* g, void* stream_) {
     return backward_impl(dp, in, p, workspace, workspace_bytes, dscores, g, stream_, 0);
+}
+
+int ncx_backward_adam(const ncx_dims* dp, const ncx_inputs* in, const ncx_params* p, void* workspace, size_t workspace_bytes,
+                      const float* dscores, const ncx_grads* g, const ncx_adam_state* opt, void* stream_) {
+    int rc = check_dims(dp);
+    if (rc != NCX_OK) return rc;
+    if (!in || !p || !g || !opt || !opt->param || !opt->grad || !opt->exp_avg || !opt->exp_avg_sq) return NCX_E_NULL;
+    if (!p->answer_embedding || !g->answer_embedding) return NCX_E_NULL;
+    const ncx_dims& d = *dp;
+    const size_t n = opt->n, n_emb = opt->n_emb, emb = (size_t)d.A * d.da;
+    if (opt->step < 1 || n == 0 || n_emb > n || n_emb < emb) return NCX_E_DIMS;
+    if (((uintptr_t)opt->param | (uintptr_t)opt->grad | (uintptr_t)opt->exp_avg | (uintptr_t)opt->exp_avg_sq) & 15) return NCX_E_WORKSPACE;
+    if (p->answer_embedding != opt->param || g->answer_embedding != opt->grad) return NCX_E_DIMS;
+    const SegOffsets o = seg_offsets(d);
+    const size_t H = (size_t)d.H;
+    auto inside = [&](const float* x, const float* base, size_t count) { return !x || (x >= base + n_emb && x + count <= base + n); };
+    const float* const pf[8] = {p->w1, p->b1, p->w2, p->b2, p->w3, p->b3, p->w_out, p->b_out};
+    const float* const gf[8] = {g->w1, g->b1, g->w2, g->b2, g->w3, g->b3, g->w_out, g->b_out};
+    const size_t cnt[8] = {H * (size_t)o.din, H, H * H, H, H * H, H, H, 1};
+    for (int i = 0; i < 8; ++i) {
+        const bool used = i < 2 || i >= 6 || (d.L >= 2 && i < 4) || d.L >= 3;
+        if (!used) continue;
+        if (!inside(pf[i], opt->param, cnt[i]) || !inside(gf[i], opt->grad, cnt[i])) return NCX_E_DIMS;
+    }
+    const AdamScalars sc = adam_scalars(opt->lr, opt->beta1, opt->beta2, opt->eps, opt->step, opt->grad_scale);
+    AdamFuse af{};
+    const bool want = fused_adam_route(d, routes(d)) && n_emb == emb && emb % 4 == 0;
+    if (want) {
+        af.p = opt->param; af.m = opt->exp_avg; af.v = opt->exp_avg_sq;
+        af.tp = opt->param + n_emb; af.tg = opt->grad + n_emb; af.tm = opt->exp_avg + n_emb; af.tv = opt->exp_avg_sq + n_emb;
+        af.tn = n - n_emb; af.s = sc;
+    }
+    bool done = false;
+    rc = backward_impl(dp, in, p, workspace, workspace_bytes, dscores, g, stream_, 0, want ? &af : nullptr, &done);
+    if (rc != NCX_OK || done) return rc;
+    return adam_launch(opt->param, opt->grad, opt->exp_avg, opt->exp_avg_sq, n, sc, (hipStream_t)stream_);
 }
 
 int ncx_backward_phase(const ncx_dims* dp, const ncx_inputs* in, const ncx_params* p, void* workspace,
diff --git a/vqa-counterexamples_amd/csrc/ncx_diag.hip b/vqa-counterexamples_amd/csrc/ncx_diag.hip
--- a/vqa-counterexamples_amd/csrc/ncx_diag.hip
+++ b/vqa-counterexamples_amd/csrc/ncx_diag.hip
@@ -77,6 +77,13 @@
         out6[5] = TN8_MAX_SEG;
         return NCX_OK;
     }
+    if (gemm_id == NCX_QUERY_FUSED_ADAM) {
+        const bool on = fused_adam_route(*d, routes(*d)) && ((size_t)d->A * d->da) % 4 == 0;
+        for (int i = 0; i < 6; ++i) out6[i] = 0;
+        out6[0] = on ? 1 : 0;
+        out6[1] = on ? main_adam_passengers() : 0;
+        return NCX_OK;
+    }
     if (gemm_id < 0 || gemm_id >= U_COUNT) return NCX_E_DIMS;
     GemmUse u[U_COUNT];
     list_uses(*d, routes(*d), u);
diff --git a/vqa-counterexamples_amd/csrc/ncx_driver.h b/vqa-counterexamples_amd/csrc/ncx_driver.h
--- a/vqa-counterexamples_amd/csrc/ncx_driver.h
+++ b/vqa-counterexamples_amd/csrc/ncx_driver.h
@@ -9,6 +9,7 @@
 int side_fork(SideStream* ss, hipStream_t main);
 int side_join(SideStream* ss, hipStream_t main);
 bool km_defers_to_side_stream(const ncx_dims& d, const StepRoutes& r);
+bool fused_adam_route(const ncx_dims& d, const StepRoutes& r);
 
 struct ProfState { bool on; unsigned mask; int n, cap; hipEvent_t* ev; int* ids; };
 extern ProfState g_prof;
diff --git a/vqa-counterexamples_amd/csrc/ncx_internal.h b/vqa-counterexamples_amd/csrc/ncx_internal.h
--- a/vqa-counterexamples_amd/csrc/ncx_internal.h
+++ b/vqa-counterexamples_amd/csrc/ncx_internal.h
@@ -1,6 +1,7 @@
 #pragma once
 #include "ncx_common.h"
 #include "ncx_gemm.h"
+#include "ncx_adam.h"
 
 namespace ncx {
 
@@ -96,9 +97,13 @@
     unsigned long long* stamps;
     int x6;
     float* t_out; float* t_out0;
+    AdamFuse adam;
 };
 int main_forward(MainArgs& a, hipStream_t s);
 int main_forward_rowmap(MainArgs& a, hipStream_t s);
+bool main_short_form(long long M, long long N, long long T, int split);
+int main_forward_adam(MainArgs& a, bool rowmap, hipStream_t s);
+int main_adam_passengers();
 int main_forward_mlb(MainArgs& a, hipStream_t s);
 int main_split(long long M, long long N, long long T);
 int main_fold_rows_eff(long long M, long long N, int rowdiv);
diff --git a/vqa-counterexamples_amd/csrc/ncx_loss_adam.hip b/vqa-counterexamples_amd/csrc/ncx_loss_adam.hip
--- a/vqa-counterexamples_amd/csrc/ncx_loss_adam.hip
+++ b/vqa-counterexamples_amd/csrc/ncx_loss_adam.hip
@@ -1,4 +1,5 @@
 #include "ncx_wave.h"
+#include "ncx_adam.h"
 
 namespace ncx {
 __global__ __launch_bounds__(256) void k_loss_rank(const float* __restrict__ scores, const int* __restrict__ gt,
@@ -43,32 +44,21 @@
 }
 
 __global__ __launch_bounds__(256) void k_adam(float* __restrict__ p, const float* __restrict__ g, float* __restrict__ m,
-                                              float* __restrict__ v, size_t n, float step_size, float b1, float b2,
-                                              float eps, float inv_bc2_sqrt, float gscale) {
+                                              float* __restrict__ v, size_t n, const AdamScalars s) {
     size_t i = ((size_t)blockIdx.x * 256 + threadIdx.x) * 4;
     const size_t stride = (size_t)gridDim.x * 256 * 4;
     for (; i < n; i += stride) {
-        if (i + 3 < n) {
-            f32x4 pv = *(f32x4*)(p + i), gv = *(const f32x4*)(g + i), mv = *(f32x4*)(m + i), vv = *(f32x4*)(v + i);
-#pragma unroll
-            for (int j = 0; j < 4; ++j) {
-                const float gj = gv[j] * gscale;
-                mv[j] = mv[j] + (gj - mv[j]) * (1.f - b1);
-                vv[j] = vv[j] * b2 + (1.f - b2) * gj * gj;
-                const float den = sqrtf(vv[j]) * inv_bc2_sqrt + eps;
-                pv[j] = pv[j] - step_size * (mv[j] / den);
-            }
-            *(f32x4*)(p + i) = pv; *(f32x4*)(m + i) = mv; *(f32x4*)(v + i) = vv;
-        } else {
-            for (size_t j = i; j < n; ++j) {
-                const float gj = g[j] * gscale;
-                const float mj = m[j] + (gj - m[j]) * (1.f - b1);
-                const float vj = v[j] * b2 + (1.f - b2) * gj * gj;
-                m[j] = mj; v[j] = vj;
-                p[j] = p[j] - step_size * (mj / (sqrtf(vj) * inv_bc2_sqrt + eps));
-            }
-        }
+        if (i + 3 < n) adam_quad(p, g, m, v, i, s);
+        else adam_tail(p, g, m, v, i, n, s);
     }
+}
+
+int adam_launch(float* param, const float* grad, float* exp_avg, float* exp_avg_sq, size_t n, const AdamScalars& s, hipStream_t stream) {
+    size_t blocks = (n + 1023) / 1024;
+    if (blocks > 4096) blocks = 4096;
+    hipLaunchKernelGGL(k_adam, dim3((unsigned)blocks), dim3(256), 0, stream, param, grad, exp_avg, exp_avg_sq, n, s);
+    NCX_HIP_TRY(hipGetLastError());
+    return NCX_OK;
 }
 }
 
@@ -95,15 +85,6 @@
     if (!param || !grad || !exp_avg || !exp_avg_sq) return NCX_E_NULL;
     if (step < 1 || n == 0) return NCX_E_DIMS;
     if (((uintptr_t)param | (uintptr_t)grad | (uintptr_t)exp_avg | (uintptr_t)exp_avg_sq) & 15) return NCX_E_WORKSPACE;
-    const double bc1 = 1.0 - pow((double)beta1, (double)step);
-    const double bc2 = 1.0 - pow((double)beta2, (double)step);
-    const float step_size = (float)((double)lr / bc1);
-    const float inv_bc2_sqrt = (float)(1.0 / sqrt(bc2));
-    size_t blocks = (n + 1023) / 1024;
-    if (blocks > 4096) blocks = 4096;
-    hipLaunchKernelGGL(k_adam, dim3((unsigned)blocks), dim3(256), 0, (hipStream_t)stream_, param, grad, exp_avg, exp_avg_sq, n,
-                       step_size, beta1, beta2, eps, inv_bc2_sqrt, grad_scale);
-    NCX_HIP_TRY(hipGetLastError());
-    return NCX_OK;
+    return adam_launch(param, grad, exp_avg, exp_avg_sq, n, adam_scalars(lr, beta1, beta2, eps, step, grad_scale), (hipStream_t)stream_);
 }
 }
diff --git a/vqa-counterexamples_amd/csrc/ncx_main.h b/vqa-counterexamples_amd/csrc/ncx_main.h
--- a/vqa-counterexamples_amd/csrc/ncx_main.h
+++ b/vqa-counterexamples_amd/csrc/ncx_main.h
@@ -1,5 +1,6 @@
 #pragma once
 #include "ncx_internal.h"
+#include "ncx_adam.h"
 #include <type_traits>
 
 namespace ncx {
@@ -15,6 +16,7 @@
     static constexpr int BM = BM_, BN = BN_, WGM = WGM_, WGN = WGN_, DEPTH = DEPTH_, OCC = OCC_, T = T_;
     static constexpr bool X6 = X6_;
     static constexpr int EPI = 0;
+    static constexpr bool ADAM = false;
     static constexpr int RP = T / 8;
     static constexpr int BM_LDS = (BM + RP - 1) / RP * RP;
     static constexpr int LDS6 = 2 * 3 * (BM_LDS + BN) * MF6_P;
@@ -28,6 +30,7 @@
 enum { EPI_STD = 0, EPI_MLB = 1, EPI_ROWMAP = 2 };
 template <class CFG> struct WithMlbEpi : CFG { static constexpr int EPI = EPI_MLB; };
 template <class CFG> struct WithRowMap : CFG { static constexpr int EPI = EPI_ROWMAP; };
+template <class CFG> struct WithAdam : CFG { static constexpr bool ADAM = true; };
 
 typedef const __attribute__((address_space(1))) float* gfptr;
 typedef const __attribute__((address_space(1))) int* giptr;
@@ -58,7 +61,13 @@
     const int M = args.M, N = args.N;
     const int tiles_m = (M + BM - 1) / BM, tiles_n = (N + BN - 1) / BN;
     const int S = args.split > 1 ? args.split : 1;
-    const int id = blockIdx.x, xcd = id & 7, local = id >> 3;
+    int bid = blockIdx.x;
+    if constexpr (CFG::ADAM) {
+        const int pa = args.adam.pass_at, np = args.adam.n_pass;
+        if (bid >= pa && bid < pa + np) { adam_passenger(args.adam, bid - pa, tid, MT); return; }
+        if (bid >= pa + np) bid -= np;
+    }
+    const int id = bid, xcd = id & 7, local = id >> 3;
     const int tn = local % tiles_n, unit = (local / tiles_n) * 8 + xcd;
     if (unit >= tiles_m * S) return;
     const int tm = unit / S, z = unit - tm * S;
@@ -1012,6 +1021,29 @@
         if constexpr (ROWMAP) o = dst + (long long)orow[f / QR] * ldd + n;
         if (n + 3 < N) *(f32x4u*)o = v;
         else { o[0] = v[0]; if (n + 1 < N) o[1] = v[1]; if (n + 2 < N) o[2] = v[2]; }
+        if constexpr (CFG::ADAM) {
+            const AdamFuse& ad = args.adam;
+            const long long off = o - dst;
+            float* const pp = ad.p + off; float* const pm = ad.m + off; float* const pv = ad.v + off;
+            if (n + 3 < N) {
+                f32x4 p4 = *(const f32x4u*)pp, m4 = *(const f32x4u*)pm, v4 = *(const f32x4u*)pv;
+#pragma unroll
+                for (int jj = 0; jj < 4; ++jj) {
+                    float pj = p4[jj], mj = m4[jj], vj = v4[jj];
+                    adam_update(pj, v[jj], mj, vj, ad.s.step_size, ad.s.b1, ad.s.b2, ad.s.eps, ad.s.inv_bc2_sqrt, ad.s.gscale);
+                    p4[jj] = pj; m4[jj] = mj; v4[jj] = vj;
+                }
+                *(f32x4u*)pp = p4; *(f32x4u*)pm = m4; *(f32x4u*)pv = v4;
+            } else {
+#pragma unroll
+                for (int jj = 0; jj < 3; ++jj) {
+                    if (n + jj >= N) break;
+                    float pj = pp[jj], mj = pm[jj], vj = pv[jj];
+                    adam_update(pj, v[jj], mj, vj, ad.s.step_size, ad.s.b1, ad.s.b2, ad.s.eps, ad.s.inv_bc2_sqrt, ad.s.gscale);
+                    pp[jj] = pj; pm[jj] = mj; pv[jj] = vj;
+                }
+            }
+        }
     }
     stamp(8);
     if (stamps && tid == 0) stamps[15] = __builtin_amdgcn_s_memrealtime();
@@ -1043,6 +1075,7 @@
 
 template <class CFG, bool DIST, int... KINDS>
 static inline int launch_main_fwd_seq(MainArgs& a, hipStream_t s) {
+    static_assert(!CFG::ADAM, "launch_main_fwd_adam sizes the grid of the forms with passengers");
     constexpr int lds = FirstKind<KINDS...>::value == MK_VFOLD ? (CFG::LDS_FOLD > CFG::LDS ? CFG::LDS_FOLD : CFG::LDS) : CFG::LDS;
     static DevMask attr{0};
     NCX_HIP_TRY(set_max_lds_once(attr, (const void*)k_main_fwd<CFG, DIST, KINDS...>, lds));
@@ -1129,4 +1162,30 @@
     }
 }
 
+
+template <class CFG>
+static inline int launch_main_fwd_adam(MainArgs& a, int n_pass, int pass_at_hint, hipStream_t s) {
+    static_assert(CFG::ADAM && CFG::EPI != EPI_MLB && !CFG::X6, "the answer-embedding gradient's forms");
+    if (a.nseg != 2 || a.M < 1 || a.N < 1 || a.split > 1 || a.dist_out || !a.out) return NCX_E_FLAGS;
+    for (int i = 0; i < 2; ++i) if (!main_fwd_operand_ok(a.seg[i].klen)) return NCX_E_DIMS;
+    const EpiArgs& e = a.epi;
+    if (e.rowadd || e.bias || e.relu || e.dropout || e.gate) return NCX_E_FLAGS;
+    AdamFuse& ad = a.adam;
+    if (!ad.p || !ad.m || !ad.v || (ad.tn && (!ad.tp || !ad.tg || !ad.tm || !ad.tv))) return NCX_E_NULL;
+    constexpr bool RM = CFG::EPI == EPI_ROWMAP;
+    constexpr int KIND = RM ? MK_GATHER : MK_PLAIN;
+    if (a.seg[0].kind != KIND || a.seg[1].kind != KIND) return NCX_E_FLAGS;
+    if (RM && (!a.seg[0].idx || a.seg[0].idx != a.seg[1].idx)) return NCX_E_FLAGS;
+    constexpr int lds = CFG::LDS;
+    static DevMask attr{0};
+    NCX_HIP_TRY(set_max_lds_once(attr, (const void*)k_main_fwd<CFG, false, KIND, KIND>, lds));
+    const int tiles_m = (a.M + CFG::BM - 1) / CFG::BM, tiles_n = (a.N + CFG::BN - 1) / CFG::BN;
+    const int grid = ((tiles_m + 7) / 8) * 8 * tiles_n;
+    ad.n_pass = ad.tn ? (n_pass > 0 ? n_pass : 1) : 0;
+    ad.pass_at = pass_at_hint >= 0 && pass_at_hint < grid ? pass_at_hint : grid;
+    hipLaunchKernelGGL((k_main_fwd<CFG, false, KIND, KIND>), dim3(grid + ad.n_pass), dim3(CFG::T), lds, s, a);
+    NCX_HIP_TRY(hipGetLastError());
+    return NCX_OK;
 }
+
+}
diff --git a/vqa-counterexamples_amd/csrc/ncx_main.hip b/vqa-counterexamples_amd/csrc/ncx_main.hip
--- a/vqa-counterexamples_amd/csrc/ncx_main.hip
+++ b/vqa-counterexamples_amd/csrc/ncx_main.hip
@@ -12,12 +12,16 @@
 typedef MainCfg<192, 64, 4, 2, 2, 2, 512, true> MainCfgFold8X6;
 typedef MainCfg<192, 64, 4, 2, 2, 2, 512> MainCfgFold8;
 
+bool main_short_form(long long M, long long N, long long T, int split) {
+    return split <= 1 && T <= 32 && ((M + 63) / 64) * ((N + 63) / 64) >= 2 * num_cus() && !hook_env("NCX_MAIN_CFG");
+}
+
 template <class C> using AsIs = C;
 template <template <class> class W>
 static int main_forward_chain(MainArgs& a, hipStream_t s) {
     long long T = 0;
     for (int i = 0; i < a.nseg; ++i) T += (a.seg[i].klen + MF_BK - 1) / MF_BK;
-    if (a.split <= 1 && T <= 32 && (long long)((a.M + 63) / 64) * ((a.N + 63) / 64) >= 2 * num_cus() && !hook_env("NCX_MAIN_CFG"))
+    if (main_short_form(a.M, a.N, T, a.split))
         return launch_main_fwd<W<MainCfg3>>(a, s);
     const long long tiles96 = (long long)((a.M + 95) / 96) * ((a.N + 127) / 128);
     constexpr bool wide_ok = W<MainCfgW>::EPI != EPI_ROWMAP;
@@ -52,6 +56,21 @@
     return main_forward_chain<WithRowMap>(a, s);
 }
 
+int main_adam_passengers() {
+    if (const char* e = hook_env("NCX_ADAM_PASS")) { const int n = atoi(e); if (n > 0) return n; }
+    return num_cus();
+}
+
+int main_forward_adam(MainArgs& a, bool rowmap, hipStream_t s) {
+    long long T = 0;
+    for (int i = 0; i < a.nseg; ++i) T += (a.seg[i].klen + MF_BK - 1) / MF_BK;
+    if (!main_short_form(a.M, a.N, T, a.split)) return NCX_E_FLAGS;
+    int at = 3 * num_cus();
+    if (const char* e = hook_env("NCX_ADAM_PASS_AT")) at = atoi(e);
+    const int np = main_adam_passengers();
+    return rowmap ? launch_main_fwd_adam<WithAdam<WithRowMap<MainCfg3>>>(a, np, at, s) : launch_main_fwd_adam<WithAdam<MainCfg3>>(a, np, at, s);
+}
+
 int main_forward_mlb(MainArgs& a, hipStream_t s) {
     const long long tiles96 = (long long)((a.M + 95) / 96) * ((a.N + 127) / 128);
     if (tiles96 * 10 >= (long long)num_cus() * 9) return launch_main_fwd<WithMlbEpi<MainCfg2>>(a, s);
diff --git a/vqa-counterexamples_amd/neuralcx/_lib.py b/vqa-counterexamples_amd/neuralcx/_lib.py
--- a/vqa-counterexamples_amd/neuralcx/_lib.py
+++ b/vqa-counterexamples_amd/neuralcx/_lib.py
@@ -12,7 +12,7 @@
 NCX_F_BF16 = 16
 
 EXPORTS = ("ncx_input_size", "ncx_workspace_bytes", "ncx_forward", "ncx_forward_phase", "ncx_loss_rank", "ncx_backward", "ncx_backward_phase",
-           "ncx_adam_step", "ncx_version", "ncx_profile_begin", "ncx_profile_end", "ncx_plan_query",
+           "ncx_adam_step", "ncx_backward_adam", "ncx_version", "ncx_profile_begin", "ncx_profile_end", "ncx_plan_query",
            "ncx_vqa_workspace_bytes", "ncx_vqa_forward", "ncx_mlb_workspace_bytes", "ncx_mlb_forward", "ncx_mlb_att_workspace_bytes", "ncx_mlb_att_forward", "ncx_mlb_att_forward_flags", "ncx_mlb_att_logits_form", "ncx_knn_workspace_bytes", "ncx_knn_status_offset", "ncx_knn", "ncx_cosine_gram_workspace_bytes", "ncx_cosine_gram", "ncx_semantic_scores",
            "ncx_similarity_scores",
            "ncx_gru_packed_bytes", "ncx_gru_pack", "ncx_gru_workspace_bytes", "ncx_gru_encode", "ncx_gru_encode_flags", "ncx_gru_step_form",
@@ -53,6 +53,12 @@
 
 class NcxGrads(C.Structure):
     _fields_ = [(n, C.c_void_p) for n in _PNAMES]
+
+
+class NcxAdamState(C.Structure):
+    _fields_ = [("param", C.c_void_p), ("grad", C.c_void_p), ("exp_avg", C.c_void_p), ("exp_avg_sq", C.c_void_p),
+                ("n", C.c_size_t), ("n_emb", C.c_size_t), ("step", C.c_int32),
+                ("lr", C.c_float), ("beta1", C.c_float), ("beta2", C.c_float), ("eps", C.c_float), ("grad_scale", C.c_float)]
 
 
 class NcxMutanParams(C.Structure):
@@ -158,6 +164,9 @@
     L.ncx_adam_step.restype = C.c_int
     L.ncx_adam_step.argtypes = [C.c_void_p, C.c_void_p, C.c_void_p, C.c_void_p, C.c_size_t, C.c_float,
                                 C.c_float, C.c_float, C.c_float, C.c_int32, C.c_float, C.c_void_p]
+    L.ncx_backward_adam.restype = C.c_int
+    L.ncx_backward_adam.argtypes = [C.POINTER(NcxDims), C.POINTER(NcxInputs), C.POINTER(NcxParams), C.c_void_p,
+                                    C.c_size_t, C.c_void_p, C.POINTER(NcxGrads), C.POINTER(NcxAdamState), C.c_void_p]
     L.ncx_vqa_workspace_bytes.restype = C.c_size_t
     L.ncx_vqa_workspace_bytes.argtypes = [C.POINTER(NcxDims), C.POINTER(NcxMutanParams)]
     L.ncx_vqa_forward.restype = C.c_int
@@ -378,8 +387,14 @@
 DW1_TN_FORMS = ("grouped", "k_dw_tn8", "k_dw_tn8_x6")
 
 
+NCX_QUERY_FUSED_ADAM = 33
+
+
 def plan_query(d, name):
     out = (C.c_int32 * 6)()
+    if name == "FUSED_ADAM":
+        check(lib().ncx_plan_query(C.byref(d), NCX_QUERY_FUSED_ADAM, out), "ncx_plan_query")
+        return dict(fused=bool(out[0]), passengers=out[1])
     if name == "DW1_ROUTE":
         check(lib().ncx_plan_query(C.byref(d), NCX_QUERY_DW1_ROUTE, out), "ncx_plan_query")
         return dict(fold=DW1_FOLD_FORMS[out[0]], tn=DW1_TN_FORMS[out[1]], tn_pieces=out[2], tn_grid=out[3],
diff --git a/vqa-counterexamples_amd/neuralcx/engine.py b/vqa-counterexamples_amd/neuralcx/engine.py
--- a/vqa-counterexamples_amd/neuralcx/engine.py
+++ b/vqa-counterexamples_amd/neuralcx/engine.py
@@ -191,7 +191,11 @@
                 ops.backward(d, batch, f, self._ws, r["dscores"], self.grads.fields())
                 torch.distributed.all_reduce(self.grads.flat[n_emb:], group=self.pg)
         else:
-            ops.backward(d, batch, self.params.fields(), self._ws, r["dscores"], self.grads.fields())
+            ops.backward_adam(d, batch, self.params.fields(), self._ws, r["dscores"], self.grads.fields(), self.params.flat,
+                              self.grads.flat, self.exp_avg, self.exp_avg_sq, self.params.offsets["linear_1.weight"], self.step_count,
+                              lr=self.lr)
+            r["scores"] = scores
+            return r
         ops.adam_step(self.params.flat, self.grads.flat, self.exp_avg, self.exp_avg_sq, self.step_count, lr=self.lr)
         r["scores"] = scores
         return r
diff --git a/vqa-counterexamples_amd/neuralcx/ops.py b/vqa-counterexamples_amd/neuralcx/ops.py
--- a/vqa-counterexamples_amd/neuralcx/ops.py
+++ b/vqa-counterexamples_amd/neuralcx/ops.py
@@ -218,6 +218,20 @@
                                         _ptr(exp_avg, torch.float32, "exp_avg"), _ptr(exp_avg_sq, torch.float32, "exp_avg_sq"),
                                         n, lr, betas[0], betas[1], eps, int(step), float(grad_scale), _stream()),
                "ncx_adam_step")
+
+
+def backward_adam(d: NcxDims, batch: Batch, params: Dict[str, torch.Tensor], ws: torch.Tensor, dscores: torch.Tensor,
+                  grads: Dict[str, torch.Tensor], param, grad, exp_avg, exp_avg_sq, n_emb, step, lr=1e-4, betas=(0.9, 0.999),
+                  eps=1e-8, grad_scale=1.0) -> None:
+    n = param.numel()
+    assert grad.numel() == n and exp_avg.numel() == n and exp_avg_sq.numel() == n
+    p, nb = _ws_ptr(ws)
+    ins, ps, gs = batch.c_struct(), _params_struct(params, NcxParams), _params_struct(grads, NcxGrads)
+    st = _lib.NcxAdamState(_ptr(param, torch.float32, "param"), _ptr(grad, torch.float32, "grad"),
+                           _ptr(exp_avg, torch.float32, "exp_avg"), _ptr(exp_avg_sq, torch.float32, "exp_avg_sq"),
+                           n, int(n_emb), int(step), lr, betas[0], betas[1], eps, float(grad_scale))
+    _lib.check(_lib.lib().ncx_backward_adam(C.byref(d), C.byref(ins), C.byref(ps), p, nb, _ptr(dscores, torch.float32, "dscores"),
+                                            C.byref(gs), C.byref(st), _stream()), "ncx_backward_adam")
 
 
 class MutanWeights:
```
